# viniciusvidal2/slam-sensor-fusion

Hardware: AMD Instinct MI355X
Metric: scans_per_s_200k_scan_vs_10M_map (higher is better)
Workload: dtype f32 points / f64 accumulation

## Files before the change

include/slamfusion.h:

```cpp
#ifndef SLAMFUSION_H
#define SLAMFUSION_H
#include <stdint.h>

#ifdef __cplusplus
extern "C" {
#endif

#define SF_VERSION 210

typedef enum {
    SF_OK = 0,
    SF_ERR_INVALID = -1,
    SF_ERR_HIP = -2,
    SF_ERR_NOMEM = -3,
    SF_ERR_STATE = -4,
    SF_ERR_OVERFLOW = -5,
    SF_ERR_COMM = -6
} sf_status;

typedef struct sf_ctx sf_ctx;
typedef struct sf_cloud sf_cloud;
typedef struct sf_map sf_map;
typedef struct sf_icp sf_icp;

// ... 28 lines not shown
int sf_cloud_from_pointcloud2(sf_cloud *c, const void *data, int64_t n_points, int point_step, int off_x, int off_y, int off_z);
#define SF_PC2_FLOAT32 7
#define SF_PC2_FLOAT64 8
int sf_cloud_from_pointcloud2_msg(sf_cloud *c, const void *data, int64_t data_bytes, int64_t width, int64_t height, int point_step, int64_t row_step,
                                  int off_x, int off_y, int off_z, int datatype, int is_bigendian);
int sf_cloud_load_pcd(sf_cloud *c, const char *path);
int sf_cloud_save_pcd(sf_cloud *c, const char *path);
int sf_pcd_read(const char *path, float **xyz, int64_t *n);
int sf_pcd_write_binary(const char *path, const float *xyz, int64_t n);
void sf_free(void *p);

#define SF_VOXEL_PCL 0
#define SF_VOXEL_O3D 1
#define SF_VOXEL_PCL64 2
#define SF_FLAG_VOXEL_OVERFLOW 1
int sf_cloud_voxel_downsample(sf_cloud *c, double leaf, int flavour, int *status_flags);
int sf_cloud_voxel_merge(sf_cloud *map, sf_cloud *pending, double leaf, int *status_flags, int *merged);
int sf_cloud_voxel_merge_min_points(int64_t n);
int sf_cloud_voxel_point_ids(sf_cloud *c, int32_t *ids, int64_t cap_values, int64_t *n_values);
int sf_cloud_voxel_out_ids(sf_cloud *c, int32_t *ids, int64_t cap_values, int64_t *n_values);
int sf_cloud_voxel_out_means_f64(sf_cloud *c, double *xyz, int64_t cap_points, int64_t *n_points);
int sf_cloud_voxel_point_ids64(sf_cloud *c, int64_t *ids, int64_t cap_values, int64_t *n_values);
int sf_cloud_voxel_out_ids64(sf_cloud *c, int64_t *ids, int64_t cap_values, int64_t *n_values);

int sf_map_create(sf_ctx *ctx, sf_map **out);
void sf_map_destroy(sf_map *m);
int sf_map_build(sf_map *m, sf_cloud *cloud, float cell);
int sf_map_size(sf_map *m, int64_t *n);
int sf_map_cell_size(sf_map *m, float *cell, int32_t dims[3]);
#define SF_PATCH_NO_MERGE        0
#define SF_PATCH_BOUND_REPLACED (-1)
#define SF_PATCH_ORIGIN_MOVED   (-2)
#define SF_PATCH_LIMITS         (-3)
#define SF_PATCH_CLAMPED_POINT  (-4)
int sf_map_patch(sf_map *m, sf_cloud *cloud, int *patched);
int sf_map_set_origin_lattice(sf_map *m, int cells);
int sf_map_index_info(sf_map *m, int64_t *n_indexed, int64_t *n_cells, float org[3], float *inv_h, float *gap_eps);
int sf_map_download_index(sf_map *m, float *pts4, int64_t cap_points, uint32_t *cell_start, int64_t cap_cells);
int sf_map_window_none(sf_map *m);
int sf_map_window_sphere(sf_map *m, const float center[3], double radius);
int sf_map_window_obb(sf_map *m, const double center[3], const double R[9], const double extent[3]);
int sf_map_window_count(sf_map *m, int64_t *n);
int sf_map_estimate_normals(sf_map *m, float radius);
int sf_map_estimate_normals_cov(sf_map *m, float radius, int with_covariance);
int sf_map_download_covariances(sf_map *m, double *cov6, int64_t cap_points, int64_t *n);
int sf_map_set_normals(sf_map *m, const float *normals, int64_t n);
int sf_map_set_normals_carry(sf_map *m, int on);
int sf_map_normals_carry_info(sf_map *m, int64_t out[4]);
int sf_map_download_normals(sf_map *m, float *normals, int32_t *n_neighbors, int64_t cap, int64_t *n);
int sf_map_nn(sf_map *m, const float *queries, int64_t n, float max_d2, int32_t *idx, float *d2);
#define SF_KNN_MAX 64
int sf_map_knn(sf_map *m, const float *queries, int64_t n, int k, float max_d2, int32_t *idx, float *d2, int32_t *count);
int sf_map_estimate_normals_knn(sf_map *m, int k, float max_radius, int with_covariance);
int sf_map_profile_launches(sf_map *m, int on);
int sf_map_last_launch_ms(sf_map *m, float *ms);

typedef struct {
    float T[16];
    float error;
    int32_t iterations;
    int32_t converged;
    int32_t n_corr;
    int32_t n_research;
    int32_t flags;
    double fitness;
    double rmse;
    double T64[16];
} sf_icp_result;
#define SF_ICP_FLAG_FEW_CORR 1
#define SF_ICP_FLAG_SINGULAR 2
#define SF_ICP_FLAG_BARRIER_TIMEOUT 8
#define SF_ICP_FLAG_SHARD_STALE 4

#define SF_ICP_REF_CPP 0
#define SF_ICP_O3D_P2P 1
#define SF_ICP_P2PLANE 2

int sf_icp_create(sf_ctx *ctx, float max_correspondence_dist, int num_iterations,
                  float acceptable_mean_error, float transformation_epsilon, sf_icp **out);
void sf_icp_destroy(sf_icp *icp);
int sf_icp_set_max_correspondence_dist(sf_icp *icp, float v);
int sf_icp_set_num_iterations(sf_icp *icp, int v);
int sf_icp_set_transformation_epsilon(sf_icp *icp, float v);
int sf_icp_set_acceptable_mean_error(sf_icp *icp, float v);
int sf_icp_set_initial_transformation(sf_icp *icp, const float T[16]);
int sf_icp_set_initial_transformation_f64(sf_icp *icp, const double T[16]);
int sf_icp_set_debug_mode(sf_icp *icp, int on);
int sf_icp_set_source(sf_icp *icp, const float *xyz, int64_t n);
int sf_icp_set_source_cloud(sf_icp *icp, sf_cloud *cloud);
int sf_icp_set_source_scan(sf_icp *icp, sf_cloud *raw, int stride, const float center[3], double radius);
int sf_icp_source_count(sf_icp *icp, int64_t *n);
int sf_icp_set_target(sf_icp *icp, const float *xyz, int64_t n);
int sf_icp_set_target_map(sf_icp *icp, sf_map *map);
int sf_icp_align(sf_icp *icp, int mode, sf_icp_result *out);

int sf_icp_set_source_batch(sf_icp *icp, const float *xyz, int64_t n_per_scan, int batch);
int sf_icp_set_source_batch_device(sf_icp *icp, const void *d_xyz, int64_t n_per_scan, int batch);
int sf_icp_set_initial_batch_f64(sf_icp *icp, const double *inits);
int sf_icp_align_batch(sf_icp *icp, int mode, sf_icp_result *out );
int sf_icp_align_batch_async(sf_icp *icp, int mode);
int sf_icp_fetch_results(sf_icp *icp, sf_icp_result *out);
int sf_icp_fetch_previous(sf_icp *icp, sf_icp_result *out);
int sf_icp_use_graph(sf_icp *icp, int on);
int sf_icp_graph_counts(sf_icp *icp, int64_t *captures, int64_t *launches);
int sf_icp_set_fused(sf_icp *icp, int on);
int sf_icp_fused_count(sf_icp *icp, int64_t *launches);
int sf_icp_fused_redone(sf_icp *icp, int64_t *redone);
int sf_icp_test_inject_barrier_timeout(sf_icp *icp);
#define SF_ORDER_AUTO 0
#define SF_ORDER_AS_GIVEN 1
#define SF_ORDER_CELL 2
int sf_icp_set_query_order(sf_icp *icp, int order);
int sf_icp_set_nn_reuse(sf_icp *icp, int on);
int sf_icp_set_wide_scan_points(sf_icp *icp, int64_t points);
int sf_icp_set_pipeline(sf_icp *icp, int on);
int sf_icp_set_tile_search(sf_icp *icp, int mode);
int sf_icp_tile_info(sf_icp *icp, int64_t out[12]);
int sf_icp_set_freeze(sf_icp *icp, int on);
int sf_icp_set_freeze_params(sf_icp *icp, float guard_scale, float guard_min, float guard_max, int max_tries, int from_launch);
int sf_icp_freeze_stats(sf_icp *icp, int64_t out[5]);
int sf_icp_set_defer_search(sf_icp *icp, int on);
int sf_icp_defer_stats(sf_icp *icp, int64_t out[2]);
#define SF_ROBUST_NONE 0
#define SF_ROBUST_HUBER 1
#define SF_ROBUST_CAUCHY 2
#define SF_ROBUST_TUKEY 3
#define SF_ROBUST_GM 4
int sf_icp_set_robust_kernel(sf_icp *icp, int kind, double k);

#define SF_COV_EIG_EPS 1e-12
#define SF_COV_FEW_CORR 1
#define SF_COV_SINGULAR 2
#define SF_COV_DEGENERATE_TRANS 4
#define SF_COV_DEGENERATE_ROT 8
typedef struct {
    double info[36];
    double cov[36];
    double sigma2, sigma2_hat, weight_sum;
    double trans_info[3], trans_dir[9];
    double rot_info[3], rot_dir[9];
    int64_t n_corr;
    int32_t flags;
} sf_icp_covariance;
int sf_icp_set_covariance(sf_icp *icp, int on, double sensor_sigma);
int sf_icp_set_degeneracy_thresholds(sf_icp *icp, double trans, double rot, double inflate_trans_var, double inflate_rot_var);
int sf_icp_fetch_covariance(sf_icp *icp, sf_icp_covariance *out);
int sf_icp_fetch_covariance_previous(sf_icp *icp, sf_icp_covariance *out);

int sf_icp_set_shard(sf_icp *icp, float x_lo, float x_hi);
int sf_icp_set_shard_margin(sf_icp *icp, float margin_m);
int sf_icp_set_exchange_buffer(sf_icp *icp, void *d_buf, int64_t nbytes);
void *sf_icp_exchange_ptr(sf_icp *icp, int64_t *nbytes);
int sf_icp_step_begin(sf_icp *icp, int mode, int first);
int sf_icp_step_end(sf_icp *icp, int mode, int last);

typedef struct sf_comm sf_comm;
int sf_comm_load_rccl(const char *library_path);
int sf_comm_unique_id(void *id128);
int sf_comm_create(sf_ctx *ctx, int nranks, int rank, const void *id128, sf_comm **out);
void sf_comm_destroy(sf_comm *c);
int sf_comm_size(const sf_comm *c, int *nranks, int *rank);
int sf_comm_allreduce_f64(sf_comm *c, void *d_buf, int64_t count);
#define SF_COMM_RCCL 0
#define SF_COMM_P2P 1
#define SF_COMM_P2P_HANDLE_BYTES 128
int sf_comm_p2p_create(sf_ctx *ctx, int nranks, int rank, int64_t max_count, sf_comm **out);
int sf_comm_p2p_handle(sf_comm *c, void *handle);
int sf_comm_p2p_connect(sf_comm *c, const void *handles);
int sf_comm_p2p_rendezvous(sf_comm *c, const char *name, double timeout_s);
int sf_comm_set_timeout(sf_comm *c, double seconds);
int sf_comm_abort(sf_comm *c);
int sf_comm_status(sf_comm *c);
int sf_comm_kind(const sf_comm *c);
int sf_icp_align_sharded_async(sf_icp *icp, int mode, sf_comm *comm, int first);
int sf_icp_align_sharded(sf_icp *icp, int mode, sf_comm *comm, sf_icp_result *out, int *resumes );
// ... 150 lines not shown
```

slam_sensor_fusion_amd/api.py:

```python
import atexit
import ctypes as C
import os
import weakref

import numpy as np

_HERE = os.path.dirname(os.path.abspath(__file__))
LIB_PATH = os.path.join(_HERE, "lib", "libslamfusion.so")

SF_ICP_REF_CPP, SF_ICP_O3D_P2P, SF_ICP_P2PLANE = 0, 1, 2
SF_VOXEL_PCL, SF_VOXEL_O3D, SF_VOXEL_PCL64 = 0, 1, 2
SF_FLAG_VOXEL_OVERFLOW = 1
SF_ICP_FLAG_FEW_CORR, SF_ICP_FLAG_SINGULAR, SF_ICP_FLAG_SHARD_STALE, SF_ICP_FLAG_BARRIER_TIMEOUT = 1, 2, 4, 8
PROF_NN, PROF_REDUCE, PROF_COLLECTIVE, PROF_SOLVE, PROF_SHARD_BUILD = 0, 1, 2, 3, 4
SF_ERR_COMM = -6
MODES = {"ref_cpp": SF_ICP_REF_CPP, "o3d_p2p": SF_ICP_O3D_P2P, "p2plane": SF_ICP_P2PLANE}
ROBUST_KINDS = {"none": 0, "huber": 1, "cauchy": 2, "tukey": 3, "gm": 4}


class SlamFusionError(RuntimeError):
    pass


class IcpResult(C.Structure):
# ... 328 lines not shown

    def set_origin_lattice(self, cells):
        _check(self.lib.sf_map_set_origin_lattice(self.h, C.c_int(int(cells))))
        return self

    def patch(self, cloud):
        done = C.c_int(0)
        _check(self.lib.sf_map_patch(self.h, cloud.h, C.byref(done)))
        self.last_patch = done.value
        return done.value > 0

    def index(self):
        n, nc, org, inv_h, eps = C.c_int64(), C.c_int64(), (C.c_float * 3)(), C.c_float(), C.c_float()
        _check(self.lib.sf_map_index_info(self.h, C.byref(n), C.byref(nc), org, C.byref(inv_h), C.byref(eps)))
        pts4 = np.empty((max(n.value, 1), 4), np.float32)
        cs = np.empty(nc.value + 1, np.uint32)
        _check(self.lib.sf_map_download_index(self.h, pts4.ctypes.data_as(C.c_void_p), C.c_int64(len(pts4)), cs.ctypes.data_as(C.c_void_p), C.c_int64(len(cs))))
        return dict(pts4=pts4[:n.value], cell_start=cs, org=np.array(list(org), np.float32), inv_h=inv_h.value, gap_eps=eps.value)

    def __len__(self):
        n = C.c_int64()
        _check(self.lib.sf_map_size(self.h, C.byref(n)))
        return n.value

    def cell_size(self):
        cell = C.c_float()
        dims = (C.c_int32 * 3)()
        _check(self.lib.sf_map_cell_size(self.h, C.byref(cell), dims))
        return cell.value, tuple(dims)

    def window_none(self):
        _check(self.lib.sf_map_window_none(self.h))

    def window_sphere(self, center, radius):
        c = _f32(center)
        _check(self.lib.sf_map_window_sphere(self.h, _p(c), C.c_double(radius)))

    def window_obb(self, center, R, extent):
        c, R, e = _f64(center), _f64(R).reshape(3, 3), _f64(extent)
        _check(self.lib.sf_map_window_obb(self.h, _p(c), _p(R), _p(e)))

    def window_count(self):
        n = C.c_int64()
        _check(self.lib.sf_map_window_count(self.h, C.byref(n)))
        return n.value

    def estimate_normals(self, radius, covariance=False):
        _check(self.lib.sf_map_estimate_normals_cov(self.h, C.c_float(radius), C.c_int(int(covariance))))

    def estimate_normals_knn(self, k, max_radius=np.inf, covariance=False):
        r = float(max_radius)
        _check(self.lib.sf_map_estimate_normals_knn(self.h, C.c_int(int(k)), C.c_float(r if np.isfinite(r) else 0.0), C.c_int(int(covariance))))

    def set_normals_carry(self, on=True):
        _check(self.lib.sf_map_set_normals_carry(self.h, C.c_int(int(bool(on)))))
        return self

    def normals_carry_info(self):
        out = (C.c_int64 * 4)()
        _check(self.lib.sf_map_normals_carry_info(self.h, out))
        return tuple(int(v) for v in out)

    def download_covariances(self):
        n = len(self)
        cov = np.empty((n, 6), np.float64)
        _check(self.lib.sf_map_download_covariances(self.h, _p(cov), C.c_int64(n), None))
        return cov

    def set_normals(self, normals):
        nrm = _f32(normals).reshape(-1, 3)
        _check(self.lib.sf_map_set_normals(self.h, _p(nrm), C.c_int64(len(nrm))))

    def download_normals(self):
        n = len(self)
        nrm = np.empty((n, 3), np.float32)
        cnt = np.empty(n, np.int32)
        _check(self.lib.sf_map_download_normals(self.h, _p(nrm), _p(cnt), C.c_int64(n), None))
        return nrm, cnt

    def nn(self, queries, max_d2=np.inf):
        q = _f32(queries).reshape(-1, 3)
        idx = np.empty(len(q), np.int32)
        d2 = np.empty(len(q), np.float32)
        _check(self.lib.sf_map_nn(self.h, _p(q), C.c_int64(len(q)), C.c_float(min(max_d2, 3.0e38)), _p(idx), _p(d2)))
        return idx, d2

    def knn(self, queries, k, max_d2=np.inf):
        q = _f32(queries).reshape(-1, 3)
        k = int(k)
        rows = max(k, 0)
        idx = np.empty((len(q), rows), np.int32)
        d2 = np.empty((len(q), rows), np.float32)
        cnt = np.empty(len(q), np.int32)
        _check(self.lib.sf_map_knn(self.h, _p(q), C.c_int64(len(q)), C.c_int(k), C.c_float(max_d2), _p(idx), _p(d2), _p(cnt)))
        return idx, d2, cnt

    def profile_launches(self, on=True):
        _check(self.lib.sf_map_profile_launches(self.h, C.c_int(int(bool(on)))))
        return self

    def last_launch_ms(self):
        ms = C.c_float()
        _check(self.lib.sf_map_last_launch_ms(self.h, C.byref(ms)))
        return ms.value

    def close(self):
# ... 123 lines not shown
        code = {False: 0, "off": 0, "auto": 1, True: 2, "always": 2}[on]
        _check(self.lib.sf_icp_set_freeze(self.h, C.c_int(code)))

    def set_robust_kernel(self, kind="none", k=None):
        code = ROBUST_KINDS[kind]
        _check(self.lib.sf_icp_set_robust_kernel(self.h, code, float("nan") if k is None and code != 0 else float(k or 0.0)))

    def set_covariance(self, on=True, sensor_sigma=0.0):
        _check(self.lib.sf_icp_set_covariance(self.h, int(bool(on)), float(sensor_sigma)))

    def set_degeneracy_thresholds(self, trans=0.0, rot=0.0, inflate_trans_var=0.0, inflate_rot_var=0.0):
        _check(self.lib.sf_icp_set_degeneracy_thresholds(self.h, float(trans), float(rot), float(inflate_trans_var), float(inflate_rot_var)))

    def fetch_covariance(self, previous=False, batch=None):
        if previous:
            arr = (IcpCovariance * int(batch or getattr(self, "_prev_batch", None) or self.batch))()
            _check(self.lib.sf_icp_fetch_covariance_previous(self.h, arr))
        else:
            arr = (IcpCovariance * int(batch or getattr(self, "_last_batch", None) or self.batch))()
            _check(self.lib.sf_icp_fetch_covariance(self.h, arr))
        return [c.as_dict() for c in arr]

    def set_wide_scan_points(self, points):
        _check(self.lib.sf_icp_set_wide_scan_points(self.h, C.c_int64(int(points))))

    def set_pipeline(self, on=True):
        _check(self.lib.sf_icp_set_pipeline(self.h, C.c_int(int(bool(on)))))

    def set_tile_search(self, on="auto"):
        code = {False: 0, "off": 0, "auto": 1, True: 2, "always": 2}[on]
        _check(self.lib.sf_icp_set_tile_search(self.h, C.c_int(code)))

    def tile_info(self):
        a = (C.c_int64 * 12)()
        _check(self.lib.sf_icp_tile_info(self.h, a))
        return {"on": bool(a[0]), "cells_per_tile": [a[1], a[2], a[3]], "tiles": [a[4], a[5], a[6]], "searched": a[7], "from_lds": a[8], "left_region": a[9],
                "beyond_ring_1": a[10], "tiles_too_dense": a[11]}

    def set_freeze_params(self, guard_scale=8.0, guard_min=2.0e-5, guard_max=3.0e-4, max_tries=3, from_launch=5):
        _check(self.lib.sf_icp_set_freeze_params(self.h, C.c_float(guard_scale), C.c_float(guard_min), C.c_float(guard_max), C.c_int(max_tries), C.c_int(from_launch)))

    def freeze_stats(self):
        a = (C.c_int64 * 5)()
        _check(self.lib.sf_icp_freeze_stats(self.h, a))
        return {"froze": a[0], "thawed": a[1], "failed": a[2], "active_queries": a[3], "frozen_at_end": a[4]}

    def set_defer_search(self, on=True):
        _check(self.lib.sf_icp_set_defer_search(self.h, C.c_int(int(bool(on)))))

    def defer_stats(self):
        a = (C.c_int64 * 2)()
        _check(self.lib.sf_icp_defer_stats(self.h, a))
        return {"deferred_queries": a[0], "capped_waves": a[1]}

    def set_query_order(self, order="auto"):
        _check(self.lib.sf_icp_set_query_order(self.h, C.c_int({"auto": 0, "as_given": 1, "cell": 2}[order])))

    def align(self, mode="ref_cpp"):
        r = IcpResult()
        _check(self.lib.sf_icp_align(self.h, C.c_int(MODES[mode]), C.byref(r)))
        return r.as_dict()

    def align_batch(self, mode="p2plane"):
        arr = (IcpResult * self.batch)()
        _check(self.lib.sf_icp_align_batch(self.h, C.c_int(MODES[mode]), arr))
        self._prev_batch, self._last_batch = getattr(self, "_last_batch", None), self.batch
        return [r.as_dict() for r in arr]

    def align_batch_async(self, mode="p2plane"):
        _check(self.lib.sf_icp_align_batch_async(self.h, C.c_int(MODES[mode])))
        self._prev_batch, self._last_batch = getattr(self, "_last_batch", None), self.batch

    def fetch_results(self, raw=False):
        arr = (IcpResult * int(getattr(self, "_last_batch", None) or self.batch))()
        _check(self.lib.sf_icp_fetch_results(self.h, arr))
        return arr if raw else [r.as_dict() for r in arr]

    def fetch_previous(self, batch=None, raw=False):
        arr = (IcpResult * int(batch or getattr(self, "_prev_batch", None) or self.batch))()
        _check(self.lib.sf_icp_fetch_previous(self.h, arr))
        return arr if raw else [r.as_dict() for r in arr]

    def set_shard(self, x_lo, x_hi):
        _check(self.lib.sf_icp_set_shard(self.h, C.c_float(x_lo), C.c_float(x_hi)))

    def set_exchange_buffer(self, ptr, nbytes):
        _check(self.lib.sf_icp_set_exchange_buffer(self.h, C.c_void_p(ptr), C.c_int64(nbytes)))

    def exchange_ptr(self):
        n = C.c_int64()
        p = self.lib.sf_icp_exchange_ptr(self.h, C.byref(n))
        return p, n.value

    def set_shard_margin(self, margin_m):
        _check(self.lib.sf_icp_set_shard_margin(self.h, C.c_float(margin_m)))

    def step_begin(self, mode, first):
        _check(self.lib.sf_icp_step_begin(self.h, C.c_int(MODES[mode]), C.c_int(int(first))))
        if int(first) == 1:
            self._last_batch = self.batch

    def step_end(self, mode, last):
        _check(self.lib.sf_icp_step_end(self.h, C.c_int(MODES[mode]), C.c_int(int(last))))

    def align_sharded(self, mode, comm):
        arr = (IcpResult * self.batch)()
# ... 610 lines not shown
```

slam_sensor_fusion_amd/csrc/sf_common.hpp:

```cpp
#pragma once
#include <hip/hip_runtime.h>
#include <cstdarg>
#include <cstdint>
#include <cstdio>
#include <cstring>
#include <new>
#include <vector>

#include "slamfusion.h"

namespace sf {

void set_error(const char *fmt, ...);

#define SF_HIP(call)                                                                          \
    do {                                                                                      \
        hipError_t e_ = (call);                                                               \
        if (e_ != hipSuccess) {                                                               \
            sf::set_error("%s failed: %s (%s:%d)", #call, hipGetErrorString(e_), __FILE__,    \
                          __LINE__);                                                          \
            return SF_ERR_HIP;                                                                \
        }                                                                                     \
    } while (0)

// ... 80 lines not shown
    bool zombie = false;
};

struct sf_cloud {
    sf_ctx *ctx = nullptr;
    sf::DevBuf xyz;
    int64_t n = 0;
    sf::DevBuf spare;
    sf::DevBuf flags;
    sf::DevBuf raw;
    sf::DevBuf last_idx;
    int64_t n_last_idx = -1;
    bool vox_wide = false;
    sf::DevBuf vox_point_ids; int64_t n_vox_point_vals = 0;
    sf::DevBuf vox_out_ids;   int64_t n_vox_out_vals = 0;
    sf::DevBuf vox_out_means; int64_t n_vox_out_pts = 0;
    uint64_t stamp = 0;
    uint64_t bounds_stamp = 0;
    float bounds_mn[3] = {0, 0, 0}, bounds_mx[3] = {0, 0, 0};
    struct MergeRecord {
        bool valid = false;
        uint64_t epoch = 0, stamp_before = 0, stamp_after = 0;
        int64_t n_old = 0, n_groups = 0, n_fresh = 0;
        float old_mn[3] = {0, 0, 0}, old_mx[3] = {0, 0, 0};
        float cen_mn[3] = {0, 0, 0}, cen_mx[3] = {0, 0, 0};
        bool touched_extreme = false;
        const uint32_t *coarse = nullptr;
        const uint32_t *g_rank = nullptr, *g_fresh = nullptr, *fresh_pos = nullptr, *fresh_rank = nullptr;
        const float *g_centroid = nullptr, *g_old = nullptr;
    } merge;
};

struct SfWindow {
    int kind;
    float c[3];
    float r2;
    double oc[3];
    double oR[9];
    double ohalf[3];
};

struct SfGrid {
    float org[3];
    float inv_h;
    float h;
    float gap_eps;
    int dim[3];
    const uint32_t *cell_start;
    const float4 *pts;
    const float4 *nrm;
    int64_t n;
};

struct sf_map {
    sf_ctx *ctx = nullptr;
    sf::DevBuf pts4, nrm4, cell_start, keys, vals, keys2, vals2;
    sf::DevBuf pts4_alt, patch_tmp;
    double h_exact = 0;
    float src_mn[3] = {0, 0, 0}, src_mx[3] = {0, 0, 0};
    int origin_lattice = 0;
    uint64_t src_stamp = 0;
    sf::DevBuf d_window;
    sf::DevBuf cov6;
    sf::DevBuf nrm4_alt, cov6_alt, carry_tmp, carry_list;
    bool normals_carry = false;
    bool nrm_estimated = false;
    float nrm_radius = 0;
    int nrm_knn_k = 0;
    bool nrm_with_cov = false;
    int64_t carry_info[4] = {-1, 0, 0, 0};
    bool profile = false;
    hipEvent_t prof_ev[2] = {nullptr, nullptr};
    float last_launch_ms = -1.0f;
    int64_t n = 0;
    bool built = false, has_normals = false, has_cov = false;
    uint64_t generation = 0;
    SfGrid grid{};
    SfWindow window{};
};

struct sf_comm;

namespace sf {
int comm_allreduce_f64(sf_comm *c, void *d_buf, int64_t count);
sf_ctx *comm_ctx(const sf_comm *c);
int compact_cloud(sf_cloud *c, const uint8_t *d_flags);
int ensure_scratch(sf_ctx *ctx, size_t bytes);
int upload_staged(sf_ctx *ctx, void *dst, const void *src, size_t bytes);
uint64_t next_generation();
inline void cloud_touch(sf_cloud *c) { c->stamp = next_generation(); c->merge.valid = false; }
void ctx_retain(sf_ctx *ctx);
void ctx_release(sf_ctx *ctx);
struct MinMaxHost { float mn[3], mx[3]; int64_t n_finite; };
struct MinMaxDev { float mn[3], mx[3]; unsigned long long cnt; };
int cloud_minmax_enqueue(sf_ctx *ctx, const float *d_xyz, int64_t n, MinMaxDev *d_out);
int cloud_minmax(sf_ctx *ctx, const float *d_xyz, int64_t n, MinMaxHost *out);
}
```

slam_sensor_fusion_amd/csrc/sf_icp.hip:

```cpp
#include "sf_common.hpp"
#include "sf_nn.hpp"
#include "sf_tile.hpp"
#include "sf_order.hpp"
#include "sf_p2p.hpp"

#include <cfloat>
#include <cstdlib>
#include <cmath>
#include <vector>
#include <mutex>
#include <string>

namespace {

constexpr int BLK = 256;
constexpr int NREC_P2P = 17;
constexpr int NREC_PLANE = 30;
constexpr int REC_STRIDE = 32;

struct IcpState {
    double T[16];
    double rec[REC_STRIDE];
    double fitness, rmse, prev_fitness, prev_rmse;
    float last_error, err_pending;
// ... 460 lines not shown
    }
    return need;
}

struct QueryIn {
    double sx, sy, sz;
    float qx, qy, qz;
    float4 c1, c2;
    float e;
    size_t o;
    bool valid;
};

template <int MODE, bool SHARD>
__device__ __forceinline__ QueryIn query_in(const float *__restrict__ X0x, const float *__restrict__ X0y, const float *__restrict__ X0z, int n, int b, const IcpState *S, float xlo,
                                            float xhi, const uint32_t *__restrict__ own_off, const float4 *__restrict__ qcache, int64_t cache_n, bool cache_live, int slot,
                                            int n_live)
{
    QueryIn q;
    q.sx = q.sy = q.sz = 0.0;
    q.qx = q.qy = q.qz = 0.0f;
    q.c1 = q.c2 = make_float4(0.f, 0.f, 0.f, 0.f);
    q.e = 0.0f;
    q.o = 0;
    q.valid = false;
    if (slot < n_live) {
        const size_t o = SHARD ? (size_t)own_off[b] + (size_t)slot : (size_t)b * n + (size_t)slot;
        q.o = o;
        if (cache_live) {
            q.c1 = qcache[o];
            if (MODE == 2) { q.c2 = qcache[(size_t)cache_n + o]; q.e = q.c2.w; }
            else q.e = reinterpret_cast<const float *>(qcache + (size_t)cache_n)[o];
        }
        const double x0 = X0x[o], y0 = X0y[o], z0 = X0z[o];
        q.sx = S->T[0] * x0 + S->T[1] * y0 + S->T[2] * z0 + S->T[3];
        q.sy = S->T[4] * x0 + S->T[5] * y0 + S->T[6] * z0 + S->T[7];
        q.sz = S->T[8] * x0 + S->T[9] * y0 + S->T[10] * z0 + S->T[11];
        q.qx = (float)q.sx; q.qy = (float)q.sy; q.qz = (float)q.sz;
        q.valid = !SHARD || (q.qx >= xlo && q.qx < xhi);
    }
    return q;
}

__device__ __forceinline__ LanePair make_pair(const QueryIn &q, const sf::NNHit &hit, const float4 &tn)
{
    LanePair P;
    P.sx = q.sx; P.sy = q.sy; P.sz = q.sz;
    P.px = hit.px; P.py = hit.py; P.pz = hit.pz;
    P.tn = tn;
    P.ok = hit.j >= 0;
    return P;
}

template <int MODE, bool WINDOW, bool SHARD>
__device__ __forceinline__ LanePair nn_pair(const SfGrid &g, const SfWindow &w, const float *__restrict__ X0x, const float *__restrict__ X0y, const float *__restrict__ X0z,
                                            int n, int b, const IcpState *S, float thr, float xlo, float xhi, const uint32_t *__restrict__ own_off,
                                            float4 *__restrict__ qcache, int64_t cache_n, int slot, int n_live, sf::WaveNN *ws, uint32_t *__restrict__ stats,
                                            sf::PhaseClock *pc = nullptr)
{
    const bool cache_live = qcache != nullptr && S->cache_live != 0;
    const QueryIn q = query_in<MODE, SHARD>(X0x, X0y, X0z, n, b, S, xlo, xhi, own_off, qcache, cache_n, cache_live, slot, n_live);
    const float qx = q.qx, qy = q.qy, qz = q.qz;
    const size_t o = q.o;
    float *ecache = reinterpret_cast<float *>(qcache + (size_t)cache_n);
    const float m_now = (float)S->motion;
    sf::NNHit hit;
    float4 tn;
    sf::NNHit seed;
    const bool need = reuse_certificate(q.valid, qx, qy, qz, thr, m_now, q.e, q.c1, q.c2, hit, tn, seed);
    const unsigned long long need_mask = __ballot(need);
    if (stats && (threadIdx.x & 63) == 0 && need_mask) {
        uint32_t *sh = stats + 2 * ((blockIdx.x + blockIdx.y * gridDim.x) & (NN_STATS_SHARDS - 1));
        atomicAdd(&sh[0], (uint32_t)__popcll(need_mask));
        atomicAdd(&sh[1], 1u);
    }
    SF_PH(pc, 0);
    if (need_mask != 0ull) {
        const sf::NNHit h = sf::nn_search_wave<WINDOW>(g, w, need, qx, qy, qz, thr, ws, seed, pc);
        if (need) {
            hit = h;
            if (MODE == 2 && h.j >= 0) tn = g.nrm[h.j];
            if (qcache) {
                const float en = fmaxf(sqrtf(h.lb2) * 0.9999f + m_now * 0.999998f - 1.0e-6f, 1.0e-30f);
                qcache[o] = make_float4(h.px, h.py, h.pz, __int_as_float(h.j));
                if (MODE == 2) qcache[(size_t)cache_n + o] = make_float4(tn.x, tn.y, tn.z, en);
                else ecache[o] = en;
            }
        }
    }
    if (qcache && !cache_live && !need && slot < n_live) {
        if (MODE == 2) qcache[(size_t)cache_n + o] = make_float4(0.f, 0.f, 0.f, 0.f);
        else ecache[o] = 0.0f;
    }
    SF_PH(pc, 6);
    return make_pair(q, hit, tn);
}

struct PairTerms { double wgt, ux, uy, uz, tx, ty, tz, ex, ey, ez, d2, r; double J[6]; };
template <int MODE>
__device__ __forceinline__ PairTerms pair_terms(const LanePair &P)
{
    PairTerms t;
    const bool ok = P.ok;
    t.wgt = ok ? 1.0 : 0.0;
    t.ux = ok ? P.sx : 0.0; t.uy = ok ? P.sy : 0.0; t.uz = ok ? P.sz : 0.0;
    t.tx = (double)(ok ? P.px : 0.0f); t.ty = (double)(ok ? P.py : 0.0f); t.tz = (double)(ok ? P.pz : 0.0f);
    t.ex = t.ux - t.tx; t.ey = t.uy - t.ty; t.ez = t.uz - t.tz;
    t.d2 = t.ex * t.ex + t.ey * t.ey + t.ez * t.ez;
    if (MODE == 2) {
        const double nx = (double)(ok ? P.tn.x : 0.0f), ny = (double)(ok ? P.tn.y : 0.0f), nz = (double)(ok ? P.tn.z : 0.0f);
        t.r = t.ex * nx + t.ey * ny + t.ez * nz;
        t.J[0] = t.uy * nz - t.uz * ny; t.J[1] = t.uz * nx - t.ux * nz; t.J[2] = t.ux * ny - t.uy * nx;
        t.J[3] = nx; t.J[4] = ny; t.J[5] = nz;
    } else {
        t.r = 0.0;
#pragma unroll
        for (int a = 0; a < 6; ++a) t.J[a] = 0.0;
    }
    return t;
}

struct RobustArg { int kind; double k; };
__device__ __forceinline__ double robust_weight(const RobustArg &rk, double r)
// ... 21 lines not shown
            v[13] = fma(t.uz, t.tx, v[13]); v[14] = fma(t.uz, t.ty, v[14]); v[15] = fma(t.uz, t.tz, v[15]);
        } else {
            v[0] += t.d2;
        }
    } else {
        if (h == 0) { v[0] += t.wgt; v[1] = fma(t.r, t.r, v[1]); }
        int k = 2;
#pragma unroll
        for (int a = 0; a < 6; ++a) {
#pragma unroll
            for (int c = a; c < 6; ++c) {
                if (h == 0 && k < 16) v[k] = fma(t.J[a], t.J[c], v[k]);
                if (h == 1 && k >= 16) v[k - 16] = fma(t.J[a], t.J[c], v[k - 16]);
                ++k;
            }
        }
        if (h == 1) {
#pragma unroll
            for (int a = 0; a < 6; ++a) v[7 + a] = fma(t.J[a], t.r, v[7 + a]);
            v[13] += t.d2;
        }
    }
}

__device__ __forceinline__ void add_half_robust(const PairTerms &t, int h, double (&v)[16], double w)
{
    double Jw[6];
#pragma unroll
    for (int a = 0; a < 6; ++a) Jw[a] = w * t.J[a];
    if (h == 0) { v[0] += t.wgt; v[1] = fma(t.r, t.r, v[1]); }
    int k = 2;
#pragma unroll
    for (int a = 0; a < 6; ++a) {
#pragma unroll
        for (int c = a; c < 6; ++c) {
            if (h == 0 && k < 16) v[k] = fma(Jw[a], t.J[c], v[k]);
            if (h == 1 && k >= 16) v[k - 16] = fma(Jw[a], t.J[c], v[k - 16]);
            ++k;
        }
    }
    if (h == 1) {
#pragma unroll
        for (int a = 0; a < 6; ++a) v[7 + a] = fma(Jw[a], t.r, v[7 + a]);
        v[13] += t.d2;
    }
}

#ifdef SF_PHASE_TRACE
__device__ unsigned long long g_phase_trace[sf::PH_SHARDS * sf::PH_SLOTS];
#endif
template <int MODE, bool WINDOW, bool SHARD, int Q>
__global__ __launch_bounds__(BLK, NN_RED_WAVES) void k_nn_red(SfGrid g, SfWindow w, const float *__restrict__ X0x, const float *__restrict__ X0y, const float *__restrict__ X0z,
                                                int n, const IcpState *__restrict__ st, float thr, float xlo, float xhi, double *__restrict__ partials, int nblocks,
                                                const uint32_t *__restrict__ own_off, float4 *__restrict__ qcache, int64_t cache_n, uint32_t *__restrict__ stats)
{
    constexpr bool ROBUST = false;
    [[maybe_unused]] constexpr RobustArg rk{0, 0.0};
#include "sf_nn_red_body.inc"
}

template <bool WINDOW, bool SHARD, int Q>
__global__ __launch_bounds__(BLK, NN_RED_WAVES) void k_nn_red_rob(SfGrid g, SfWindow w, const float *__restrict__ X0x, const float *__restrict__ X0y, const float *__restrict__ X0z,
                                                    int n, const IcpState *__restrict__ st, float thr, float xlo, float xhi, double *__restrict__ partials, int nblocks,
                                                    const uint32_t *__restrict__ own_off, float4 *__restrict__ qcache, int64_t cache_n, uint32_t *__restrict__ stats, RobustArg rk)
{
    constexpr int MODE = 2;
    constexpr bool ROBUST = true;
#include "sf_nn_red_body.inc"
}

constexpr int ORDER_YBLK = 16;
__device__ __forceinline__ uint64_t order_cell(const SfGrid &g, int cx, int cy, int cz)
{
    const uint64_t yb = (uint64_t)(cy / ORDER_YBLK), yi = (uint64_t)(cy % ORDER_YBLK);
    return ((yb * (uint64_t)g.dim[2] + (uint64_t)cz) * ORDER_YBLK + yi) * (uint64_t)g.dim[0] + (uint64_t)cx;
}

struct CellKeyFn {
    SfGrid g;
    const float *x, *y, *z;
    const IcpState *st;
    int n, shift;
    const uint16_t *lut;
    int lut_shift;
    struct Point { float x, y, z; };
    struct Pose { float T[12]; };
    __device__ __forceinline__ Pose prepare(int b) const
    {
        Pose P;
#pragma unroll
        for (int k = 0; k < 12; ++k) P.T[k] = (float)st[b].T[k];
        return P;
    }
    __device__ __forceinline__ Point load(uint32_t o) const { return Point{x[o], y[o], z[o]}; }
    __device__ __forceinline__ uint32_t key(const Pose &P, const Point &p) const
    {
        const float qx = fmaf(P.T[0], p.x, fmaf(P.T[1], p.y, fmaf(P.T[2], p.z, P.T[3])));
        const float qy = fmaf(P.T[4], p.x, fmaf(P.T[5], p.y, fmaf(P.T[6], p.z, P.T[7])));
        const float qz = fmaf(P.T[8], p.x, fmaf(P.T[9], p.y, fmaf(P.T[10], p.z, P.T[11])));
        if (!(isfinite(qx) && isfinite(qy) && isfinite(qz))) return sf::ORD_KEY_NONE;
        const int cx = (int)fminf(fmaxf(floorf((qx - g.org[0]) * g.inv_h), 0.0f), (float)(g.dim[0] - 1));
        const int cy = (int)fminf(fmaxf(floorf((qy - g.org[1]) * g.inv_h), 0.0f), (float)(g.dim[1] - 1));
        const int cz = (int)fminf(fmaxf(floorf((qz - g.org[2]) * g.inv_h), 0.0f), (float)(g.dim[2] - 1));
        if (lut) return (uint32_t)lut[order_cell(g, cx, cy, cz) >> lut_shift];
        const uint64_t key = order_cell(g, cx, cy, cz) >> shift;
        return (uint32_t)(key < (uint64_t)(sf::ORD_KEY_NONE - 1u) ? key : (uint64_t)(sf::ORD_KEY_NONE - 1u));
    }
};

__global__ __launch_bounds__(sf::ORD_BLK) void k_order_hist(sf::OrderSrc s, CellKeyFn kf, uint16_t *__restrict__ keys, uint32_t *__restrict__ counts)
{
    sf::order_hist_body(s, kf, keys, counts);
}

constexpr int ORDER_LUT_LOG2 = 16;
__global__ __launch_bounds__(256) void k_order_lut_hist(SfGrid g, int lut_shift, uint32_t *__restrict__ hist)
{
// ... 688 lines not shown
    return stays_in || stays_out;
}

struct FzArgs {
    const float *X0x, *X0y, *X0z;
    int n;
    const IcpState *st;
    float thr, xlo, xhi;
    double *partials;
    int nblocks;
    const uint32_t *own_off;
    float4 *qcache;
    int64_t cache_n;
    uint32_t *stats;
    const FreezeState *fz;
    double *mom_part;
    uint32_t *act_cnt;
    uint16_t *act_ids;
    const uint32_t *act_all;
};

template <int Q, bool SHARD>
__device__ __forceinline__ void nn_red_fz_row(const SfGrid &g, const SfWindow &w, const FzArgs &A, int b, int bx, int fmode)
{
    constexpr int MODE = 2;
    constexpr int NREC = NREC_PLANE;
    static_assert(FZ_CAP == 64 * Q, "wave 0 takes FZ_CAP active queries in Q rounds of 64");
    const float *__restrict__ X0x = A.X0x, *__restrict__ X0y = A.X0y, *__restrict__ X0z = A.X0z;
    const int n = A.n, nblocks = A.nblocks;
    const float thr = A.thr, xlo = A.xlo, xhi = A.xhi;
    double *__restrict__ partials = A.partials, *__restrict__ mom_part = A.mom_part;
    const uint32_t *__restrict__ own_off = A.own_off, *__restrict__ act_all = A.act_all;
    float4 *__restrict__ qcache = A.qcache;
    const int64_t cache_n = A.cache_n;
    uint32_t *__restrict__ stats = A.stats, *__restrict__ act_cnt = A.act_cnt;
    uint16_t *__restrict__ act_ids = A.act_ids;
    const FreezeState *__restrict__ fz = A.fz;
    const IcpState *S = A.st + b;
    const int n_live = SHARD ? (int)(own_off[b + 1] - own_off[b]) : n;
    const int wv = threadIdx.x >> 6, lane = threadIdx.x & 63;
    const size_t row = (size_t)b * nblocks + bx;
    double *dst = partials + row * REC_STRIDE;
    __shared__ sf::WaveNN nn_ws[BLK / 64];
    LanePair P[Q];
    if (fmode == 2) {
        const int64_t total = fz[b].n_active, first = (int64_t)bx * FZ_CAP;
        if (first >= total) return;
        __shared__ double fstage[Q][32];
        if (wv < Q) {
            const uint32_t cnt = (uint32_t)min<int64_t>(total - first, FZ_CAP);
            const uint32_t *list = act_all + (size_t)b * nblocks * FZ_CAP + (size_t)first;
            const uint32_t i = (uint32_t)(wv * 64 + lane);
            const int slot = i < cnt ? (int)list[i] : n_live;
            const LanePair A1 = nn_pair<MODE, false, SHARD>(g, w, X0x, X0y, X0z, n, b, S, thr, xlo, xhi, own_off, qcache, cache_n, slot, n_live, &nn_ws[wv], stats);
#pragma unroll
            for (int h = 0; h < 2; ++h) {
                double v[16];
#pragma unroll
                for (int k = 0; k < 16; ++k) v[k] = 0.0;
                const PairTerms t = pair_terms<MODE>(A1);
                add_half<MODE>(t, h, v);
                const double t0 = wave_reduce_16(v);
                if ((lane & 3) == 0) fstage[wv][16 * h + (lane >> 2)] = t0;
            }
        }
        __syncthreads();
        if (threadIdx.x < NREC) {
            double v = fstage[0][threadIdx.x];
#pragma unroll
            for (int u = 1; u < Q; ++u) v += fstage[u][threadIdx.x];
            dst[threadIdx.x] = v;
        }
        return;
    }
    if (SHARD && bx * (BLK * Q) >= n_live) return;
    __shared__ double stage[BLK / 64][32];
    __shared__ uint32_t act_w[BLK / 64][Q];
    bool active[Q];
#pragma unroll
    for (int u = 0; u < Q; ++u) active[u] = false;
    bool fast = false;
    const float m_now = (float)S->motion;
    const float guard = fz[b].guard;
    const bool attempted = qcache != nullptr && S->cache_live != 0;
    if (attempted) {
        bool any_need = false;
#pragma unroll
        for (int u = 0; u < Q; ++u) {
            const int slot = bx * (BLK * Q) + u * BLK + (int)threadIdx.x;
            const QueryIn q = query_in<MODE, SHARD>(X0x, X0y, X0z, n, b, S, xlo, xhi, own_off, qcache, cache_n, true, slot, n_live);
            sf::NNHit hit, seed;
            float4 tn;
            any_need = reuse_certificate(q.valid, q.qx, q.qy, q.qz, thr, m_now, q.e, q.c1, q.c2, hit, tn, seed) || any_need;
            P[u] = make_pair(q, hit, tn);
            if (fmode == 1) active[u] = !stays_frozen<SHARD>(q, slot < n_live, thr, m_now, guard, xlo, xhi);
        }
        fast = __ballot(any_need) == 0ull;
    }
    if (!fast) {
        asm volatile("" ::: "memory");
#pragma unroll
        for (int u = 0; u < Q; ++u) {
            const int slot = bx * (BLK * Q) + u * BLK + (int)threadIdx.x;
            P[u] = nn_pair<MODE, false, SHARD>(g, w, X0x, X0y, X0z, n, b, S, thr, xlo, xhi, own_off, qcache, cache_n, slot, n_live, &nn_ws[wv], stats);
            if (fmode == 1 && !attempted) active[u] = slot < n_live;
        }
    }
    if (fmode == 1) {
#pragma unroll
        for (int u = 0; u < Q; ++u) {
            const unsigned long long bal = __ballot(active[u]);
            if (lane == 0) act_w[wv][u] = (uint32_t)__popcll(bal);
        }
        __syncthreads();
        uint32_t total = 0;
#pragma unroll
        for (int u = 0; u < Q; ++u) {
            uint32_t base = 0;
#pragma unroll
            for (int ww = 0; ww < BLK / 64; ++ww) {
                if (ww < wv) base += act_w[ww][u];
                total += act_w[ww][u];
            }
            uint32_t before = 0;
#pragma unroll
            for (int uu = 0; uu < Q; ++uu)
                if (uu < u)
#pragma unroll
                    for (int ww = 0; ww < BLK / 64; ++ww) before += act_w[ww][uu];
            const unsigned long long bal = __ballot(active[u]);
            const uint32_t rank = (uint32_t)__builtin_amdgcn_mbcnt_hi((uint32_t)(bal >> 32), __builtin_amdgcn_mbcnt_lo((uint32_t)bal, 0u));
            const uint32_t pos = before + base + rank;
            if (active[u] && pos < (uint32_t)FZ_CAP) act_ids[row * FZ_CAP + pos] = (uint16_t)(u * BLK + (int)threadIdx.x);
        }
        if (threadIdx.x == 0) act_cnt[row] = total;
    }
    bool wave_has_pairs = true;
    if (fmode == 1) {
        bool any = false;
#pragma unroll
        for (int u = 0; u < Q; ++u) any = any || (P[u].ok && active[u]);
        wave_has_pairs = __ballot(any) != 0ull;
        if (!wave_has_pairs && lane < 32) stage[wv][lane] = 0.0;
    }
    if (wave_has_pairs)
#pragma unroll
    for (int h = 0; h < 2; ++h) {
        double v[16];
#pragma unroll
        for (int k = 0; k < 16; ++k) v[k] = 0.0;
#pragma unroll
        for (int u = 0; u < Q; ++u) {
            LanePair A = P[u];
            if (fmode == 1) A.ok = A.ok && active[u];
            const PairTerms t = pair_terms<MODE>(A);
            add_half<MODE>(t, h, v);
        }
// ... 28 lines not shown
    }
}

template <int Q, bool SHARD>
__global__ __launch_bounds__(BLK, NN_RED_WAVES) void k_nn_red_fz(SfGrid g, SfWindow w, FzArgs A)
{
    const int L = blockIdx.y * gridDim.x + blockIdx.x;
    const int kk = L >> 3;
    const int b = kk % (int)gridDim.y;
    const int bx = (L & 7) * ((int)gridDim.x >> 3) + kk / (int)gridDim.y;
    if (bx >= A.nblocks) return;
    if (A.st[b].done) return;
    nn_red_fz_row<Q, SHARD>(g, w, A, b, bx, A.fz[b].mode);
}

constexpr int FZ_FEW = 16;
template <int Q, bool SHARD>
__global__ __launch_bounds__(BLK, NN_RED_WAVES) void k_nn_red_fz_few(SfGrid g, SfWindow w, FzArgs A)
{
    const int r = (int)blockIdx.x, b = (int)blockIdx.y;
    if (A.st[b].done) return;
    const int fmode = A.fz[b].mode;
    if (fmode == 2) {
        const int64_t total = A.fz[b].n_active;
        for (int bx = r; (int64_t)bx * FZ_CAP < total; bx += FZ_FEW) {
            nn_red_fz_row<Q, SHARD>(g, w, A, b, bx, 2);
            __syncthreads();
        }
        return;
    }
    for (int bx = r; bx < A.nblocks; bx += FZ_FEW) {
        nn_red_fz_row<Q, SHARD>(g, w, A, b, bx, fmode);
        __syncthreads();
    }
}


#ifndef SF_DF_WCAP
#define SF_DF_WCAP 8
#endif
constexpr int DF_WCAP = SF_DF_WCAP;
constexpr int DF_CAPPED = 255;
static_assert((BLK / 64) * DF_WCAP <= FZ_CAP && DF_WCAP < DF_CAPPED, "a row defers fewer queries than it could list as active");
struct DeferBufs {
    uint8_t *cnt;
    uint16_t *ids;
    double *part;
    uint32_t *stat;
};

template <int Q>
__global__ __launch_bounds__(BLK, NN_RED_WAVES) void k_nn_red_df(SfGrid g, SfWindow w, const float *__restrict__ X0x, const float *__restrict__ X0y, const float *__restrict__ X0z,
                                                                 int n, const IcpState *__restrict__ st, float thr, double *__restrict__ partials, int nblocks,
                                                                 float4 *__restrict__ qcache, int64_t cache_n, uint32_t *__restrict__ stats, DeferBufs df)
{
    constexpr int MODE = 2;
    constexpr int NREC = NREC_PLANE;
    const int L = blockIdx.y * gridDim.x + blockIdx.x;
    const int kk = L >> 3;
    const int b = kk % (int)gridDim.y;
    const int bx = (L & 7) * ((int)gridDim.x >> 3) + kk / (int)gridDim.y;
    if (bx >= nblocks) return;
    const IcpState *S = st + b;
    if (S->done) return;
    __shared__ sf::WaveNN nn_ws[BLK / 64];
    __shared__ double stage[BLK / 64][32];
    const int wv = threadIdx.x >> 6, lane = threadIdx.x & 63;
    const size_t seg = ((size_t)b * nblocks + bx) * (BLK / 64) + wv;
    LanePair P[Q];
    bool need[Q];
#pragma unroll
    for (int u = 0; u < Q; ++u) need[u] = false;
    const bool attempted = qcache != nullptr && S->cache_live != 0 && S->n_research >= VERIFY_FROM_SEARCH;
    bool fast = false;
    uint32_t listed = 0;
    if (attempted) {
        const float m_now = (float)S->motion;
#pragma unroll
        for (int u = 0; u < Q; ++u) {
            const int slot = bx * (BLK * Q) + u * BLK + (int)threadIdx.x;
            const QueryIn q = query_in<MODE, false>(X0x, X0y, X0z, n, b, S, 0.0f, 0.0f, nullptr, qcache, cache_n, true, slot, n);
            sf::NNHit hit, seed;
            float4 tn;
            need[u] = reuse_certificate(q.valid, q.qx, q.qy, q.qz, thr, m_now, q.e, q.c1, q.c2, hit, tn, seed);
            P[u] = make_pair(q, hit, tn);
        }
        uint32_t failing = 0;
#pragma unroll
        for (int u = 0; u < Q; ++u) failing += (uint32_t)__popcll(__ballot(need[u]));
        fast = failing <= (uint32_t)DF_WCAP;
        listed = fast ? failing : (uint32_t)DF_CAPPED;
    }
    if (lane == 0) df.cnt[seg] = (uint8_t)listed;
    if (fast && listed != 0u) {
        uint32_t before = 0;
#pragma unroll
        for (int u = 0; u < Q; ++u) {
            const unsigned long long bal = __ballot(need[u]);
            const uint32_t rank = (uint32_t)__builtin_amdgcn_mbcnt_hi((uint32_t)(bal >> 32), __builtin_amdgcn_mbcnt_lo((uint32_t)bal, 0u));
            if (need[u]) df.ids[seg * DF_WCAP + before + rank] = (uint16_t)(u * BLK + (int)threadIdx.x);
            before += (uint32_t)__popcll(bal);
        }
    }
    if (!fast) {
        asm volatile("" ::: "memory");
#pragma unroll
        for (int u = 0; u < Q; ++u) {
            const int slot = bx * (BLK * Q) + u * BLK + (int)threadIdx.x;
            P[u] = nn_pair<MODE, false, false>(g, w, X0x, X0y, X0z, n, b, S, thr, 0.0f, 0.0f, nullptr, qcache, cache_n, slot, n, &nn_ws[wv], stats);
        }
    }
#pragma unroll
    for (int h = 0; h < 2; ++h) {
        double v[16];
#pragma unroll
        for (int k = 0; k < 16; ++k) v[k] = 0.0;
#pragma unroll
        for (int u = 0; u < Q; ++u) {
            const PairTerms t = pair_terms<MODE>(P[u]);
            add_half<MODE>(t, h, v);
        }
        const double t0 = wave_reduce_16(v);
        if ((lane & 3) == 0) stage[wv][16 * h + (lane >> 2)] = t0;
    }
    __syncthreads();
    if (threadIdx.x < NREC) {
        const int c = threadIdx.x;
        double *dst = partials + ((size_t)b * nblocks + bx) * REC_STRIDE;
        dst[c] = ((stage[0][c] + stage[1][c]) + stage[2][c]) + stage[3][c];
    }
}

template <int Q>
__global__ __launch_bounds__(BLK, 2) void k_nn_deferred(SfGrid g, SfWindow w, const float *__restrict__ X0x, const float *__restrict__ X0y, const float *__restrict__ X0z,
                                                                   int n, const IcpState *__restrict__ st, float thr, int nblocks, float4 *__restrict__ qcache, int64_t cache_n,
                                                                   uint32_t *__restrict__ stats, DeferBufs df)
{
    constexpr int MODE = 2;
    constexpr int NW = BLK / 64;
    const int r = (int)blockIdx.x, b = (int)blockIdx.y;
    const IcpState *S = st + b;
    if (S->done) return;
    __shared__ sf::WaveNN nn_ws[NW];
    __shared__ double fstage[NW][32];
    __shared__ uint32_t list[BLK * DF_WCAP];
    __shared__ uint32_t wsum[NW];
    __shared__ uint32_t capped;
    const int wv = threadIdx.x >> 6, lane = threadIdx.x & 63;
    if (threadIdx.x == 0) capped = 0u;
    __syncthreads();
    const int my_rows = r < nblocks ? (nblocks - r + FZ_FEW - 1) / FZ_FEW : 0;
    const int nseg = my_rows * NW;
    double acc = 0.0;
    uint32_t n_listed = 0;
    for (int s0 = 0; s0 < nseg; s0 += BLK) {
        const int sg = s0 + (int)threadIdx.x;
        const int bx = r + (sg / NW) * FZ_FEW;
        const size_t seg = ((size_t)b * nblocks + bx) * NW + (sg % NW);
        uint32_t c = sg < nseg ? (uint32_t)df.cnt[seg] : 0u;
        if (c > (uint32_t)DF_WCAP) {
            atomicAdd(&capped, 1u);
            c = 0u;
        }
        uint32_t incl = c;
#pragma unroll
        for (int off = 1; off < 64; off <<= 1) {
            const uint32_t t = __shfl_up(incl, off, 64);
            if (lane >= off) incl += t;
        }
        if (lane == 63) wsum[wv] = incl;
        __syncthreads();
        uint32_t base = 0, total = 0;
#pragma unroll
        for (int ww = 0; ww < NW; ++ww) {
            if (ww < wv) base += wsum[ww];
            total += wsum[ww];
        }
        const uint32_t start = base + incl - c;
        for (uint32_t i = 0; i < c; ++i) list[start + i] = (uint32_t)bx * (uint32_t)(BLK * Q) + (uint32_t)df.ids[seg * DF_WCAP + i];
        __syncthreads();
        n_listed += total;
        for (uint32_t q0 = 0; q0 < total; q0 += BLK) {
            const uint32_t i = q0 + (uint32_t)threadIdx.x;
            if (q0 + (uint32_t)(wv * 64) < total) {
                const int slot = i < total ? (int)list[i] : n;
                const LanePair A1 = nn_pair<MODE, false, false>(g, w, X0x, X0y, X0z, n, b, S, thr, 0.0f, 0.0f, nullptr, qcache, cache_n, slot, n, &nn_ws[wv], stats);
#pragma unroll
                for (int h = 0; h < 2; ++h) {
                    double v[16];
#pragma unroll
                    for (int k = 0; k < 16; ++k) v[k] = 0.0;
                    const PairTerms t = pair_terms<MODE>(A1);
                    add_half<MODE>(t, h, v);
                    const double t0 = wave_reduce_16(v);
                    if ((lane & 3) == 0) fstage[wv][16 * h + (lane >> 2)] = t0;
                }
            } else if (lane < 32) {
                fstage[wv][lane] = 0.0;
            }
            __syncthreads();
            if (threadIdx.x < 32) acc += ((fstage[0][threadIdx.x] + fstage[1][threadIdx.x]) + fstage[2][threadIdx.x]) + fstage[3][threadIdx.x];
            __syncthreads();
        }
    }
    if (threadIdx.x < REC_STRIDE) df.part[((size_t)b * FZ_FEW + r) * REC_STRIDE + threadIdx.x] = threadIdx.x < NREC_PLANE ? acc : 0.0;
    __syncthreads();
    if (threadIdx.x == 0) {
        if (n_listed) atomicAdd(&df.stat[0], n_listed);
        if (capped) atomicAdd(&df.stat[1], capped);
    }
}

__device__ __forceinline__ void add_deferred_rows(const double *__restrict__ df_part, int b, double *rec)
{
    if (threadIdx.x < NREC_PLANE) {
        double v = 0.0;
#pragma unroll
        for (int r = 0; r < FZ_FEW; ++r) v += df_part[((size_t)b * FZ_FEW + r) * REC_STRIDE + threadIdx.x];
        rec[threadIdx.x] += v;
    }
    __syncthreads();
}

template <int STRIDE, int NCOL, int NT>
__device__ __forceinline__ void reduce_columns(const double *__restrict__ part, int nrows, double *out)
{
    constexpr int NS = 8;
    static_assert(NT % 128 == 0 && NT / 128 >= 1 && NT / 128 <= NS && NCOL <= 128, "slices of 128 columns");
    __shared__ double sl[NS][128];
    const int c = threadIdx.x & 127;
    for (int sidx = threadIdx.x >> 7; sidx < NS; sidx += NT / 128) {
        double v0 = 0, v1 = 0, v2 = 0, v3 = 0;
        if (c < NCOL) {
            int r = sidx;
            for (; r + 3 * NS < nrows; r += 4 * NS) {
                const double a0 = part[(size_t)r * STRIDE + c], a1 = part[(size_t)(r + NS) * STRIDE + c];
                const double a2 = part[(size_t)(r + 2 * NS) * STRIDE + c], a3 = part[(size_t)(r + 3 * NS) * STRIDE + c];
                v0 += a0; v1 += a1; v2 += a2; v3 += a3;
            }
// ... 171 lines not shown
                F->froze += 1;
                if (S->froze_launch < 0) S->froze_launch = S->n_research;
                F->motion0 = S->motion;
                for (int i = 0; i < 12; ++i) { F->Tf[i] = S->T[i]; F->D[i] = (i % 5 == 0) ? 1.0 : 0.0; }
                for (int i = 0; i < FZ_NMOM; ++i) F->mom[i] = mom[i];
            }
        }
    }
    __syncthreads();
}

__device__ __forceinline__ void freeze_after_update(const IcpState *S, FreezeState *F, double m0, double m1, const FreezeParams &fp, int request, const double *upd)
{
    if (F->mode == 2) {
        double Dn[12];
        for (int r = 0; r < 3; ++r) {
            for (int c = 0; c < 4; ++c) Dn[4 * r + c] = upd[4 * r] * F->D[c] + upd[4 * r + 1] * F->D[4 + c] + upd[4 * r + 2] * F->D[8 + c] + (c == 3 ? upd[4 * r + 3] : 0.0);
        }
        for (int i = 0; i < 12; ++i) F->D[i] = Dn[i];
    }
    if (F->mode == 2 && !(m1 - F->motion0 <= (double)F->guard * 0.98)) {
        F->mode = 0;
        F->tries += 1;
        F->thawed += 1;
    }
    if (F->mode == 0 && F->launch_mode == 0 && request && !S->done && F->tries < fp.max_tries) {
        const float gd = fmaxf((float)(m1 - m0) * fp.guard_scale, fp.guard_min);
        if (gd <= fp.guard_max) { F->guard = gd; F->mode = 1; }
    }
}

__global__ __launch_bounds__(RBLK) void k_reduce_solve_fz(IcpState *__restrict__ st, const double *__restrict__ partials, int nblocks, int n_src, int K,
                                                          const ScanBox *__restrict__ boxp, FreezeBufs fb, FreezeParams fp, int request)
{
    const int b = blockIdx.x;
    IcpState *S = st + b;
    if (S->done) return;
    FreezeState *F = fb.fz + b;
    __shared__ double rec[REC_STRIDE];
    freeze_fold<RBLK>(S, F, b, partials, nblocks, nblocks, fb, rec);
    if (fb.df_part) add_deferred_rows(fb.df_part, b, rec);
    if (threadIdx.x == 0) {
        for (int c = 0; c < NREC_PLANE; ++c) S->rec[c] = rec[c];
        double To[12];
#pragma unroll
        for (int i = 0; i < 12; ++i) To[i] = S->T[i];
        const double m0 = S->motion;
        double upd[12];
        solve_plane(S, rec, n_src, K, upd);
        track_motion(S, To, boxp[b]);
        freeze_after_update(S, F, m0, S->motion, fp, request, upd);
    }
}

__global__ void k_fz_init(FreezeState *__restrict__ fz, int batch, uint32_t *__restrict__ df_stat)
{
    const int b = blockIdx.x * blockDim.x + threadIdx.x;
    if (b == 0) df_stat[0] = df_stat[1] = 0u;
    if (b >= batch) return;
    FreezeState *F = fz + b;
    F->mode = 0; F->tries = 0; F->froze = 0; F->thawed = 0; F->n_active = 0; F->guard = 0.0f; F->launch_mode = 0; F->motion0 = 0.0;
}

constexpr int SBLK = 256;
template <int MODE>
__global__ __launch_bounds__(SBLK) void k_reduce_only(IcpState *__restrict__ st, const double *__restrict__ partials, int nblocks, double *__restrict__ xchg,
                                                      const uint32_t *__restrict__ own_off, int qpl, FreezeBufs fb)
{
    constexpr int NREC = MODE == 2 ? NREC_PLANE : NREC_P2P;
    const int b = blockIdx.x;
    __shared__ double rec[REC_STRIDE];
    if (st[b].done) {
        if (threadIdx.x < REC_STRIDE) xchg[(size_t)b * REC_STRIDE + threadIdx.x] = 0.0;
        return;
    }
    const int rows = own_off ? (int)((own_off[b + 1] - own_off[b] + BLK * qpl - 1) / (BLK * qpl)) : nblocks;
    if (MODE == 2 && fb.fz) freeze_fold<SBLK>(st + b, fb.fz + b, b, partials, nblocks, rows, fb, rec);
    else reduce_partials<NREC, SBLK>(partials + (size_t)b * nblocks * REC_STRIDE, rows, rec);
    if (MODE == 2 && fb.df_part) add_deferred_rows(fb.df_part, b, rec);
    if (threadIdx.x < REC_STRIDE) xchg[(size_t)b * REC_STRIDE + threadIdx.x] = rec[threadIdx.x];
}

template <int MODE>
__global__ void k_solve_only(IcpState *__restrict__ st, const double *__restrict__ xchg, int n_src, int K, int batch, const ScanBox *__restrict__ boxp, float margin,
                             FreezeState *__restrict__ fz, FreezeParams fp, int request)
{
    constexpr int NREC = MODE == 2 ? NREC_PLANE : NREC_P2P;
    const int b = blockIdx.x * blockDim.x + threadIdx.x;
    if (b >= batch) return;
    IcpState *S = st + b;
    if (S->done) return;
    double rec[REC_STRIDE];
#pragma unroll
    for (int c = 0; c < REC_STRIDE; ++c) rec[c] = c < NREC ? xchg[(size_t)b * REC_STRIDE + c] : 0.0;
#pragma unroll
    for (int c = 0; c < NREC; ++c) S->rec[c] = rec[c];
    double To[12];
#pragma unroll
    for (int i = 0; i < 12; ++i) To[i] = S->T[i];
    const double m0 = S->motion;
    double upd[12];
    if (MODE == 1) solve_o3d(S, rec, n_src, 0, K);
    else solve_plane(S, rec, n_src, K, upd);
    track_motion(S, To, boxp[b]);
    if (margin > 0.0f && !S->done) own_check_motion(S, boxp[b], margin);
    if (MODE == 2 && fz) freeze_after_update(S, fz + b, m0, S->motion, fp, request, upd);
// ... 473 lines not shown
#include "sf_icp_fused_body.inc"
}

#include "sf_cov.hpp"

}

struct sf_icp {
    sf_ctx *ctx = nullptr;
    IcpParams prm{};
    int debug = 0;
    int64_t cache_n = 0;
    bool reuse = true;
    int order = SF_ORDER_AUTO;
    bool ordered = false;
    std::vector<double> inits;
    double *h_inits = nullptr;
    size_t h_inits_cap = 0;
    hipEvent_t inits_ev = nullptr;
    bool inits_ev_pending = false;
    sf_map *map = nullptr;
    sf_map *own_map = nullptr;
    sf_cloud *own_cloud = nullptr;
    sf::DevBuf xchg_own;
    void *xchg = nullptr;
    int64_t xchg_bytes = 0;
    int64_t wide_from = WIDE_SCAN_POINTS;
    bool wide_auto = true;
    std::vector<IcpState> h_state;
    bool shard = false;
    float xlo = 0, xhi = 0;
    sf::DevBuf own_idx, own_blk, own_count, own_off, own_keep;
    std::vector<uint32_t> h_own;
    int64_t own_total = 0;
    float own_margin = 1.0f;
    int own_nblocks = 1;
    sf::DevBuf d_box;
    int last_mode = 0;
    bool fused = true;
    bool last_fused = false;
    sf::DevBuf bar;
    int fused_limit[4] = {-1, -1, -1, -1};
    double fused_share = 0.0;
    int64_t fused_redone = 0;
    bool inject_timeout = false;
    int64_t fused_launches = 0;
    IcpState *h_pin = nullptr;
    size_t h_pin_cap = 0;
    bool use_graph = false;
    int64_t graph_captures = 0, graph_replays = 0;
    struct GraphKey {
        int mode = -1, iters = -1, batch = -1, window = -1, ordered = -1, reuse = -1, robust_kind = -1, cov_on = -1;
        int64_t n = -1;
        const void *map = nullptr;
        uint64_t map_generation = 0, epochs = 0;
        float max_corr = 0, accept = 0, eps = 0;
        double robust_k = 0;
        double cov_prm[5] = {0, 0, 0, 0, 0};
        bool operator==(const GraphKey &o) const
        {
            return mode == o.mode && iters == o.iters && batch == o.batch && window == o.window && ordered == o.ordered && reuse == o.reuse && n == o.n && map == o.map &&
                   map_generation == o.map_generation && epochs == o.epochs && max_corr == o.max_corr && accept == o.accept && eps == o.eps &&
                   robust_kind == o.robust_kind && robust_k == o.robust_k && cov_on == o.cov_on && std::memcmp(cov_prm, o.cov_prm, sizeof(cov_prm)) == 0;
        }
    };
    struct LaneMeta {
        bool valid = false;
        bool cov = false;
        int batch = 0, mode = 0;
        std::vector<double> inits;
        int src_set = 0;
        uint64_t src_version = 0;
    };
    struct Lane {
        sf::DevBuf X;
        sf::DevBuf qcache;
        sf::DevBuf Xq, qkeys, qkeys2, qidx, qidx2;
        sf::DevBuf corr;
        sf::DevBuf state, d_inits, partials;
        sf::DevBuf fz_state, fz_part, fz_cnt, fz_ids, fz_all;
        sf::DevBuf df_cnt, df_ids, df_part, df_stat;
        sf::DevBuf qtkey, tseg, tile_stats;
        sf::DevBuf cov_part, cov_out;
        hipGraphExec_t graph_exec = nullptr;
        GraphKey graph_key;
        std::vector<double> inits_uploaded;
        uint32_t d_inits_epoch = 0xffffffffu;
        hipStream_t stream = nullptr;
        hipEvent_t done = nullptr;
        bool used = false;
        hipEvent_t started = nullptr;
        bool started_rec = false;
        LaneMeta meta;
    } lanes[2];
    int lane = 0;
    Lane &cur() { return lanes[lane]; }
    const Lane &cur() const { return lanes[lane]; }
    Lane &prev() { return lanes[lane ^ 1]; }
    struct SrcSet {
        sf::DevBuf X0;
        sf::DevBuf X0r;
        sf::DevBuf stage;
        sf::DevBuf d_boxes, d_box_parts;
        sf::DevBuf n_dev;
        int64_t n = 0;
        int64_t n_cap = 0;
        int64_t plane = 0;
        int batch = 0;
        int nblocks = 0;
        int nblocks_nn = 0;
        int qpl = 1;
        bool have_source = false;
        bool n_on_device = false;
        hipEvent_t used = nullptr;
        bool used_rec = false;
    } srcs[2];
    int src_set = 0;
    SrcSet &src() { return srcs[src_set]; }
    const SrcSet &src() const { return srcs[src_set]; }
    hipEvent_t src_ready = nullptr;
    bool src_ahead = false;
    hipEvent_t unmarked_ev = nullptr;
    bool src_unmarked_use = false;
    bool prev_ok = false;
    std::vector<IcpState> h_prev;
    sf::DevBuf order_lut;
    uint64_t order_lut_gen = 0;
    int order_lut_shift = 0, order_lut_on = 1;
    int pipeline = 1;
    hipEvent_t main_mark = nullptr;
    bool unfetched = false;
    bool mark_valid = false;
    uint64_t src_version = 0, mark_src_version = 0, mark_map_generation = 0;
    const void *mark_map = nullptr;
    SfWindow mark_window{};
    bool profiling = false;
    std::vector<hipEvent_t> ev;
    size_t ev_used = 0;
    int64_t prof_launches = 0;
    double prof_ms = 0;
    std::vector<float> prof_each;
    std::vector<int> ev_kind;
    std::vector<float> prof_phase[SF_PROF_KINDS];
    sf::DevBuf nn_stats;
    int freeze = 1;
    FreezeParams fz_prm{8.0f, 2.0e-5f, 3.0e-4f, 3};
    int fz_from = 5;
    bool fz_from_auto = true;
    int fz_fetches = 0;
    int fz_step = 0;
    int defer = 1;
    bool df_planned = false;
    int64_t nn_stats_used = 0;
    static constexpr int64_t NN_STATS_CAP = 1024;
    int robust_kind = SF_ROBUST_NONE;
    double robust_k = 0.0;
    int cov_on = 0;
    CovArg cov_arg{0.0, 0.0, 0.0, 0.0, 0.0};
    bool prev_cov_ok = false;
    int tile_mode = 0;
    bool tile_on = false;
    sf::SfTiles tiles{};
};

namespace {

using Lane = sf_icp::Lane;
using SrcSet = sf_icp::SrcSet;
float *soa(sf::DevBuf &b, int64_t total, int axis) { return b.as<float>() + (size_t)axis * (size_t)total; }
const float *queries(sf_icp *icp, int axis)
{
    Lane &ln = icp->cur(); SrcSet &ss = icp->src();
    if (icp->shard) return soa(ln.Xq, icp->own_total, axis);
    return soa(icp->ordered ? ln.Xq : ss.X0, ss.plane, axis);
}

int fused_capacity(sf_icp *icp, int mode, bool robust = false);

bool robust_on(const sf_icp *icp, int mode) { return mode == SF_ICP_P2PLANE && icp->robust_kind != SF_ROBUST_NONE; }
RobustArg robust_arg(const sf_icp *icp) { return RobustArg{icp->robust_kind, icp->robust_k}; }

constexpr int64_t ORDER_AUTO_MIN_QUERIES = 300000;

struct OrderSpan { uint64_t cells; int bits; };
OrderSpan order_span(const SfGrid &g)
{
    const uint64_t ny_pad = ((uint64_t)g.dim[1] + ORDER_YBLK - 1) / ORDER_YBLK * ORDER_YBLK;
    OrderSpan sp{(uint64_t)g.dim[0] * ny_pad * (uint64_t)g.dim[2], 0};
    while (sp.bits < 63 && (1ull << sp.bits) < sp.cells) ++sp.bits;
    return sp;
}

int order_key_shift(const SfGrid &g) { return std::max(0, order_span(g).bits - sf::ORD_KEY_BITS); }

int reuse_reset(sf_icp *icp, int64_t count)
{
    if (!icp->reuse && !icp->tile_on) return SF_OK;
    const size_t c = (size_t)std::max<int64_t>(count, 1);
    SF_TRY(icp->cur().qcache.reserve(sizeof(float4) * 2 * c));
    icp->cache_n = (int64_t)c;
    return SF_OK;
}

// ... 12 lines not shown
        if (tc[a] <= 2) return false;
        tc[a] /= 2;
    }
    for (;;) {
        int a = tc[2] <= tc[1] && tc[2] <= tc[0] ? 2 : (tc[1] <= tc[0] ? 1 : 0);
        int t2[3] = {tc[0], tc[1], tc[2]};
        t2[a] *= 2;
        if (!fits_tables(t2) || region_cells(t2) * density > budget) break;
        tc[0] = t2[0]; tc[1] = t2[1]; tc[2] = t2[2];
    }
    if (!fits_tables(tc)) return false;
    sf::SfTiles tl;
    int64_t nt = 1;
    for (int a = 0; a < 3; ++a) {
        tl.tc[a] = tc[a];
        tl.nt[a] = (g.dim[a] + tc[a] - 1) / tc[a];
        nt *= tl.nt[a];
    }
    if (nt >= (int64_t)TILE_KEY_NONE) return false;
    tl.ntiles = (int)nt;
    *out = tl;
    return true;
}

bool tile_wanted(const sf_icp *icp, int mode)
{
    const SrcSet &ss = icp->src();
    if (icp->tile_mode == 0 || robust_on(icp, mode) || icp->shard || icp->map->window.kind != 0 || (mode != SF_ICP_P2PLANE && mode != SF_ICP_O3D_P2P)) return false;
    if (ss.qpl == 1) return false;
    return icp->tile_mode == 2 || ss.n * ss.batch >= TILE_AUTO_MIN_QUERIES;
}

bool tile_launch(const sf_icp *icp, int k) { return icp->tile_on && (!icp->reuse || k < VERIFY_FROM_SEARCH); }

constexpr int ORDER_LUT_BINS = (1 << ORDER_LUT_LOG2) + 1;
int order_lut_prepare(sf_icp *icp)
{
    if (!icp->order_lut_on || !icp->map || !icp->map->built) return SF_OK;
    const SfGrid &g = icp->map->grid;
    if (g.n <= 0 || (icp->order_lut.p && icp->order_lut_gen == icp->map->generation)) return SF_OK;
    const OrderSpan sp = order_span(g);
    icp->order_lut_shift = std::max(0, sp.bits - ORDER_LUT_LOG2);
    const int nbins = (int)(sp.cells >> icp->order_lut_shift) + 1;
    SF_TRY(icp->order_lut.reserve(sizeof(uint32_t) * (size_t)ORDER_LUT_BINS + sizeof(uint16_t) * (size_t)ORDER_LUT_BINS));
    uint32_t *hist = icp->order_lut.as<uint32_t>();
    uint16_t *lut = reinterpret_cast<uint16_t *>(hist + ORDER_LUT_BINS);
    hipStream_t st = icp->ctx->stream;
    SF_HIP(hipMemsetAsync(hist, 0, sizeof(uint32_t) * (size_t)ORDER_LUT_BINS, st));
    hipLaunchKernelGGL(k_order_lut_hist, dim3(nblk(g.n)), dim3(256), 0, st, g, icp->order_lut_shift, hist);
    hipLaunchKernelGGL(k_order_lut_make, dim3(1), dim3(1024), 0, st, hist, nbins, (uint32_t)g.n, lut);
    SF_HIP(hipGetLastError());
    icp->order_lut_gen = icp->map->generation;
    return SF_OK;
}

int run_order_sort(sf_icp *icp, int nseg, int64_t longest, int64_t total, const uint32_t *seg_off, const uint32_t *src_idx)
{
    Lane &ln = icp->cur(); SrcSet &ss = icp->src();
    const SfGrid &g = icp->map->grid;
    if (seg_off) icp->tile_on = false;
    sf::OrderSrc src;
    src.src_idx = src_idx;
    src.seg_off = seg_off;
    src.n = (int)ss.n;
    src.tiles = (int)std::max<int64_t>(1, sf::div_up(longest, sf::ORD_TILE));
    CellKeyFn kf;
    kf.g = g;
    kf.x = soa(ss.X0, ss.plane, 0); kf.y = soa(ss.X0, ss.plane, 1); kf.z = soa(ss.X0, ss.plane, 2);
    kf.st = ln.state.as<IcpState>();
    kf.shift = order_key_shift(g);
    kf.lut = nullptr;
    kf.lut_shift = 0;
    if (icp->order_lut_on && icp->order_lut.p && icp->order_lut_gen == icp->map->generation) {
        kf.lut = reinterpret_cast<const uint16_t *>(icp->order_lut.as<uint32_t>() + ORDER_LUT_BINS);
        kf.lut_shift = icp->order_lut_shift;
    }
    const size_t cap = (size_t)std::max<int64_t>(total, 1);
    SF_TRY(ln.Xq.reserve(sizeof(float) * 3 * std::max(cap, (size_t)(seg_off ? 0 : ss.plane))));
    SF_TRY(ln.qkeys.reserve(sizeof(uint16_t) * cap));
    SF_TRY(ln.qkeys2.reserve(sizeof(uint32_t) * (size_t)nseg * (size_t)(src.tiles + 1) * sf::ORD_BINS));
    SF_TRY(ln.qidx.reserve(sizeof(uint32_t) * cap));
    uint16_t *keys = ln.qkeys.as<uint16_t>();
    uint32_t *counts = ln.qkeys2.as<uint32_t>(), *ordered = ln.qidx.as<uint32_t>();
    hipStream_t s = icp->ctx->stream;
    src.nseg = nseg;
    const dim3 grid(sf::order_grid(src.tiles, nseg)), blk(sf::ORD_BLK);
    if (icp->tile_on) {
        TileKeyFn tk;
        tk.g = g; tk.tl = icp->tiles;
        tk.x = kf.x; tk.y = kf.y; tk.z = kf.z;
        tk.st = kf.st; tk.n = (int)ss.n;
        const bool two = icp->tiles.ntiles > sf::ORD_BINS;
        uint32_t *first = ordered;
        if (two) {
            SF_TRY(ln.qidx2.reserve(sizeof(uint32_t) * cap));
            first = ln.qidx2.as<uint32_t>();
        }
        tk.digit = 0;
        hipLaunchKernelGGL(k_order_hist_tile, grid, blk, 0, s, src, tk, keys, counts);
        hipLaunchKernelGGL(sf::k_order_scan, dim3((unsigned)nseg), dim3(sf::ORD_BINS), 0, s, counts, src.tiles);
        hipLaunchKernelGGL(k_order_scatter, grid, blk, 0, s, src, keys, counts, first);
        if (two) {
            sf::OrderSrc src2 = src;
            src2.src_idx = first;
            tk.digit = 1;
            hipLaunchKernelGGL(k_order_hist_tile, grid, blk, 0, s, src2, tk, keys, counts);
// ... 64 lines not shown
{
    if (!icp->src_ahead) return SF_OK;
    SF_HIP(hipStreamWaitEvent(s, icp->src_ready, 0));
    icp->src_ahead = false;
    return SF_OK;
}

struct SrcScope {
    sf_icp *icp;
    hipStream_t main = nullptr;
    bool ahead = false;
    uint64_t version0 = 0;
    int rc = SF_OK;
    SrcScope(sf_icp *i, bool allowed) : icp(i), main(i->ctx->stream), version0(i->src_version)
    {
        static const bool ahead_on = []() { const char *e = std::getenv("SF_SRC_AHEAD"); return !e || std::atoi(e) != 0; }();
        const bool go = ahead_on && allowed && icp->pipeline != 0 && icp->unfetched && !icp->shard && !icp->profiling;
        if (!go) {
            rc = wait_src_ahead(icp, main);
            return;
        }
        rc = ensure_lanes(icp);
        if (rc != SF_OK) return;
        if (!icp->src_ahead) icp->src_set ^= 1;
        const SrcSet &ss = icp->src();
        hipStream_t ls = icp->prev().stream;
        if (icp->src_unmarked_use) {
            if (hipEventRecord(icp->unmarked_ev, main) != hipSuccess || hipStreamWaitEvent(ls, icp->unmarked_ev, 0) != hipSuccess) { rc = SF_ERR_HIP; return; }
            icp->src_unmarked_use = false;
        }
        if (ss.used_rec && hipStreamWaitEvent(ls, ss.used, 0) != hipSuccess) { rc = SF_ERR_HIP; return; }
        static const bool stagger_on = []() { const char *e = std::getenv("SF_UPLOAD_STAGGER"); return !e || std::atoi(e) != 0; }();
        if (stagger_on && icp->cur().started_rec && hipStreamWaitEvent(ls, icp->cur().started, 0) != hipSuccess) { rc = SF_ERR_HIP; return; }
        icp->ctx->stream = ls;
        ahead = true;
    }
    ~SrcScope()
    {
        hipStream_t ran = icp->ctx->stream;
        icp->ctx->stream = main;
        if (!ahead) return;
        if (hipEventRecord(icp->src_ready, ran) == hipSuccess) icp->src_ahead = true;
        if (icp->mark_valid && icp->mark_src_version == version0) icp->mark_src_version = icp->src_version;
    }
};

int lane_reserve(sf_icp *icp)
{
    Lane &ln = icp->cur(); const SrcSet &ss = icp->src();
    const int batch = std::max(ss.batch, 1);
    SF_TRY(ln.state.reserve(sizeof(IcpState) * (size_t)batch));
    SF_TRY(ln.d_inits.reserve(sizeof(double) * 16 * (size_t)batch));
    SF_TRY(ln.partials.reserve(sizeof(double) * (size_t)REC_STRIDE * (size_t)std::max(ss.nblocks, 1) * (size_t)batch));
    return SF_OK;
}

int icp_alloc(sf_icp *icp, int64_t n, int batch, bool outputs = true)
{
    Lane &ln = icp->cur(); SrcSet &ss = icp->src();
    const int64_t total = n * batch;
    ss.plane = std::max<int64_t>(ss.plane, sf::div_up(std::max<int64_t>(total, 1), 4096) * 4096);
    SF_TRY(ss.X0.reserve(sizeof(float) * 3 * (size_t)ss.plane));
    SF_TRY(ss.X0r.reserve(sizeof(float4) * (size_t)ss.plane));
    ss.n_cap = batch == 1 ? sf::div_up(std::max<int64_t>(n, 1), 4096) * 4096 : n;
    ss.nblocks = (int)std::max<int64_t>(1, sf::div_up(ss.n_cap, BLK));
    bool wide = n > icp->wide_from;
    if (!wide && icp->wide_auto && n > WIDE_AUTO_POINTS) {
        const int64_t cap = std::max(fused_capacity(icp, SF_ICP_O3D_P2P), fused_capacity(icp, SF_ICP_P2PLANE));
        wide = sf::div_up(n, BLK) * (int64_t)batch > cap;
    }
    ss.qpl = wide ? SF_WIDE_QPL : 1;
    ss.nblocks_nn = (int)std::max<int64_t>(1, sf::div_up(n, BLK * ss.qpl));
    ss.n = n;
    ss.batch = batch;
    if (outputs) {
        const auto e0 = ln.state.epoch;
        SF_TRY(lane_reserve(icp));
        if (ln.state.epoch != e0) ln.meta.valid = false;
        SF_TRY(icp->xchg_own.reserve(sizeof(double) * REC_STRIDE * (size_t)batch));
    }
    if (icp->inits.size() != (size_t)batch * 16) {
        icp->inits.assign((size_t)batch * 16, 0.0);
        for (int b = 0; b < batch; ++b)
            for (int d = 0; d < 4; ++d) icp->inits[(size_t)b * 16 + 5 * d] = 1.0;
    }
    icp->h_state.resize((size_t)batch);
    return SF_OK;
}

int icp_set_source_device_aos(sf_icp *icp, const float *d_aos, int64_t n, int batch, bool ahead = false)
{
    SrcSet &ss = icp->src();
    SF_TRY(icp_alloc(icp, n, batch, !ahead));
    ss.n_on_device = false;
    const int64_t total = n * batch;
    if (total > 0)
        hipLaunchKernelGGL(k_soa_from_aos, dim3(nblk(total)), dim3(256), 0, icp->ctx->stream, d_aos, total, soa(ss.X0, ss.plane, 0), soa(ss.X0, ss.plane, 1),
                           soa(ss.X0, ss.plane, 2), ss.X0r.as<float4>());
    SF_TRY(ss.n_dev.reserve(sizeof(int)));
    hipLaunchKernelGGL(k_set_int, dim3(1), dim3(1), 0, icp->ctx->stream, ss.n_dev.as<int>(), (int)n);
    SF_HIP(hipGetLastError());
    SF_TRY(ss.d_boxes.reserve(sizeof(ScanBox) * (size_t)std::max(batch, 1)));
    SF_TRY(ss.d_box_parts.reserve(sizeof(ScanBox) * BOX_PARTS * (size_t)std::max(batch, 1)));
    hipLaunchKernelGGL(k_scan_boxes_partial, dim3(BOX_PARTS, (unsigned)std::max(batch, 1)), dim3(256), 0, icp->ctx->stream, soa(ss.X0, ss.plane, 0), soa(ss.X0, ss.plane, 1),
                       soa(ss.X0, ss.plane, 2), (int)n, ss.d_box_parts.as<ScanBox>());
    hipLaunchKernelGGL(k_scan_boxes_final, dim3(nblk(std::max(batch, 1), 64)), dim3(64), 0, icp->ctx->stream, ss.d_box_parts.as<ScanBox>(), std::max(batch, 1), ss.d_boxes.as<ScanBox>());
    ss.have_source = true;
    icp->src_version += 1;
    return SF_OK;
}

struct ProfScope {
    sf_icp *icp;
    explicit ProfScope(sf_icp *i, int kind = SF_PROF_NN) : icp(i)
    {
        if (!icp->profiling) return;
        while (icp->ev.size() < icp->ev_used + 2) {
            hipEvent_t e;
            if (hipEventCreate(&e) != hipSuccess) { icp->profiling = false; return; }
            icp->ev.push_back(e);
        }
        if (icp->ev_kind.size() < icp->ev_used / 2 + 1) icp->ev_kind.resize(icp->ev_used / 2 + 1);
        icp->ev_kind[icp->ev_used / 2] = kind;
        hipError_t e = hipEventRecord(icp->ev[icp->ev_used], icp->ctx->stream);
        (void)e;
    }
    ~ProfScope()
    {
        if (!icp->profiling) return;
        hipError_t e = hipEventRecord(icp->ev[icp->ev_used + 1], icp->ctx->stream);
        (void)e;
        icp->ev_used += 2;
    }
};

void prof_collect(sf_icp *icp)
{
    for (size_t k = 0; k + 1 < icp->ev_used; k += 2) {
        float ms = 0;
        if (hipEventElapsedTime(&ms, icp->ev[k], icp->ev[k + 1]) != hipSuccess) continue;
        const int kind = k / 2 < icp->ev_kind.size() ? icp->ev_kind[k / 2] : SF_PROF_NN;
        if (kind == SF_PROF_NN) { icp->prof_ms += ms; icp->prof_launches += 1; icp->prof_each.push_back(ms); }
        else if (kind > 0 && kind < SF_PROF_KINDS) icp->prof_phase[kind].push_back(ms);
    }
    icp->ev_used = 0;
}

sf_icp::GraphKey graph_key_now(const sf_icp *icp, int mode)
{
    const Lane &ln = icp->cur(); const SrcSet &ss = icp->src();
    sf_icp::GraphKey k;
    k.mode = mode; k.iters = icp->prm.num_iters; k.batch = ss.batch; k.window = icp->map->window.kind; k.ordered = (int)icp->ordered | ((int)icp->tile_on << 1); k.reuse = (int)icp->reuse | (icp->freeze << 1) | (icp->fz_from << 3) | (icp->defer << 16);
    k.n = (mode == SF_ICP_REF_CPP && ss.batch == 1) ? -ss.n_cap : ss.n;
    k.map = (const void *)icp->map;
    k.map_generation = icp->map->generation;
    k.robust_kind = robust_on(icp, mode) ? icp->robust_kind : SF_ROBUST_NONE; k.robust_k = robust_on(icp, mode) ? icp->robust_k : 0.0;
    k.cov_on = icp->cov_on;
    if (icp->cov_on) { const double cp[5] = {icp->cov_arg.sensor_sigma, icp->cov_arg.thr_t, icp->cov_arg.thr_r, icp->cov_arg.infl_t, icp->cov_arg.infl_r}; std::memcpy(k.cov_prm, cp, sizeof(cp)); }
    k.max_corr = icp->prm.max_corr; k.accept = icp->prm.accept; k.eps = icp->prm.eps + icp->fz_prm.guard_scale * 1.0e-3f + icp->fz_prm.guard_min + icp->fz_prm.guard_max + (float)icp->fz_prm.max_tries;
    const sf::DevBuf *bufs[] = {&ss.X0, &ss.X0r, &ln.X, &ln.Xq, &ln.qcache, &ln.corr, &ln.state, &ln.partials, &icp->d_box, &ss.d_boxes, &ss.n_dev,
                                &icp->map->pts4, &icp->map->nrm4, &icp->map->cell_start, &icp->map->d_window, &ln.fz_state, &ln.fz_part, &ln.fz_cnt, &ln.fz_ids, &ln.fz_all, &ln.df_cnt, &ln.df_ids, &ln.df_part, &ln.df_stat, &ln.tseg, &ln.tile_stats, &ln.cov_part, &ln.cov_out};
    k.epochs = (uint64_t)ss.plane;
    for (const sf::DevBuf *b : bufs) k.epochs = (k.epochs * 1000003ull + b->epoch) * 1000003ull + (uint64_t)(uintptr_t)b->p;
    return k;
}

float o3d_thr(const sf_icp *icp) { return (float)((double)icp->prm.max_corr * (double)icp->prm.max_corr); }

template <int MODE>
void launch_nn_red(sf_icp *icp, bool sharded = false, bool one_per_lane = false)
{
    Lane &ln = icp->cur(); SrcSet &ss = icp->src();
    sf_map *m = icp->map;
    const int nb = sharded ? (one_per_lane ? icp->own_nblocks * ss.qpl : icp->own_nblocks) : (one_per_lane ? ss.nblocks : ss.nblocks_nn);
    const dim3 grid((unsigned)((nb + 7) & ~7), (unsigned)ss.batch), blk(BLK);
    const float *x = queries(icp, 0), *y = queries(icp, 1), *z = queries(icp, 2);
    const IcpState *st = ln.state.as<IcpState>();
    double *part = ln.partials.as<double>();
    const float thr = o3d_thr(icp);
    hipStream_t s = icp->ctx->stream;
    ProfScope ps(icp);
    uint32_t *stats = nullptr;
    if (icp->profiling && icp->nn_stats.p && icp->nn_stats_used < sf_icp::NN_STATS_CAP) stats = icp->nn_stats.as<uint32_t>() + 2 * NN_STATS_SHARDS * icp->nn_stats_used++;
    const bool win = m->window.kind != 0;
    if (MODE == 2 && robust_on(icp, MODE)) {
        const RobustArg rk = robust_arg(icp);
#define SF_LAUNCH_NNRED_ROB(W, S, QQ)                                                                                                                         \
    hipLaunchKernelGGL((k_nn_red_rob<W, S, QQ>), grid, blk, 0, s, m->grid, m->window, x, y, z, (int)ss.n, st, thr, icp->xlo, icp->xhi, part, nb, \
                       icp->own_off.as<uint32_t>(), icp->reuse ? ln.qcache.as<float4>() : nullptr, icp->cache_n, stats, rk)
        const bool q1 = ss.qpl == 1 || one_per_lane;
        if (win && sharded) { if (q1) SF_LAUNCH_NNRED_ROB(true, true, 1); else SF_LAUNCH_NNRED_ROB(true, true, SF_WIDE_QPL); }
        else if (win) { if (q1) SF_LAUNCH_NNRED_ROB(true, false, 1); else SF_LAUNCH_NNRED_ROB(true, false, SF_WIDE_QPL); }
        else if (sharded) { if (q1) SF_LAUNCH_NNRED_ROB(false, true, 1); else SF_LAUNCH_NNRED_ROB(false, true, SF_WIDE_QPL); }
        else { if (q1) SF_LAUNCH_NNRED_ROB(false, false, 1); else SF_LAUNCH_NNRED_ROB(false, false, SF_WIDE_QPL); }
#undef SF_LAUNCH_NNRED_ROB
        return;
    }
#define SF_LAUNCH_NNRED_Q(W, S, QQ)                                                                                                                              \
    hipLaunchKernelGGL((k_nn_red<MODE, W, S, QQ>), grid, blk, 0, s, m->grid, m->window, x, y, z, (int)ss.n, st, thr, icp->xlo, icp->xhi, part, nb, \
                       icp->own_off.as<uint32_t>(), icp->reuse ? ln.qcache.as<float4>() : nullptr, icp->cache_n, stats)
#define SF_LAUNCH_NNRED(W, S)                                  \
    do {                                                       \
        if (ss.qpl == 1 || one_per_lane) SF_LAUNCH_NNRED_Q(W, S, 1); \
        else SF_LAUNCH_NNRED_Q(W, S, SF_WIDE_QPL);             \
    } while (0)
    if (win && sharded) SF_LAUNCH_NNRED(true, true);
    else if (win) SF_LAUNCH_NNRED(true, false);
    else if (sharded) SF_LAUNCH_NNRED(false, true);
    else SF_LAUNCH_NNRED(false, false);
#undef SF_LAUNCH_NNRED_Q
#undef SF_LAUNCH_NNRED
}

template <int MODE>
void launch_tile_search(sf_icp *icp, bool one_per_lane)
{
    Lane &ln = icp->cur(); SrcSet &ss = icp->src();
    sf_map *m = icp->map;
    const int nb = one_per_lane ? ss.nblocks : ss.nblocks_nn;
    const float *x = queries(icp, 0), *y = queries(icp, 1), *z = queries(icp, 2);
    const IcpState *st = ln.state.as<IcpState>();
    const float thr = o3d_thr(icp);
    hipStream_t s = icp->ctx->stream;
    ProfScope ps(icp);
    unsigned long long *stats = icp->profiling ? ln.tile_stats.as<unsigned long long>() : nullptr;
    if (icp->profiling && icp->nn_stats.p && icp->nn_stats_used < sf_icp::NN_STATS_CAP) icp->nn_stats_used++;
    const unsigned tgrid = (unsigned)((icp->tiles.ntiles + 7) & ~7);
    hipLaunchKernelGGL((k_tile_search<MODE>), dim3(tgrid), dim3(sf::TILE_BLK), 0, s, m->grid, icp->tiles, x, y, z, (int)ss.n, ss.batch, st, thr, ln.tseg.as<uint32_t>(),
                       ln.qcache.as<float4>(), icp->cache_n, (int)icp->reuse, stats);
    const dim3 grid((unsigned)((nb + 7) & ~7), (unsigned)ss.batch), blk(BLK);
    if (ss.qpl == 1 || one_per_lane)
        hipLaunchKernelGGL((k_red_cached<MODE, 1>), grid, blk, 0, s, x, y, z, (int)ss.n, st, thr, ln.partials.as<double>(), nb, ln.qcache.as<float4>(), icp->cache_n);
    else
        hipLaunchKernelGGL((k_red_cached<MODE, SF_WIDE_QPL>), grid, blk, 0, s, x, y, z, (int)ss.n, st, thr, ln.partials.as<double>(), nb, ln.qcache.as<float4>(), icp->cache_n);
}

bool freeze_on(const sf_icp *icp, int mode)
{
    const SrcSet &ss = icp->src();
    const int64_t nq = icp->shard ? icp->own_total : ss.n * ss.batch;
    const bool wanted = icp->freeze == 2 || (icp->freeze == 1 && nq >= FREEZE_AUTO_MIN_QUERIES);
    return mode == SF_ICP_P2PLANE && wanted && !robust_on(icp, mode) && icp->reuse && ss.qpl == SF_WIDE_QPL && icp->map->window.kind == 0 && icp->prm.num_iters > icp->fz_from + 1 &&
           icp->fz_from >= VERIFY_FROM_SEARCH;
}

int freeze_alloc(sf_icp *icp)
{
    Lane &ln = icp->cur(); SrcSet &ss = icp->src();
    const size_t rows = (size_t)ss.batch * (size_t)std::max(ss.nblocks_nn, icp->shard ? icp->own_nblocks : 0);
    SF_TRY(ln.fz_state.reserve(sizeof(FreezeState) * (size_t)ss.batch));
    SF_TRY(ln.fz_part.reserve(sizeof(double) * FZ_NMOM * rows));
    SF_TRY(ln.fz_cnt.reserve(sizeof(uint32_t) * rows));
    SF_TRY(ln.fz_ids.reserve(sizeof(uint16_t) * FZ_CAP * rows));
    SF_TRY(ln.fz_all.reserve(sizeof(uint32_t) * FZ_CAP * rows));
    SF_TRY(ln.df_cnt.reserve(sizeof(uint8_t) * (BLK / 64) * rows));
    SF_TRY(ln.df_ids.reserve(sizeof(uint16_t) * (BLK / 64) * DF_WCAP * rows));
    SF_TRY(ln.df_part.reserve(sizeof(double) * REC_STRIDE * FZ_FEW * (size_t)ss.batch));
    SF_TRY(ln.df_stat.reserve(sizeof(uint32_t) * 2));
    return SF_OK;
}

FreezeBufs freeze_bufs(sf_icp *icp, bool on, bool deferred = false)
{
    Lane &ln = icp->cur();
    FreezeBufs fb;
    fb.fz = on ? ln.fz_state.as<FreezeState>() : nullptr;
    fb.mom_part = ln.fz_part.as<double>();
    fb.act_cnt = ln.fz_cnt.as<uint32_t>();
    fb.act_ids = ln.fz_ids.as<uint16_t>();
    fb.act_all = ln.fz_all.as<uint32_t>();
    fb.df_part = deferred ? ln.df_part.as<double>() : nullptr;
    return fb;
}

DeferBufs defer_bufs(sf_icp *icp)
{
    Lane &ln = icp->cur();
    DeferBufs d;
    d.cnt = ln.df_cnt.as<uint8_t>();
    d.ids = ln.df_ids.as<uint16_t>();
    d.part = ln.df_part.as<double>();
    d.stat = ln.df_stat.as<uint32_t>();
    return d;
}

bool defer_now(const sf_icp *icp, int mode, int k)
{
    return freeze_on(icp, mode) && icp->defer != 0 && !icp->shard && k >= VERIFY_FROM_SEARCH && k + 1 == icp->fz_from;
}

bool defer_planned(const sf_icp *icp, int mode) { return defer_now(icp, mode, icp->fz_from - 1); }

void launch_nn_deferred(sf_icp *icp, uint32_t *stats)
{
    Lane &ln = icp->cur(); SrcSet &ss = icp->src();
    sf_map *m = icp->map;
    hipLaunchKernelGGL((k_nn_deferred<SF_WIDE_QPL>), dim3((unsigned)FZ_FEW, (unsigned)ss.batch), dim3(BLK), 0, icp->ctx->stream, m->grid, m->window, queries(icp, 0), queries(icp, 1), queries(icp, 2),
                       (int)ss.n, ln.state.as<IcpState>(), o3d_thr(icp), ss.nblocks_nn, ln.qcache.as<float4>(), icp->cache_n, stats, defer_bufs(icp));
}

void launch_nn_red_df(sf_icp *icp)
{
    Lane &ln = icp->cur(); SrcSet &ss = icp->src();
    sf_map *m = icp->map;
    const int nb = ss.nblocks_nn;
    const dim3 grid((unsigned)((nb + 7) & ~7), (unsigned)ss.batch), blk(BLK);
    ProfScope ps(icp);
    uint32_t *stats = nullptr;
    if (icp->profiling && icp->nn_stats.p && icp->nn_stats_used < sf_icp::NN_STATS_CAP) stats = icp->nn_stats.as<uint32_t>() + 2 * NN_STATS_SHARDS * icp->nn_stats_used++;
    hipLaunchKernelGGL((k_nn_red_df<SF_WIDE_QPL>), grid, blk, 0, icp->ctx->stream, m->grid, m->window, queries(icp, 0), queries(icp, 1), queries(icp, 2), (int)ss.n, ln.state.as<IcpState>(),
                       o3d_thr(icp), ln.partials.as<double>(), nb, ln.qcache.as<float4>(), icp->cache_n, stats, defer_bufs(icp));
    launch_nn_deferred(icp, stats);
}

void launch_nn_red_fz(sf_icp *icp, bool sharded, bool few)
{
    Lane &ln = icp->cur(); SrcSet &ss = icp->src();
    sf_map *m = icp->map;
    const int nb = sharded ? icp->own_nblocks : ss.nblocks_nn;
    const dim3 grid_full((unsigned)((nb + 7) & ~7), (unsigned)ss.batch), grid_few((unsigned)FZ_FEW, (unsigned)ss.batch), blk(BLK);
    ProfScope ps(icp);
    FzArgs A;
    A.X0x = queries(icp, 0); A.X0y = queries(icp, 1); A.X0z = queries(icp, 2);
    A.n = (int)ss.n;
    A.st = ln.state.as<IcpState>();
    A.thr = o3d_thr(icp); A.xlo = icp->xlo; A.xhi = icp->xhi;
    A.partials = ln.partials.as<double>();
    A.nblocks = nb;
    A.own_off = icp->own_off.as<uint32_t>();
    A.qcache = ln.qcache.as<float4>();
    A.cache_n = icp->cache_n;
    A.stats = nullptr;
    if (icp->profiling && icp->nn_stats.p && icp->nn_stats_used < sf_icp::NN_STATS_CAP) A.stats = icp->nn_stats.as<uint32_t>() + 2 * NN_STATS_SHARDS * icp->nn_stats_used++;
    A.fz = ln.fz_state.as<FreezeState>();
    A.mom_part = ln.fz_part.as<double>();
    A.act_cnt = ln.fz_cnt.as<uint32_t>();
    A.act_ids = ln.fz_ids.as<uint16_t>();
    A.act_all = ln.fz_all.as<uint32_t>();
    hipStream_t s = icp->ctx->stream;
    if (few) {
        if (sharded) hipLaunchKernelGGL((k_nn_red_fz_few<SF_WIDE_QPL, true>), grid_few, blk, 0, s, m->grid, m->window, A);
        else hipLaunchKernelGGL((k_nn_red_fz_few<SF_WIDE_QPL, false>), grid_few, blk, 0, s, m->grid, m->window, A);
    } else {
        if (sharded) hipLaunchKernelGGL((k_nn_red_fz<SF_WIDE_QPL, true>), grid_full, blk, 0, s, m->grid, m->window, A);
        else hipLaunchKernelGGL((k_nn_red_fz<SF_WIDE_QPL, false>), grid_full, blk, 0, s, m->grid, m->window, A);
    }
}

bool freeze_nn_now(const sf_icp *icp, int mode) { return freeze_on(icp, mode) && icp->fz_step >= icp->fz_from; }
bool freeze_solve_now(const sf_icp *icp, int mode) { return freeze_on(icp, mode) && icp->fz_step + 1 >= icp->fz_from; }
int freeze_start_pass(sf_icp *icp, int mode)
{
    Lane &ln = icp->cur(); SrcSet &ss = icp->src();
    icp->fz_step = 0;
    if (!freeze_on(icp, mode)) return SF_OK;
    SF_TRY(freeze_alloc(icp));
    hipLaunchKernelGGL(k_fz_init, dim3(nblk(ss.batch, 64)), dim3(64), 0, icp->ctx->stream, ln.fz_state.as<FreezeState>(), ss.batch, ln.df_stat.as<uint32_t>());
    return SF_OK;
}

int launch_state_init(sf_icp *icp)
{
    Lane &ln = icp->cur();
    hipStream_t s = icp->ctx->stream;
// ... 23 lines not shown
    }
    hipLaunchKernelGGL(k_state_init, dim3(nblk(B, 64)), dim3(64), 0, s, ln.state.as<IcpState>(), ln.d_inits.as<double>(), args, B);
    return SF_OK;
}

#define COV_DECLINE_MSG "the pose covariance (sf_icp_set_covariance) serves unsharded alignments enqueued whole: switch it off for sharded / stepping alignments"
int cov_alloc(sf_icp *icp)
{
    Lane &ln = icp->cur(); SrcSet &ss = icp->src();
    const size_t B = (size_t)std::max(ss.batch, 1);
    SF_TRY(ln.cov_part.reserve(sizeof(double) * (size_t)REC_STRIDE * (size_t)std::max(ss.nblocks, 1) * B));
    SF_TRY(ln.cov_out.reserve(sizeof(sf_icp_covariance) * B));
    return SF_OK;
}

template <int MODE>
void launch_cov(sf_icp *icp, bool in_list)
{
    Lane &ln = icp->cur(); SrcSet &ss = icp->src();
    sf_map *m = icp->map;
    hipStream_t s = icp->ctx->stream;
    const int nb = ss.nblocks, B = ss.batch;
    const dim3 grid((unsigned)((nb + 7) & ~7), (unsigned)B), blk(BLK);
    const bool win = m->window.kind != 0;
    const float thr = MODE == 0 ? icp->prm.max_corr : o3d_thr(icp);
    const SfWindow *wdev = (MODE == 0 && win && in_list) ? m->d_window.as<SfWindow>() : nullptr;
    const int *nl = (MODE == 0 && B == 1) ? ss.n_dev.as<int>() : nullptr;
    const RobustArg rk = robust_on(icp, MODE) ? robust_arg(icp) : RobustArg{SF_ROBUST_NONE, 0.0};
    double *part = ln.cov_part.as<double>();
    if (win)
        hipLaunchKernelGGL((k_nn_cov<MODE, true>), grid, blk, 0, s, m->grid, m->window, wdev, queries(icp, 0), queries(icp, 1), queries(icp, 2), (int)ss.n, nl, ln.state.as<IcpState>(), thr, part, nb, rk);
    else
        hipLaunchKernelGGL((k_nn_cov<MODE, false>), grid, blk, 0, s, m->grid, m->window, wdev, queries(icp, 0), queries(icp, 1), queries(icp, 2), (int)ss.n, nl, ln.state.as<IcpState>(), thr, part, nb, rk);
    hipLaunchKernelGGL(k_cov_solve<MODE>, dim3((unsigned)B), dim3(COV_SBLK), 0, s, part, nb, icp->cov_arg, ln.cov_out.as<sf_icp_covariance>());
}

void enqueue_cov(sf_icp *icp, int mode, bool in_list)
{
    if (mode == SF_ICP_REF_CPP) launch_cov<0>(icp, in_list);
    else if (mode == SF_ICP_O3D_P2P) launch_cov<1>(icp, in_list);
    else launch_cov<2>(icp, in_list);
}

int enqueue_align(sf_icp *icp, int mode)
{
    Lane &ln = icp->cur(); SrcSet &ss = icp->src();
    sf_map *m = icp->map;
    hipStream_t s = icp->ctx->stream;
    IcpState *st = ln.state.as<IcpState>();
    double *part = ln.partials.as<double>();
    const int K = icp->prm.num_iters;
    const int B = ss.batch;
    const int n = (int)ss.n;
    if (mode == SF_ICP_O3D_P2P) {
        for (int k = 0; k <= K; ++k) {
            if (tile_launch(icp, k)) launch_tile_search<1>(icp, false);
            else launch_nn_red<1>(icp);
            hipLaunchKernelGGL(k_reduce_solve<1>, dim3(B), dim3(RBLK), 0, s, st, part, ss.nblocks_nn, n, k, K, ss.d_boxes.as<ScanBox>());
        }
    } else if (mode == SF_ICP_P2PLANE) {
        const bool fz = freeze_on(icp, mode);
        if (fz) {
            hipLaunchKernelGGL(k_fz_init, dim3(nblk(B, 64)), dim3(64), 0, s, ln.fz_state.as<FreezeState>(), B, ln.df_stat.as<uint32_t>());
        }
        const bool wide = ss.qpl > 1 && !icp->shard;
        for (int k = 0; k < K; ++k) {
            const bool q1 = wide && k < VERIFY_FROM_SEARCH;
            const bool df = !q1 && defer_now(icp, mode, k);
            if (fz && k >= icp->fz_from) launch_nn_red_fz(icp, false, k > icp->fz_from);
            else if (tile_launch(icp, k)) launch_tile_search<2>(icp, q1);
            else if (df) launch_nn_red_df(icp);
            else launch_nn_red<2>(icp, false, q1);
            if (fz && k + 1 >= icp->fz_from)
                hipLaunchKernelGGL(k_reduce_solve_fz, dim3(B), dim3(RBLK), 0, s, st, part, q1 ? ss.nblocks : ss.nblocks_nn, n, K, ss.d_boxes.as<ScanBox>(), freeze_bufs(icp, true, df),
                                   icp->fz_prm, (int)(k + 2 < K));
            else if (q1)
                hipLaunchKernelGGL(k_reduce_solve<2>, dim3(B), dim3(RBLK), 0, s, st, part, ss.nblocks, n, k, K, ss.d_boxes.as<ScanBox>());
            else
                hipLaunchKernelGGL(k_reduce_solve<2>, dim3(B), dim3(RBLK), 0, s, st, part, ss.nblocks_nn, n, k, K, ss.d_boxes.as<ScanBox>());
        }
    } else {
        SF_TRY(ln.X.reserve(sizeof(float) * 3 * (size_t)std::max<int64_t>(ss.plane, 1)));
        SF_TRY(ln.corr.reserve(sizeof(float4) * (size_t)std::max<int64_t>(ss.plane, 1)));
        float *Xx = soa(ln.X, ss.plane, 0), *Xy = soa(ln.X, ss.plane, 1), *Xz = soa(ln.X, ss.plane, 2);
        float4 *corr = ln.corr.as<float4>();
        const dim3 gpts((unsigned)ss.nblocks, (unsigned)B), gred((unsigned)ss.nblocks, (unsigned)B);
        const int *nl = B == 1 ? ss.n_dev.as<int>() : nullptr;
        const bool win = m->window.kind != 0;
        const float thr = icp->prm.max_corr;
        const dim3 gnn((unsigned)((ss.nblocks + 7) & ~7), (unsigned)B);
        auto nn = [&](int force) {
            ProfScope ps(icp);
            if (win) hipLaunchKernelGGL(k_ref_nn<true>, gnn, dim3(BLK), 0, s, m->grid, m->d_window.as<SfWindow>(), Xx, Xy, Xz, n, nl, st, thr, force, corr, ss.nblocks);
            else hipLaunchKernelGGL(k_ref_nn<false>, gnn, dim3(BLK), 0, s, m->grid, (const SfWindow *)nullptr, Xx, Xy, Xz, n, nl, st, thr, force, corr, ss.nblocks);
        };
        auto red = [&](int apply, int only_research) {
            hipLaunchKernelGGL(k_ref_red, gred, dim3(BLK), 0, s, Xx, Xy, Xz, n, nl, st, corr, apply, only_research, part, ss.nblocks);
        };
        auto decide = [&](int phase) { hipLaunchKernelGGL(k_ref_decide, dim3(B), dim3(RBLK), 0, s, st, part, ss.nblocks, icp->prm, phase); };
        hipLaunchKernelGGL(k_ref_init, gpts, dim3(BLK), 0, s, queries(icp, 0), queries(icp, 1), queries(icp, 2), n, nl, st, Xx, Xy, Xz, corr);
        nn(1);
        red(0, 0);
        decide(0);
        for (int i = 0; i < K; ++i) {
            decide(1);
            nn(0);
// ... 177 lines not shown
        r->T[i] = (float)r->T64[i];
    }
    r->iterations = S.iterations;
    r->n_corr = S.n_corr;
    r->n_research = S.n_research;
    r->flags = S.flags;
    r->fitness = S.fitness;
    r->rmse = S.rmse;
    if (mode == SF_ICP_REF_CPP) {
        r->error = failed ? 1e6f : S.last_error;
        r->converged = failed ? 0 : (S.last_error < icp->prm.accept);
    } else {
        r->error = (float)S.rmse;
        r->converged = S.converged;
    }
}

int states_to_host(sf_icp *icp, int count = -1)
{
    hipStream_t s = icp->ctx->stream;
    const size_t nb = (size_t)(count >= 0 ? count : icp->src().batch);
    if (icp->h_state.size() < nb) icp->h_state.resize(nb);
    if (icp->last_fused && icp->h_pin) {
        SF_HIP(hipStreamSynchronize(s));
        std::memcpy(icp->h_state.data(), icp->h_pin, sizeof(IcpState) * nb);
        return SF_OK;
    }
    SF_HIP(hipMemcpyAsync(icp->h_state.data(), icp->cur().state.p, sizeof(IcpState) * nb, hipMemcpyDeviceToHost, s));
    SF_HIP(hipStreamSynchronize(s));
    return SF_OK;
}

int fetch_states(sf_icp *icp)
{
    SF_TRY(states_to_host(icp));
    if (icp->profiling) prof_collect(icp);
    return SF_OK;
}

}

extern "C" int sf_icp_create(sf_ctx *ctx, float max_correspondence_dist, int num_iterations, float acceptable_mean_error, float transformation_epsilon, sf_icp **out)
{
    SF_CHECK(ctx && out, SF_ERR_INVALID, "bad arguments");
    sf_icp *icp = new (std::nothrow) sf_icp();
    SF_CHECK(icp, SF_ERR_NOMEM, "out of host memory");
    icp->ctx = ctx;
    sf::ctx_retain(ctx);
    icp->prm.max_corr = max_correspondence_dist;
    icp->prm.num_iters = num_iterations;
    icp->prm.accept = acceptable_mean_error;
    icp->prm.eps = transformation_epsilon;
    if (const char *e = std::getenv("SF_ORDER_LUT")) icp->order_lut_on = std::atoi(e) != 0;
    *out = icp;
    return SF_OK;
}

extern "C" void sf_icp_destroy(sf_icp *icp)
{
    if (!icp) return;
    hipError_t e = hipStreamSynchronize(icp->ctx->stream);
    (void)e;
    fused_release(icp);
    for (Lane &ln : icp->lanes)
        if (ln.graph_exec) { e = hipGraphExecDestroy(ln.graph_exec); (void)e; }
    for (Lane &ln : icp->lanes) {
        if (ln.stream) { e = hipStreamSynchronize(ln.stream); (void)e; e = hipStreamDestroy(ln.stream); (void)e; }
        if (ln.done) { e = hipEventDestroy(ln.done); (void)e; }
        if (ln.started) { e = hipEventDestroy(ln.started); (void)e; }
    }
    for (SrcSet &ss : icp->srcs)
        if (ss.used) { e = hipEventDestroy(ss.used); (void)e; }
    if (icp->src_ready) { e = hipEventDestroy(icp->src_ready); (void)e; }
    if (icp->unmarked_ev) { e = hipEventDestroy(icp->unmarked_ev); (void)e; }
    if (icp->main_mark) { e = hipEventDestroy(icp->main_mark); (void)e; }
    for (hipEvent_t ev : icp->ev) { e = hipEventDestroy(ev); (void)e; }
    if (icp->inits_ev) { e = hipEventDestroy(icp->inits_ev); (void)e; }
    if (icp->h_inits) { e = hipHostFree(icp->h_inits); (void)e; }
    if (icp->h_pin) { e = hipHostFree(icp->h_pin); (void)e; }
    if (icp->own_map) sf_map_destroy(icp->own_map);
    if (icp->own_cloud) sf_cloud_destroy(icp->own_cloud);
    sf_ctx *ctx = icp->ctx;
    delete icp;
    sf::ctx_release(ctx);
}

extern "C" int sf_icp_set_max_correspondence_dist(sf_icp *icp, float v) { SF_CHECK(icp, SF_ERR_INVALID, "icp is NULL"); icp->prm.max_corr = v; return SF_OK; }
extern "C" int sf_icp_set_num_iterations(sf_icp *icp, int v) { SF_CHECK(icp, SF_ERR_INVALID, "icp is NULL"); icp->prm.num_iters = v; return SF_OK; }
extern "C" int sf_icp_set_transformation_epsilon(sf_icp *icp, float v) { SF_CHECK(icp, SF_ERR_INVALID, "icp is NULL"); icp->prm.eps = v; return SF_OK; }
extern "C" int sf_icp_set_acceptable_mean_error(sf_icp *icp, float v) { SF_CHECK(icp, SF_ERR_INVALID, "icp is NULL"); icp->prm.accept = v; return SF_OK; }
extern "C" int sf_icp_set_debug_mode(sf_icp *icp, int on) { SF_CHECK(icp, SF_ERR_INVALID, "icp is NULL"); icp->debug = on; return SF_OK; }

extern "C" int sf_icp_set_initial_transformation(sf_icp *icp, const float T[16])
{
    SF_CHECK(icp && T, SF_ERR_INVALID, "bad arguments");
    if (icp->inits.size() < 16) icp->inits.assign(16, 0.0);
    for (int i = 0; i < 16; ++i) icp->inits[i] = T[i];
    return SF_OK;
}

extern "C" int sf_icp_set_initial_transformation_f64(sf_icp *icp, const double T[16])
{
    SF_CHECK(icp && T, SF_ERR_INVALID, "bad arguments");
    if (icp->inits.size() < 16) icp->inits.assign(16, 0.0);
    for (int i = 0; i < 16; ++i) icp->inits[i] = T[i];
    return SF_OK;
// ... 132 lines not shown
}

extern "C" int sf_icp_set_pipeline(sf_icp *icp, int on)
{
    SF_CHECK(icp, SF_ERR_INVALID, "icp is NULL");
    icp->pipeline = on != 0;
    return SF_OK;
}

extern "C" int sf_icp_set_tile_search(sf_icp *icp, int mode)
{
    SF_CHECK(icp && mode >= 0 && mode <= 2, SF_ERR_INVALID, "bad arguments");
    icp->tile_mode = mode;
    return SF_OK;
}

extern "C" int sf_icp_tile_info(sf_icp *icp, int64_t out[12])
{
    SF_CHECK(icp && out, SF_ERR_INVALID, "bad arguments");
    for (int i = 0; i < 12; ++i) out[i] = 0;
    out[0] = icp->tile_on ? 1 : 0;
    if (!icp->tile_on) return SF_OK;
    for (int a = 0; a < 3; ++a) { out[1 + a] = icp->tiles.tc[a]; out[4 + a] = icp->tiles.nt[a]; }
    if (icp->cur().tile_stats.p) {
        SF_HIP(hipSetDevice(icp->ctx->device));
        unsigned long long h[TILE_STATS];
        SF_HIP(hipMemcpyAsync(h, icp->cur().tile_stats.p, sizeof(h), hipMemcpyDeviceToHost, icp->ctx->stream));
        SF_HIP(hipStreamSynchronize(icp->ctx->stream));
        for (int i = 0; i < 5; ++i) out[7 + i] = (int64_t)h[i];
    }
    return SF_OK;
}

extern "C" int sf_icp_set_defer_search(sf_icp *icp, int on)
{
    SF_CHECK(icp, SF_ERR_INVALID, "icp is NULL");
    icp->defer = on != 0;
    return SF_OK;
}

extern "C" int sf_icp_defer_stats(sf_icp *icp, int64_t out[2])
{
    SF_CHECK(icp && out, SF_ERR_INVALID, "bad arguments");
    out[0] = out[1] = 0;
    if (!icp->df_planned || !icp->cur().df_stat.p) return SF_OK;
    uint32_t h[2] = {0u, 0u};
    SF_HIP(hipMemcpyAsync(h, icp->cur().df_stat.p, sizeof(h), hipMemcpyDeviceToHost, icp->ctx->stream));
    SF_HIP(hipStreamSynchronize(icp->ctx->stream));
    out[0] = (int64_t)h[0];
    out[1] = (int64_t)h[1];
    return SF_OK;
}

extern "C" int sf_icp_set_freeze(sf_icp *icp, int on)
{
    SF_CHECK(icp, SF_ERR_INVALID, "icp is NULL");
    SF_CHECK(on >= 0 && on <= 2, SF_ERR_INVALID, "sf_icp_set_freeze: 0 (off), 1 (auto) or 2 (always)");
    icp->freeze = on;
    return SF_OK;
}

namespace {
constexpr int FZ_FROM_DEFAULT = 5, FZ_PROBE_EVERY = 32;
void freeze_learn_schedule(sf_icp *icp)
{
    if (!icp->fz_from_auto || icp->last_fused || icp->shard || icp->last_mode != SF_ICP_P2PLANE) return;
    const int K = icp->prm.num_iters;
    if (++icp->fz_fetches >= FZ_PROBE_EVERY) { icp->fz_fetches = 0; icp->fz_from = FZ_FROM_DEFAULT; return; }
    if (!freeze_on(icp, icp->last_mode)) return;
    int latest = -1, never = 0;
    for (int b = 0; b < icp->src().batch; ++b) {
        const IcpState &S = icp->h_state[(size_t)b];
        if (S.froze_launch >= 0) latest = std::max(latest, S.froze_launch);
        else if (S.iterations >= K) never += 1;
    }
    if (latest < 0) icp->fz_from = std::max(FZ_FROM_DEFAULT, K);
    else if (never * 4 <= icp->src().batch) icp->fz_from = std::min(std::max(FZ_FROM_DEFAULT, latest), std::max(FZ_FROM_DEFAULT, K - 2));
}
}

extern "C" int sf_icp_set_robust_kernel(sf_icp *icp, int kind, double k)
{
    SF_CHECK(icp, SF_ERR_INVALID, "icp is NULL");
    SF_CHECK(kind >= SF_ROBUST_NONE && kind <= SF_ROBUST_GM, SF_ERR_INVALID, "unknown robust kernel %d", kind);
    SF_CHECK(kind == SF_ROBUST_NONE || (std::isfinite(k) && k > 0.0), SF_ERR_INVALID, "the robust kernel's scale must be finite and > 0 (got %g)", k);
    icp->robust_kind = kind;
    icp->robust_k = kind == SF_ROBUST_NONE ? 0.0 : k;
    return SF_OK;
}

extern "C" int sf_icp_set_freeze_params(sf_icp *icp, float guard_scale, float guard_min, float guard_max, int max_tries, int from_launch)
{
    SF_CHECK(icp, SF_ERR_INVALID, "icp is NULL");
    SF_CHECK(guard_scale >= 0.0f && guard_min >= 0.0f && guard_max >= guard_min && max_tries >= 0 && from_launch >= VERIFY_FROM_SEARCH && from_launch < 1024, SF_ERR_INVALID,
             "bad freeze parameters");
    icp->fz_prm = FreezeParams{guard_scale, guard_min, guard_max, max_tries};
    icp->fz_from = from_launch;
    icp->fz_from_auto = false;
    return SF_OK;
}

extern "C" int sf_icp_freeze_stats(sf_icp *icp, int64_t out[5])
{
    SF_CHECK(icp && out, SF_ERR_INVALID, "bad arguments");
    Lane &ln = icp->cur(); SrcSet &ss = icp->src();
    for (int i = 0; i < 5; ++i) out[i] = 0;
// ... 114 lines not shown
        Lane &ln = icp->cur();
        rc = lane_reserve(icp);
        if (rc != SF_OK) return;
        if (hipStreamWaitEvent(ln.stream, icp->main_mark, 0) != hipSuccess) { rc = SF_ERR_HIP; return; }
        if (ln.used && hipStreamWaitEvent(ln.stream, ln.done, 0) != hipSuccess) { rc = SF_ERR_HIP; return; }
        rc = wait_src_ahead(icp, ln.stream);
        if (rc != SF_OK) return;
        icp->ctx->stream = ln.stream;
        piped = true;
        if (hipEventRecord(ln.started, ln.stream) == hipSuccess) ln.started_rec = true;
    }
    ~LaneScope()
    {
        hipStream_t ran = icp->ctx->stream;
        icp->ctx->stream = main;
        Lane &ln = icp->cur(); SrcSet &ss = icp->src();
        if (!ln.done) return;
        if (ss.used && hipEventRecord(ss.used, ran) == hipSuccess) ss.used_rec = true;
        if (hipEventRecord(ln.done, ran) != hipSuccess) return;
        ln.used = true;
        if (piped) { hipError_t e = hipStreamWaitEvent(main, ln.done, 0); (void)e; }
    }
};

void lane_describe(sf_icp *icp, int mode, bool cov)
{
    sf_icp::LaneMeta &M = icp->cur().meta;
    M.valid = true; M.cov = cov; M.batch = icp->src().batch; M.mode = mode;
    M.inits = icp->inits; M.src_set = icp->src_set; M.src_version = icp->src_version;
}

int step_adopt_source(sf_icp *icp)
{
    SF_TRY(wait_src_ahead(icp, icp->ctx->stream));
    Lane &ln = icp->cur();
    const auto e0 = ln.state.epoch;
    SF_TRY(lane_reserve(icp));
    if (ln.state.epoch != e0) ln.meta.valid = false;
    SF_TRY(icp->xchg_own.reserve(sizeof(double) * REC_STRIDE * (size_t)std::max(icp->src().batch, 1)));
    icp->src_unmarked_use = true;
    return SF_OK;
}
}

extern "C" int sf_icp_align_batch_async(sf_icp *icp, int mode)
{
    SF_TRY(check_ready(icp, mode));
    SF_CHECK(!icp->shard, SF_ERR_STATE, "a sharded alignment needs the exchange between its halves: use sf_icp_step_begin / sf_icp_step_end");
    SF_HIP(hipSetDevice(icp->ctx->device));
    const SrcSet &ss = icp->src();
    icp->last_mode = mode;
    icp->last_fused = fused_eligible(icp, mode);
    icp->df_planned = !icp->last_fused && defer_planned(icp, mode);
    SF_TRY(order_lut_prepare(icp));
    const bool beside = icp->unfetched;
    LaneScope lanes(icp, icp->pipeline != 0 && !icp->last_fused && !icp->profiling && !ss.n_on_device);
    SF_TRY(lanes.rc);
    Lane &ln = icp->cur();
    if (!lanes.piped) SF_TRY(lane_reserve(icp));
    icp->unfetched = true;
    icp->prev_ok = lanes.piped && beside && icp->prev().meta.valid;
    icp->prev_cov_ok = icp->prev_ok && icp->prev().meta.cov;
    lane_describe(icp, mode, icp->cov_on != 0);
    hipStream_t s = icp->ctx->stream;
    if (icp->cov_on) SF_TRY(cov_alloc(icp));
    SF_TRY(launch_state_init(icp));
    if (icp->last_fused) {
        SF_TRY(order_queries(icp, mode));
        SF_TRY(launch_fused(icp, mode));
        if (icp->cov_on) {
            enqueue_cov(icp, mode, false);
            SF_HIP(hipGetLastError());
        }
        return SF_OK;
    }
    if (mode == SF_ICP_REF_CPP && icp->map->window.kind != 0) {
        SF_TRY(icp->map->d_window.reserve(sizeof(SfWindow)));
        hipLaunchKernelGGL(k_set_window, dim3(1), dim3(1), 0, s, icp->map->d_window.as<SfWindow>(), icp->map->window);
    }
    SF_TRY(order_queries(icp, mode));
    if (mode != SF_ICP_REF_CPP) SF_TRY(reuse_reset(icp, ss.n * ss.batch));
    if (freeze_on(icp, mode)) SF_TRY(freeze_alloc(icp));
    if (icp->use_graph && !icp->profiling && (icp->map->window.kind == 0 || mode == SF_ICP_REF_CPP)) {
        if (mode == SF_ICP_REF_CPP) {
            SF_TRY(ln.X.reserve(sizeof(float) * 3 * (size_t)std::max<int64_t>(ss.plane, 1)));
            SF_TRY(ln.corr.reserve(sizeof(float4) * (size_t)std::max<int64_t>(ss.plane, 1)));
        }
        const sf_icp::GraphKey key = graph_key_now(icp, mode);
        const bool hit = ln.graph_exec && key == ln.graph_key;
        if (!hit) {
            if (ln.graph_exec) { hipError_t e = hipGraphExecDestroy(ln.graph_exec); (void)e; ln.graph_exec = nullptr; }
            hipGraph_t graph = nullptr;
            SF_HIP(hipStreamBeginCapture(s, hipStreamCaptureModeThreadLocal));
            int rc = enqueue_align(icp, mode);
            hipError_t e = hipStreamEndCapture(s, &graph);
            if (rc != SF_OK) return rc;
            SF_CHECK(e == hipSuccess, SF_ERR_HIP, "hipStreamEndCapture: %s", hipGetErrorString(e));
            e = hipGraphInstantiate(&ln.graph_exec, graph, nullptr, nullptr, 0);
            hipError_t e2 = hipGraphDestroy(graph);
            (void)e2;
            SF_CHECK(e == hipSuccess, SF_ERR_HIP, "hipGraphInstantiate: %s", hipGetErrorString(e));
            ln.graph_key = key;
            icp->graph_captures += 1;
        }
        icp->graph_replays += 1;
        SF_HIP(hipGraphLaunch(ln.graph_exec, s));
        return SF_OK;
// ... 186 lines not shown
    hipStream_t s = icp->ctx->stream;
    IcpState *st = ln.state.as<IcpState>();
    SF_TRY(icp->own_blk.reserve(sizeof(uint32_t) * (size_t)nbf * (size_t)B));
    SF_TRY(icp->own_count.reserve(sizeof(uint32_t) * (size_t)B));
    SF_TRY(icp->own_off.reserve(sizeof(uint32_t) * (size_t)(B + 1)));
    const float *X = soa(ss.X0, ss.plane, 0), *Y = soa(ss.X0, ss.plane, 1), *Z = soa(ss.X0, ss.plane, 2);
    const dim3 grid((unsigned)nbf, (unsigned)B);
    if (resume) hipLaunchKernelGGL(k_own_resume, dim3(nblk(B, 64)), dim3(64), 0, s, st, B);
    SF_TRY(icp->own_keep.reserve(sizeof(unsigned long long) * (size_t)nbf * (size_t)B * (BLK / 64)));
    hipLaunchKernelGGL(k_own_count, grid, dim3(BLK), 0, s, X, Y, Z, n, st, icp->xlo, icp->xhi, icp->own_margin, icp->own_blk.as<uint32_t>(), nbf, icp->own_keep.as<unsigned long long>());
    hipLaunchKernelGGL(k_own_scan, dim3((unsigned)B), dim3(1024), 0, s, st, icp->own_blk.as<uint32_t>(), nbf, icp->own_count.as<uint32_t>());
    icp->h_own.assign((size_t)B + 1, 0u);
    SF_HIP(hipMemcpyAsync(icp->h_own.data() + 1, icp->own_count.p, sizeof(uint32_t) * (size_t)B, hipMemcpyDeviceToHost, s));
    SF_HIP(hipStreamSynchronize(s));
    uint32_t maxc = 0;
    for (int b = 0; b < B; ++b) {
        maxc = std::max(maxc, icp->h_own[(size_t)b + 1]);
        icp->h_own[(size_t)b + 1] += icp->h_own[(size_t)b];
    }
    const int64_t own = (int64_t)icp->h_own[(size_t)B];
    icp->own_total = own;
    icp->own_nblocks = (int)std::max<int64_t>(1, sf::div_up((int64_t)maxc, BLK * ss.qpl));
    SF_HIP(hipMemcpyAsync(icp->own_off.p, icp->h_own.data(), sizeof(uint32_t) * (size_t)(B + 1), hipMemcpyHostToDevice, s));
    const size_t cap = (size_t)std::max<int64_t>(own, 1);
    SF_TRY(icp->own_idx.reserve(sizeof(uint32_t) * cap));
    SF_TRY(ln.Xq.reserve(sizeof(float) * 3 * cap));
    if (own > 0) {
        hipLaunchKernelGGL(k_own_scatter, grid, dim3(BLK), 0, s, n, st, icp->own_keep.as<unsigned long long>(), icp->own_blk.as<uint32_t>(), nbf, icp->own_off.as<uint32_t>(),
                           icp->own_idx.as<uint32_t>());
        SF_TRY(run_order_sort(icp, B, (int64_t)maxc, own, icp->own_off.as<uint32_t>(), icp->own_idx.as<uint32_t>()));
    }
    hipLaunchKernelGGL(k_own_mark, dim3(nblk(B, 64)), dim3(64), 0, s, st, B);
    SF_HIP(hipGetLastError());
    return reuse_reset(icp, own);
}

}

extern "C" int sf_icp_step_begin(sf_icp *icp, int mode, int first)
{
    SF_TRY(check_ready(icp, mode));
    SF_CHECK(mode != SF_ICP_REF_CPP, SF_ERR_INVALID, "stepping supports O3D_P2P and P2PLANE");
    SF_CHECK(first >= 0 && first <= 2, SF_ERR_INVALID, "first must be 0, 1 or 2");
    SF_CHECK(!icp->cov_on, SF_ERR_STATE, COV_DECLINE_MSG);
    SF_CHECK(first != 2 || icp->shard, SF_ERR_STATE, "resume (first = 2) is a sharded-path operation");
    Lane &ln = icp->cur(); SrcSet &ss = icp->src();
    SF_HIP(hipSetDevice(icp->ctx->device));
    icp->last_mode = mode;
    icp->last_fused = false;
    if (first) SF_TRY(step_adopt_source(icp));
    if (first == 1) lane_describe(icp, mode, false);
    if (first) icp->df_planned = defer_planned(icp, mode);
    if (first) SF_TRY(order_lut_prepare(icp));
    if (first == 1) SF_TRY(launch_state_init(icp));
    if (icp->shard) {
        if (first) SF_TRY(shard_build(icp, first == 2));
    } else if (first) {
        SF_TRY(order_queries(icp, mode));
        SF_TRY(reuse_reset(icp, ss.n * ss.batch));
    }
    if (first) SF_TRY(freeze_start_pass(icp, mode));
    double *x = reinterpret_cast<double *>(sf_icp_exchange_ptr(icp, nullptr));
    hipStream_t s = icp->ctx->stream;
    const bool q1 = mode == SF_ICP_P2PLANE && ss.qpl > 1 && icp->fz_step < VERIFY_FROM_SEARCH;
    const int nb = icp->shard ? (q1 ? icp->own_nblocks * ss.qpl : icp->own_nblocks) : (q1 ? ss.nblocks : ss.nblocks_nn);
    const int qpl_now = q1 ? 1 : ss.qpl;
    const uint32_t *off = icp->shard ? icp->own_off.as<uint32_t>() : nullptr;
    if (mode == SF_ICP_O3D_P2P) {
        launch_nn_red<1>(icp, icp->shard);
        ProfScope ps(icp, SF_PROF_REDUCE);
        hipLaunchKernelGGL(k_reduce_only<1>, dim3(ss.batch), dim3(SBLK), 0, s, ln.state.as<IcpState>(), ln.partials.as<double>(), nb, x, off, ss.qpl, freeze_bufs(icp, false));
    } else {
        const bool df = !q1 && defer_now(icp, mode, icp->fz_step);
        if (freeze_nn_now(icp, mode)) launch_nn_red_fz(icp, icp->shard, icp->fz_step > icp->fz_from);
        else if (df) launch_nn_red_df(icp);
        else launch_nn_red<2>(icp, icp->shard, q1);
        ProfScope ps(icp, SF_PROF_REDUCE);
        hipLaunchKernelGGL(k_reduce_only<2>, dim3(ss.batch), dim3(SBLK), 0, s, ln.state.as<IcpState>(), ln.partials.as<double>(), nb, x, off, qpl_now,
                           freeze_bufs(icp, freeze_nn_now(icp, mode), df));
    }
    SF_HIP(hipGetLastError());
    return SF_OK;
}

extern "C" int sf_icp_step_end(sf_icp *icp, int mode, int last)
{
    SF_TRY(check_ready(icp, mode));
    Lane &ln = icp->cur(); SrcSet &ss = icp->src();
    (void)last;
    const double *x = reinterpret_cast<const double *>(sf_icp_exchange_ptr(icp, nullptr));
    hipStream_t s = icp->ctx->stream;
    const int K = icp->prm.num_iters;
    ProfScope ps(icp, SF_PROF_SOLVE);
    if (mode == SF_ICP_O3D_P2P)
        hipLaunchKernelGGL(k_solve_only<1>, dim3(nblk(ss.batch, 64)), dim3(64), 0, s, ln.state.as<IcpState>(), x, (int)ss.n, K, ss.batch, ss.d_boxes.as<ScanBox>(),
                           icp->shard ? icp->own_margin : 0.0f, (FreezeState *)nullptr, icp->fz_prm, 0);
    else
        hipLaunchKernelGGL(k_solve_only<2>, dim3(nblk(ss.batch, 64)), dim3(64), 0, s, ln.state.as<IcpState>(), x, (int)ss.n, K, ss.batch, ss.d_boxes.as<ScanBox>(),
                           icp->shard ? icp->own_margin : 0.0f, freeze_solve_now(icp, mode) ? ln.fz_state.as<FreezeState>() : (FreezeState *)nullptr, icp->fz_prm,
                           (int)(icp->fz_step + 2 < K));
    icp->fz_step += 1;
    SF_HIP(hipGetLastError());
    return SF_OK;
}

extern "C" int sf_icp_profile_read_launches(sf_icp *icp, float *ms, uint32_t *searched_queries, uint32_t *searched_waves, int64_t cap, int64_t *n)
// ... 233 lines not shown
```

slam_sensor_fusion_amd/csrc/sf_map.hip:

```cpp
#include "sf_common.hpp"
#include "sf_nn.hpp"
#include "sf_knn.hpp"

#include "sf_sort.hpp"
#include <cmath>
#include <cstring>

namespace {

inline unsigned nblk(int64_t n, int b = 256) { return (unsigned)sf::div_up(n > 0 ? n : 1, b); }

struct GridGeom { float org[3]; float inv_h; int dim[3]; uint64_t ncell; };

inline void prof_begin(sf_map *m)
{
    if (!m->profile) return;
    for (int i = 0; i < 2; ++i)
        if (!m->prof_ev[i] && hipEventCreate(&m->prof_ev[i]) != hipSuccess) { m->prof_ev[i] = nullptr; m->profile = false; return; }
    hipError_t e = hipEventRecord(m->prof_ev[0], m->ctx->stream);
    (void)e;
}
inline void prof_end(sf_map *m)
{
    if (!m->profile) return;
// ... 84 lines not shown
    const double step = (double)lattice * h;
    return (float)(std::floor((double)mn / step) * step);
}

inline bool table_by_scan(uint64_t ncell, int64_t n_points, int lattice) { return ncell > (1ull << 28) || lattice > 0 || ncell > 16ull * (uint64_t)std::max<int64_t>(n_points, 1); }

int build_cell_table(sf_map *m, const GridGeom &g, const void *sorted_keys, int64_t n_valid, bool wide, bool by_scan)
{
    sf_ctx *ctx = m->ctx;
    hipStream_t st = ctx->stream;
    uint32_t *cs = m->cell_start.as<uint32_t>() + 1;
    if (by_scan && n_valid > 0) {
        const size_t entries = (size_t)g.ncell + 8;
        SF_HIP(hipMemsetAsync(m->cell_start.p, 0, sizeof(uint32_t) * entries, st));
        if (wide) hipLaunchKernelGGL(k_cell_tails<uint64_t>, dim3(nblk(n_valid)), dim3(256), 0, st, static_cast<const uint64_t *>(sorted_keys), n_valid, cs);
        else hipLaunchKernelGGL(k_cell_tails<uint32_t>, dim3(nblk(n_valid)), dim3(256), 0, st, static_cast<const uint32_t *>(sorted_keys), n_valid, cs);
        const size_t piece = (size_t)1 << 30;
        uint32_t *t = m->cell_start.as<uint32_t>();
        for (size_t off = 0; off < entries; off += piece) {
            const size_t len = std::min(piece, entries - off);
            if (off > 0) hipLaunchKernelGGL(k_carry_max, dim3(1), dim3(1), 0, st, t + off);
            SF_TRY(sf::scan_u32<1>(ctx, t + off, t + off, (int64_t)len));
        }
    } else {
        hipLaunchKernelGGL(k_fill_u32, dim3(nblk((int64_t)g.ncell + 8)), dim3(256), 0, st, m->cell_start.as<uint32_t>(), (int64_t)g.ncell + 8, (uint32_t)n_valid);
        SF_HIP(hipMemsetAsync(m->cell_start.p, 0, sizeof(uint32_t), st));
        if (n_valid > 0)
            hipLaunchKernelGGL(k_cell_bounds, dim3(nblk(n_valid)), dim3(256), 0, st, static_cast<const uint32_t *>(sorted_keys), n_valid, (uint32_t)g.ncell, cs);
        else
            hipLaunchKernelGGL(k_fill_u32, dim3(nblk((int64_t)g.ncell + 2)), dim3(256), 0, st, cs, (int64_t)g.ncell + 2, 0u);
    }
    return SF_OK;
}
}

extern "C" int sf_map_create(sf_ctx *ctx, sf_map **out)
{
    SF_CHECK(ctx && out, SF_ERR_INVALID, "bad arguments");
    sf_map *m = new (std::nothrow) sf_map();
    SF_CHECK(m, SF_ERR_NOMEM, "out of host memory");
    m->ctx = ctx;
    sf::ctx_retain(ctx);
    *out = m;
    return SF_OK;
}

extern "C" void sf_map_destroy(sf_map *m)
{
    if (!m) return;
    hipError_t e = hipStreamSynchronize(m->ctx->stream);
    (void)e;
    m->pts4.release(); m->nrm4.release(); m->cov6.release(); m->d_window.release(); m->cell_start.release(); m->keys.release(); m->vals.release();
    m->keys2.release(); m->vals2.release(); m->pts4_alt.release(); m->patch_tmp.release();
    m->nrm4_alt.release(); m->cov6_alt.release(); m->carry_tmp.release(); m->carry_list.release();
    for (hipEvent_t ev : m->prof_ev)
        if (ev) { hipError_t e2 = hipEventDestroy(ev); (void)e2; }
    sf_ctx *ctx = m->ctx;
    delete m;
    sf::ctx_release(ctx);
}

extern "C" int sf_map_build(sf_map *m, sf_cloud *cloud, float cell)
{
    SF_CHECK(m && cloud, SF_ERR_INVALID, "bad arguments");
    SF_CHECK(cloud->n < (int64_t)(1 << 28), SF_ERR_OVERFLOW, "map too large for one GPU index (2^28 points): shard it");
    sf_ctx *ctx = m->ctx;
    SF_HIP(hipSetDevice(ctx->device));
    hipStream_t st = ctx->stream;
    const int64_t n = cloud->n;
    m->built = false;
    m->has_normals = false;
    m->nrm_estimated = false;
    m->nrm_knn_k = 0;
    m->n = 0;
    m->window.kind = 0;
    const float *xyz = cloud->xyz.as<float>();

    sf::MinMaxHost mm;
    if (n > 0 && cloud->stamp != 0 && cloud->bounds_stamp == cloud->stamp) {
        for (int d = 0; d < 3; ++d) { mm.mn[d] = cloud->bounds_mn[d]; mm.mx[d] = cloud->bounds_mx[d]; }
        mm.n_finite = n;
    } else {
        SF_TRY(sf::cloud_minmax(ctx, xyz, n, &mm));
    }
    const int64_t n_valid = mm.n_finite;

    double ext[3];
    for (int d = 0; d < 3; ++d) ext[d] = n_valid > 0 ? (double)mm.mx[d] - (double)mm.mn[d] : 0.0;
    double h = cell;
    if (!(h > 0)) {
        double vol = std::max(ext[0], 1e-3) * std::max(ext[1], 1e-3) * std::max(ext[2], 1e-3);
        h = std::cbrt(1.5 * vol / (double)std::max<int64_t>(n_valid, 1));
        h = std::min(std::max(h, 0.05), 1.0e6);
    }
    size_t free_b = 0, total_b = 0;
    SF_HIP(hipMemGetInfo(&free_b, &total_b));
    const double max_cells = std::min(34359738368.0, std::max(1.0e9, (double)free_b / 4.0 / sizeof(uint32_t)));
    int dim[3];
    float org[3] = {0, 0, 0};
    for (;;) {
        h = (double)(float)h;
        double cells = 1;
        bool ok = true;
        for (int d = 0; d < 3; ++d) {
            org[d] = n_valid > 0 ? grid_origin(mm.mn[d], h, m->origin_lattice) : 0.0f;
            double c = std::floor((n_valid > 0 ? (double)mm.mx[d] - (double)org[d] : 0.0) / h) + 1;
            if (c > 2.0e9) ok = false;
            dim[d] = ok ? (int)c : 1;
            cells *= c;
        }
        if (ok && cells <= max_cells) break;
        SF_CHECK(cell <= 0, SF_ERR_OVERFLOW, "cell %.4g gives too many cells for this extent (%.3g; this device holds a table of %.3g)", (double)cell, cells, max_cells);
        h *= 1.5;
    }
    GridGeom g;
    for (int d = 0; d < 3; ++d) { g.org[d] = org[d]; g.dim[d] = dim[d]; }
    g.inv_h = (float)(1.0 / h);
    g.ncell = (uint64_t)dim[0] * (uint64_t)dim[1] * (uint64_t)dim[2];
    const bool wide = g.ncell >= 0xffffffffull;
    const bool by_scan = table_by_scan(g.ncell, n_valid, m->origin_lattice);

    const size_t np = (size_t)std::max<int64_t>(n, 1), ksz = wide ? sizeof(uint64_t) : sizeof(uint32_t);
    SF_TRY(m->keys.reserve(ksz * np));
    SF_TRY(m->vals.reserve(sizeof(uint32_t) * np));
// ... 153 lines not shown
    const uint32_t del = wpre[w] + (uint32_t)__popc(words[w] & ((1u << bit) - 1u));
    const size_t o = (size_t)p - (size_t)del + (size_t)lo;
    const uint32_t id = j + f;
    if (CARRY >= 1 && o >= (size_t)n_out) return;
    pts_out[o] = make_float4(a.x, a.y, a.z, __uint_as_float(id));
    keys_out[o] = key;
    if (CARRY >= 1) {
        nrm_out[o] = nrm[p];
        if (CARRY == 2) {
#pragma unroll
            for (int d = 0; d < 3; ++d) cov_out[3 * o + d] = cov[3 * (size_t)p + d];
        }
    }
}

__global__ __launch_bounds__(256) void k_patch_new(PatchGeom geo, const float4 *__restrict__ pts, int64_t n_old, const uint32_t *__restrict__ bitmap, const uint32_t *__restrict__ blk_pre,
                                                    const uint32_t *__restrict__ skey, const uint32_t *__restrict__ sval, int64_t n_groups, const uint32_t *__restrict__ g_rank,
                                                    const uint32_t *__restrict__ fresh_pos, const float *__restrict__ g_centroid, float4 *__restrict__ pts_out,
                                                    uint32_t *__restrict__ keys_out)
{
    const int64_t e = (int64_t)blockIdx.x * blockDim.x + threadIdx.x;
    if (e >= n_groups) return;
    const uint32_t key = skey[e], g = sval[e], r = g_rank[g];
    int64_t lo = 0, hi = n_old;
    while (lo < hi) {
        const int64_t mid = (lo + hi) >> 1;
        const float4 a = pts[mid];
        const uint32_t k = patch_key(geo, a.x, a.y, a.z, nullptr);
        if (k < key || (k == key && __float_as_uint(a.w) < r)) lo = mid + 1;
        else hi = mid;
    }
    const size_t o = (size_t)e + (size_t)lo - (size_t)patch_del_before(bitmap, blk_pre, (uint32_t)lo);
    const uint32_t id = r + fresh_pos[g];
    pts_out[o] = make_float4(g_centroid[3 * (size_t)g], g_centroid[3 * (size_t)g + 1], g_centroid[3 * (size_t)g + 2], __uint_as_float(id));
    keys_out[o] = key;
}

int carry_reestimate(sf_map *m, const sf_cloud::MergeRecord &rec, const int old_dim[3], float radius, bool with_cov, int64_t *n_dirty);

}

extern "C" int sf_map_patch(sf_map *m, sf_cloud *cloud, int *patched)
{
    SF_CHECK(m && cloud, SF_ERR_INVALID, "bad arguments");
    SF_CHECK(m->built, SF_ERR_STATE, "sf_map_patch: the map has no index yet (sf_map_build)");
    SF_CHECK(m->ctx == cloud->ctx, SF_ERR_INVALID, "map and cloud must live on the same context");
    if (patched) *patched = 0;
    sf_ctx *ctx = m->ctx;
    SF_HIP(hipSetDevice(ctx->device));
    hipStream_t st = ctx->stream;
    const float cell = (float)m->h_exact;
    const sf_cloud::MergeRecord &rec = cloud->merge;
    const SfGrid old = m->grid;
    const uint64_t old_cells = (uint64_t)old.dim[0] * (uint64_t)old.dim[1] * (uint64_t)old.dim[2];
    const int64_t n_old = rec.n_old, ng = rec.n_groups, n_out = cloud->n;
    const int knn_k = (m->normals_carry && m->has_normals && m->nrm_estimated) ? m->nrm_knn_k : 0;
    const bool knn_cov = knn_k > 0 && m->has_cov && m->nrm_with_cov;
    const bool carry = m->normals_carry && m->has_normals && m->nrm_estimated && knn_k == 0;
    const float carry_radius = m->nrm_radius;
    const bool carry_cov = carry && m->has_cov && m->nrm_with_cov;
    auto knn_again = [&]() -> int {
        SF_TRY(sf_map_estimate_normals_knn(m, knn_k, carry_radius, knn_cov ? 1 : 0));
        m->carry_info[0] = 0;
        m->carry_info[1] = 0;
        m->carry_info[2] = m->grid.n;
        return SF_OK;
    };
    m->carry_info[0] = -1; m->carry_info[1] = m->carry_info[2] = 0; m->carry_info[3] = m->n;
    auto rebuild = [&](int why) -> int {
        if (patched) *patched = why;
        SF_TRY(sf_map_build(m, cloud, cell));
        m->carry_info[3] = m->n;
        if (knn_k > 0) return knn_again();
        if (!carry) return SF_OK;
        SF_TRY(sf_map_estimate_normals_cov(m, carry_radius, carry_cov ? 1 : 0));
        m->carry_info[0] = 0;
        m->carry_info[2] = m->grid.n;
        return SF_OK;
    };
    if (!rec.valid || rec.epoch != ctx->merge_epoch || rec.stamp_after != cloud->stamp || rec.stamp_before != m->src_stamp || n_old != m->n || old.n != m->n || ng <= 0 ||
        n_out != n_old + rec.n_fresh)
        return rebuild(SF_PATCH_NO_MERGE);
    if (n_out >= (int64_t)(1 << 28) || old_cells >= 0xffffffffull) return rebuild(SF_PATCH_LIMITS);

    float new_mn[3], new_mx[3];
    for (int d = 0; d < 3; ++d)
        if (rec.old_mn[d] != m->src_mn[d] || rec.old_mx[d] != m->src_mx[d]) return rebuild(SF_PATCH_NO_MERGE);
    if (rec.touched_extreme) {
        sf::MinMaxHost mm;
        SF_TRY(sf::cloud_minmax(ctx, cloud->xyz.as<float>(), n_out, &mm));
        if (mm.n_finite != n_out) return rebuild(SF_PATCH_BOUND_REPLACED);
        for (int d = 0; d < 3; ++d) { cloud->bounds_mn[d] = new_mn[d] = mm.mn[d]; cloud->bounds_mx[d] = new_mx[d] = mm.mx[d]; }
        cloud->bounds_stamp = cloud->stamp;
    } else {
        for (int d = 0; d < 3; ++d) { new_mn[d] = std::min(m->src_mn[d], rec.cen_mn[d]); new_mx[d] = std::max(m->src_mx[d], rec.cen_mx[d]); }
    }
    for (int d = 0; d < 3; ++d)
        if (grid_origin(new_mn[d], m->h_exact, m->origin_lattice) != old.org[d]) return rebuild(SF_PATCH_ORIGIN_MOVED);

    const double h = m->h_exact;
    size_t free_b = 0, total_b = 0;
    SF_HIP(hipMemGetInfo(&free_b, &total_b));
    free_b += m->cell_start.cap;
    const double max_cells = std::min(34359738368.0, std::max(1.0e9, (double)free_b / 4.0 / sizeof(uint32_t)));
    GridGeom g;
    PatchGeom pg;
// ... 574 lines not shown
    SF_TRY(m->nrm4.reserve(sizeof(float4) * (size_t)std::max<int64_t>(m->n, 1)));
    m->has_cov = false;
    if (with_covariance) SF_TRY(m->cov6.reserve(sizeof(double) * 6 * (size_t)std::max<int64_t>(m->n, 1)));
    const int R = normals_reach(radius, m->grid.h);
    prof_begin(m);
    if (m->grid.n > 0)
        hipLaunchKernelGGL(k_normals, dim3(nblk(m->grid.n)), dim3(256), 0, ctx->stream, m->grid, (double)radius * (double)radius, R, m->nrm4.as<float4>(),
                           with_covariance ? m->cov6.as<double>() : nullptr);
    prof_end(m);
    SF_HIP(hipGetLastError());
    SF_HIP(hipStreamSynchronize(ctx->stream));
    prof_read(m);
    m->grid.nrm = m->nrm4.as<float4>();
    m->has_normals = true;
    m->has_cov = with_covariance != 0;
    m->nrm_estimated = true;
    m->nrm_knn_k = 0;
    m->nrm_radius = radius;
    m->nrm_with_cov = with_covariance != 0;
    m->generation = sf::next_generation();
    return SF_OK;
}

extern "C" int sf_map_estimate_normals_knn(sf_map *m, int k, float max_radius, int with_covariance)
{
    SF_CHECK(m && m->built, SF_ERR_STATE, "map not built");
    SF_CHECK(k >= 1 && k <= SF_KNN_MAX, SF_ERR_INVALID, "k must be 1 .. %d (got %d)", SF_KNN_MAX, k);
    SF_CHECK(!std::isnan(max_radius), SF_ERR_INVALID, "max_radius must be a number (<= 0 or inf: no limit)");
    sf_ctx *ctx = m->ctx;
    SF_HIP(hipSetDevice(ctx->device));
    SF_TRY(m->nrm4.reserve(sizeof(float4) * (size_t)std::max<int64_t>(m->n, 1)));
    m->has_cov = false;
    if (with_covariance) SF_TRY(m->cov6.reserve(sizeof(double) * 6 * (size_t)std::max<int64_t>(m->n, 1)));
    const float thr = (max_radius > 0 && std::isfinite(max_radius)) ? (float)(max_radius * max_radius) : INFINITY;
    SfWindow none{};
    prof_begin(m);
    if (m->grid.n > 0)
        hipLaunchKernelGGL(k_normals_knn, dim3(nblk(m->grid.n)), dim3(256), 0, ctx->stream, m->grid, none, k, thr, m->nrm4.as<float4>(), with_covariance ? m->cov6.as<double>() : nullptr);
    prof_end(m);
    SF_HIP(hipGetLastError());
    SF_HIP(hipStreamSynchronize(ctx->stream));
    prof_read(m);
    m->grid.nrm = m->nrm4.as<float4>();
    m->has_normals = true;
    m->has_cov = with_covariance != 0;
    m->nrm_estimated = true;
    m->nrm_knn_k = k;
    m->nrm_radius = max_radius;
    m->nrm_with_cov = with_covariance != 0;
    m->generation = sf::next_generation();
    return SF_OK;
}

extern "C" int sf_map_profile_launches(sf_map *m, int on)
{
    SF_CHECK(m, SF_ERR_INVALID, "bad arguments");
    m->profile = on != 0;
    m->last_launch_ms = -1.0f;
    return SF_OK;
}

extern "C" int sf_map_last_launch_ms(sf_map *m, float *ms)
{
    SF_CHECK(m && ms, SF_ERR_INVALID, "bad arguments");
    SF_CHECK(m->profile && m->last_launch_ms >= 0.0f, SF_ERR_STATE, "nothing timed (sf_map_profile_launches, then a query or an estimate)");
    *ms = m->last_launch_ms;
    return SF_OK;
}

extern "C" int sf_map_set_normals_carry(sf_map *m, int on)
{
    SF_CHECK(m, SF_ERR_INVALID, "bad arguments");
    m->normals_carry = on != 0;
    return SF_OK;
}

extern "C" int sf_map_normals_carry_info(sf_map *m, int64_t out[4])
{
    SF_CHECK(m && out, SF_ERR_INVALID, "bad arguments");
    for (int k = 0; k < 4; ++k) out[k] = m->carry_info[k];
    return SF_OK;
}

extern "C" int sf_map_estimate_normals(sf_map *m, float radius) { return sf_map_estimate_normals_cov(m, radius, 0); }

extern "C" int sf_map_download_covariances(sf_map *m, double *cov6, int64_t cap, int64_t *n)
{
    SF_CHECK(m && m->built && m->has_cov, SF_ERR_STATE, "no covariances (sf_map_estimate_normals_cov with with_covariance = 1)");
    if (n) *n = m->n;
    SF_CHECK(cap >= m->n && cov6, SF_ERR_INVALID, "buffer too small");
    sf_ctx *ctx = m->ctx;
    SF_HIP(hipSetDevice(ctx->device));
    sf::DevBuf dc;
    const size_t bytes = sizeof(double) * 6 * (size_t)std::max<int64_t>(m->n, 1);
    SF_TRY(dc.reserve(bytes));
    SF_HIP(hipMemsetAsync(dc.p, 0, bytes, ctx->stream));
    if (m->grid.n > 0)
        hipLaunchKernelGGL(k_cov_to_host_order, dim3(nblk(m->grid.n)), dim3(256), 0, ctx->stream, m->grid, m->cov6.as<double>(), dc.as<double>());
    SF_HIP(hipMemcpyAsync(cov6, dc.p, sizeof(double) * 6 * (size_t)m->n, hipMemcpyDeviceToHost, ctx->stream));
    SF_HIP(hipStreamSynchronize(ctx->stream));
    return SF_OK;
}

extern "C" int sf_map_set_normals(sf_map *m, const float *normals, int64_t n)
{
    SF_CHECK(m && m->built, SF_ERR_STATE, "map not built");
// ... 39 lines not shown
```

slam_sensor_fusion_amd/csrc/sf_nn_red_body.inc:

```
    constexpr int NREC = MODE == 2 ? NREC_PLANE : NREC_P2P;
    const int L = blockIdx.y * gridDim.x + blockIdx.x;
    const int kk = L >> 3;
    const int b = kk % (int)gridDim.y;
    const int bx = (L & 7) * ((int)gridDim.x >> 3) + kk / (int)gridDim.y;
    if (bx >= nblocks) return;
    const IcpState *S = st + b;
    if (S->done) return;
    const int n_live = SHARD ? (int)(own_off[b + 1] - own_off[b]) : n;
    if (SHARD && bx * (BLK * Q) >= n_live) return;
    __shared__ sf::WaveNN nn_ws[BLK / 64];
    __shared__ double stage[BLK / 64][32];
    const int wv = threadIdx.x >> 6, lane = threadIdx.x & 63;
#ifdef SF_PHASE_TRACE
    sf::PhaseClock pclk, *pc = &pclk;
    pclk.start();
#else
    sf::PhaseClock *pc = nullptr;
#endif
    LanePair P[Q];
    bool fast = false;
    if (Q > 1 && qcache != nullptr && S->cache_live != 0 && S->n_research >= VERIFY_FROM_SEARCH) {
        const float m_now = (float)S->motion;
        bool any_need = false;
#pragma unroll
        for (int u = 0; u < Q; ++u) {
            const int slot = bx * (BLK * Q) + u * BLK + (int)threadIdx.x;
            const QueryIn q = query_in<MODE, SHARD>(X0x, X0y, X0z, n, b, S, xlo, xhi, own_off, qcache, cache_n, true, slot, n_live);
            sf::NNHit hit, seed;
            float4 tn;
            any_need = reuse_certificate(q.valid, q.qx, q.qy, q.qz, thr, m_now, q.e, q.c1, q.c2, hit, tn, seed) || any_need;
            P[u] = make_pair(q, hit, tn);
        }
        fast = __ballot(any_need) == 0ull;
    }
    if (!fast) {
        asm volatile("" ::: "memory");
#pragma unroll
        for (int u = 0; u < Q; ++u) {
            const int slot = bx * (BLK * Q) + u * BLK + (int)threadIdx.x;
            P[u] = nn_pair<MODE, WINDOW, SHARD>(g, w, X0x, X0y, X0z, n, b, S, thr, xlo, xhi, own_off, qcache, cache_n, slot, n_live, &nn_ws[wv], stats, pc);
        }
    }
#pragma unroll
    for (int h = 0; h < 2; ++h) {
        double v[16];
#pragma unroll
        for (int k = 0; k < 16; ++k) v[k] = 0.0;
#pragma unroll
        for (int u = 0; u < Q; ++u) {
            const PairTerms t = pair_terms<MODE>(P[u]);
            if constexpr (ROBUST) add_half_robust(t, h, v, robust_weight(rk, t.r));
            else add_half<MODE>(t, h, v);
        }
        if (MODE == 1 && h == 1) {
            const double t1 = wave_reduce_1(v[0]);
            if (lane == 0) stage[wv][16] = t1;
        } else {
            const double t0 = wave_reduce_16(v);
            if ((lane & 3) == 0) stage[wv][16 * h + (lane >> 2)] = t0;
        }
    }
    SF_PH(pc, 7);
    __syncthreads();
    if (threadIdx.x < NREC) {
        const int c = threadIdx.x;
        double *dst = partials + ((size_t)b * nblocks + bx) * REC_STRIDE;
        dst[c] = ((stage[0][c] + stage[1][c]) + stage[2][c]) + stage[3][c];
    }
#ifdef SF_PHASE_TRACE
    SF_PH(pc, 8);
    pclk.count(14, 1u);
    if (lane == 0) {
        unsigned long long *dstp = g_phase_trace + (size_t)(L & (sf::PH_SHARDS - 1)) * sf::PH_SLOTS;
        for (int i = 0; i < sf::PH_SLOTS; ++i) atomicAdd(&dstp[i], (unsigned long long)pclk.acc[i]);
    }
#endif
```

Baseline: 19370.

## Add precomputed map k-NN adjacency to certify nearest neighbours without grid search

Builds a per-map-point adjacency table holding its 6 nearest neighbours plus first-neighbour and K-th-neighbour radii. During ICP, queries whose reuse certificate fails try the previous match's adjacency line. Either a triangle-inequality test on r1 proves the old match is still nearest, or the 6 neighbours are scanned and checked against rK, so the full grid search can be skipped. The cost is a one-off k-NN build over the whole map, extra per-query loads and divergence, stat atomics, and a new graph-key dependency.

After: 19170. 0.99x the previous value.

```diff
diff --git a/include/slamfusion.h b/include/slamfusion.h
--- a/include/slamfusion.h
+++ b/include/slamfusion.h
@@ -104,6 +104,10 @@
 #define SF_KNN_MAX 64
 int sf_map_knn(sf_map *m, const float *queries, int64_t n, int k, float max_d2, int32_t *idx, float *d2, int32_t *count);
 int sf_map_estimate_normals_knn(sf_map *m, int k, float max_radius, int with_covariance);
+#define SF_ADJ_K 6
+int sf_map_build_adjacency(sf_map *m);
+int sf_map_adjacency_info(sf_map *m, int64_t out[6], float *radius, float *build_ms);
+int sf_map_download_adjacency(sf_map *m, int32_t *idx, float *r1, float *rK, int64_t cap, int64_t *n);
 int sf_map_profile_launches(sf_map *m, int on);
 int sf_map_last_launch_ms(sf_map *m, float *ms);
 
@@ -173,6 +177,8 @@
 int sf_icp_freeze_stats(sf_icp *icp, int64_t out[5]);
 int sf_icp_set_defer_search(sf_icp *icp, int on);
 int sf_icp_defer_stats(sf_icp *icp, int64_t out[2]);
+int sf_icp_set_adjacency(sf_icp *icp, int mode);
+int sf_icp_adjacency_stats(sf_icp *icp, int64_t out[3]);
 #define SF_ROBUST_NONE 0
 #define SF_ROBUST_HUBER 1
 #define SF_ROBUST_CAUCHY 2
diff --git a/slam_sensor_fusion_amd/api.py b/slam_sensor_fusion_amd/api.py
--- a/slam_sensor_fusion_amd/api.py
+++ b/slam_sensor_fusion_amd/api.py
@@ -404,6 +404,21 @@
         r = float(max_radius)
         _check(self.lib.sf_map_estimate_normals_knn(self.h, C.c_int(int(k)), C.c_float(r if np.isfinite(r) else 0.0), C.c_int(int(covariance))))
 
+    def build_adjacency(self):
+        _check(self.lib.sf_map_build_adjacency(self.h))
+
+    def adjacency_info(self):
+        a, r, ms = (C.c_int64 * 6)(), C.c_float(), C.c_float()
+        _check(self.lib.sf_map_adjacency_info(self.h, a, C.byref(r), C.byref(ms)))
+        return {"valid": bool(a[0]), "k": a[1], "line_bytes": a[2], "lines": a[3], "builds": a[4], "drops": a[5], "radius": r.value, "build_ms": ms.value}
+
+    def download_adjacency(self):
+        info = self.adjacency_info()
+        n, k = max(int(info["lines"]), 1), int(info["k"])
+        idx, r1, rk, got = np.empty((n, k), np.int32), np.empty(n, np.float32), np.empty(n, np.float32), C.c_int64()
+        _check(self.lib.sf_map_download_adjacency(self.h, _p(idx), _p(r1), _p(rk), C.c_int64(n), C.byref(got)))
+        return idx[:got.value], r1[:got.value], rk[:got.value]
+
     def set_normals_carry(self, on=True):
         _check(self.lib.sf_map_set_normals_carry(self.h, C.c_int(int(bool(on)))))
         return self
@@ -633,6 +648,14 @@
         a = (C.c_int64 * 2)()
         _check(self.lib.sf_icp_defer_stats(self.h, a))
         return {"deferred_queries": a[0], "capped_waves": a[1]}
+
+    def set_adjacency(self, mode="auto"):
+        _check(self.lib.sf_icp_set_adjacency(self.h, C.c_int({"off": 0, "auto": 1, "always": 2}.get(mode, mode))))
+
+    def adjacency_stats(self):
+        a = (C.c_int64 * 3)()
+        _check(self.lib.sf_icp_adjacency_stats(self.h, a))
+        return {"anchor": a[0], "adjacency": a[1], "searched": a[2]}
 
     def set_query_order(self, order="auto"):
         _check(self.lib.sf_icp_set_query_order(self.h, C.c_int({"auto": 0, "as_given": 1, "cell": 2}[order])))
diff --git a/slam_sensor_fusion_amd/csrc/sf_common.hpp b/slam_sensor_fusion_amd/csrc/sf_common.hpp
--- a/slam_sensor_fusion_amd/csrc/sf_common.hpp
+++ b/slam_sensor_fusion_amd/csrc/sf_common.hpp
@@ -156,6 +156,16 @@
     int64_t n;
 };
 
+#ifndef SF_ADJ_K
+#define SF_ADJ_K 6
+#endif
+namespace sf {
+struct alignas(32) AdjLine {
+    float r1, rK;
+    int32_t idx[SF_ADJ_K];
+};
+}
+
 struct sf_map {
     sf_ctx *ctx = nullptr;
     sf::DevBuf pts4, nrm4, cell_start, keys, vals, keys2, vals2;
@@ -179,6 +189,12 @@
     int64_t n = 0;
     bool built = false, has_normals = false, has_cov = false;
     uint64_t generation = 0;
+    sf::DevBuf adj;
+    bool adj_valid = false;
+    uint64_t adj_stamp = 0;
+    float adj_radius = 0;
+    int64_t adj_builds = 0, adj_drops = 0;
+    float adj_build_ms = -1.0f;
     SfGrid grid{};
     SfWindow window{};
 };
@@ -192,6 +208,8 @@
 int ensure_scratch(sf_ctx *ctx, size_t bytes);
 int upload_staged(sf_ctx *ctx, void *dst, const void *src, size_t bytes);
 uint64_t next_generation();
+int map_adjacency_enqueue(sf_map *m);
+inline void map_adjacency_drop(sf_map *m) { if (m->adj_valid) m->adj_drops += 1; m->adj_valid = false; m->adj_stamp = 0; }
 inline void cloud_touch(sf_cloud *c) { c->stamp = next_generation(); c->merge.valid = false; }
 void ctx_retain(sf_ctx *ctx);
 void ctx_release(sf_ctx *ctx);
diff --git a/slam_sensor_fusion_amd/csrc/sf_icp.hip b/slam_sensor_fusion_amd/csrc/sf_icp.hip
--- a/slam_sensor_fusion_amd/csrc/sf_icp.hip
+++ b/slam_sensor_fusion_amd/csrc/sf_icp.hip
@@ -536,11 +536,14 @@
     return P;
 }
 
+struct AdjArg { const sf::AdjLine *lines; unsigned long long *stat; int t1_from, t2_from; };
+constexpr int ADJ_STAT_SHARDS = 256;
+
 template <int MODE, bool WINDOW, bool SHARD>
 __device__ __forceinline__ LanePair nn_pair(const SfGrid &g, const SfWindow &w, const float *__restrict__ X0x, const float *__restrict__ X0y, const float *__restrict__ X0z,
                                             int n, int b, const IcpState *S, float thr, float xlo, float xhi, const uint32_t *__restrict__ own_off,
                                             float4 *__restrict__ qcache, int64_t cache_n, int slot, int n_live, sf::WaveNN *ws, uint32_t *__restrict__ stats,
-                                            sf::PhaseClock *pc = nullptr)
+                                            const AdjArg &adj, sf::PhaseClock *pc = nullptr)
 {
     const bool cache_live = qcache != nullptr && S->cache_live != 0;
     const QueryIn q = query_in<MODE, SHARD>(X0x, X0y, X0z, n, b, S, xlo, xhi, own_off, qcache, cache_n, cache_live, slot, n_live);
@@ -551,8 +554,66 @@
     sf::NNHit hit;
     float4 tn;
     sf::NNHit seed;
-    const bool need = reuse_certificate(q.valid, qx, qy, qz, thr, m_now, q.e, q.c1, q.c2, hit, tn, seed);
+    bool need = reuse_certificate(q.valid, qx, qy, qz, thr, m_now, q.e, q.c1, q.c2, hit, tn, seed);
+    if (!WINDOW && !SHARD && adj.lines != nullptr) {
+        const bool cand = need && seed.j >= 0 && S->n_research >= adj.t1_from;
+        if (__ballot(cand) != 0ull) {
+            int tier = 0;
+            if (cand) {
+                const int32_t ja = seed.j;
+                const float4 *line = reinterpret_cast<const float4 *>(adj.lines + ja);
+                const float4 l0 = line[0];
+                const float da = sqrtf(seed.d2) * 1.0001f + 1.0e-6f;
+                sf::NNHit h = seed;
+                h.lb2 = 3.0e38f;
+                float room = 0.0f;
+                if (da + da < l0.x) {
+                    tier = 1;
+                    room = l0.x - da;
+                } else if (da < l0.y && S->n_research >= adj.t2_from) {
+                    const float4 l1 = line[1];
+                    static_assert(SF_ADJ_K == 6, "the two 16-byte halves of a line are read as such");
+                    const int32_t id[SF_ADJ_K] = {__float_as_int(l0.z), __float_as_int(l0.w), __float_as_int(l1.x), __float_as_int(l1.y), __float_as_int(l1.z), __float_as_int(l1.w)};
+                    float4 p[SF_ADJ_K];
+#pragma unroll
+                    for (int r = 0; r < SF_ADJ_K; ++r) p[r] = sf::load_point(g, (uint32_t)id[r], id[r] >= 0);
+#pragma unroll
+                    for (int r = 0; r < SF_ADJ_K; ++r) sf::consider<false, true>(w, p[r].x, p[r].y, p[r].z, id[r], id[r] >= 0, qx, qy, qz, h);
+                    room = l0.y - da;
+                    if (sqrtf(h.d2) * 1.0001f + 1.0e-6f < room) tier = 2;
+                    else seed = sf::NNHit{h.d2, h.j, h.px, h.py, h.pz, 0.0f};
+                }
+                if (tier != 0) {
+                    need = false;
+                    const bool none = !(h.d2 < thr);
+                    const float dn = fminf(fminf(sqrtf(h.lb2), room), none ? sqrtf(h.d2) : 3.0e38f);
+                    const float en = fmaxf(dn * 0.9999f + m_now * 0.999998f - 1.0e-6f, 1.0e-30f);
+                    if (!none) {
+                        hit.d2 = h.d2; hit.j = h.j; hit.px = h.px; hit.py = h.py; hit.pz = h.pz;
+                        tn = q.c2;
+                        if (MODE == 2 && h.j != ja) tn = g.nrm[h.j];
+                    }
+                    if (none || h.j != ja) {
+                        qcache[o] = none ? make_float4(0.f, 0.f, 0.f, __int_as_float(-1)) : make_float4(h.px, h.py, h.pz, __int_as_float(h.j));
+                        if (MODE == 2) qcache[(size_t)cache_n + o] = make_float4(tn.x, tn.y, tn.z, en);
+                        else ecache[o] = en;
+                    } else {
+                        if (MODE == 2) reinterpret_cast<float *>(qcache + (size_t)cache_n + o)[3] = en;
+                        else ecache[o] = en;
+                    }
+                }
+            }
+            const unsigned long long t1 = __ballot(tier == 1), t2 = __ballot(tier == 2);
+            if (adj.stat && (threadIdx.x & 63) == 0) {
+                unsigned long long *sh = adj.stat + 4 * ((blockIdx.x + blockIdx.y * gridDim.x) & (ADJ_STAT_SHARDS - 1));
+                if (t1) atomicAdd(&sh[0], (unsigned long long)__popcll(t1));
+                if (t2) atomicAdd(&sh[1], (unsigned long long)__popcll(t2));
+            }
+        }
+    }
     const unsigned long long need_mask = __ballot(need);
+    if (!WINDOW && !SHARD && adj.stat && (threadIdx.x & 63) == 0 && need_mask)
+        atomicAdd(&adj.stat[4 * ((blockIdx.x + blockIdx.y * gridDim.x) & (ADJ_STAT_SHARDS - 1)) + 2], (unsigned long long)__popcll(need_mask));
     if (stats && (threadIdx.x & 63) == 0 && need_mask) {
         uint32_t *sh = stats + 2 * ((blockIdx.x + blockIdx.y * gridDim.x) & (NN_STATS_SHARDS - 1));
         atomicAdd(&sh[0], (uint32_t)__popcll(need_mask));
@@ -680,7 +741,7 @@
 template <int MODE, bool WINDOW, bool SHARD, int Q>
 __global__ __launch_bounds__(BLK, NN_RED_WAVES) void k_nn_red(SfGrid g, SfWindow w, const float *__restrict__ X0x, const float *__restrict__ X0y, const float *__restrict__ X0z,
                                                 int n, const IcpState *__restrict__ st, float thr, float xlo, float xhi, double *__restrict__ partials, int nblocks,
-                                                const uint32_t *__restrict__ own_off, float4 *__restrict__ qcache, int64_t cache_n, uint32_t *__restrict__ stats)
+                                                const uint32_t *__restrict__ own_off, float4 *__restrict__ qcache, int64_t cache_n, uint32_t *__restrict__ stats, AdjArg adj)
 {
     constexpr bool ROBUST = false;
     [[maybe_unused]] constexpr RobustArg rk{0, 0.0};
@@ -690,7 +751,7 @@
 template <bool WINDOW, bool SHARD, int Q>
 __global__ __launch_bounds__(BLK, NN_RED_WAVES) void k_nn_red_rob(SfGrid g, SfWindow w, const float *__restrict__ X0x, const float *__restrict__ X0y, const float *__restrict__ X0z,
                                                     int n, const IcpState *__restrict__ st, float thr, float xlo, float xhi, double *__restrict__ partials, int nblocks,
-                                                    const uint32_t *__restrict__ own_off, float4 *__restrict__ qcache, int64_t cache_n, uint32_t *__restrict__ stats, RobustArg rk)
+                                                    const uint32_t *__restrict__ own_off, float4 *__restrict__ qcache, int64_t cache_n, uint32_t *__restrict__ stats, RobustArg rk, AdjArg adj)
 {
     constexpr int MODE = 2;
     constexpr bool ROBUST = true;
@@ -1485,7 +1546,7 @@
             const uint32_t *list = act_all + (size_t)b * nblocks * FZ_CAP + (size_t)first;
             const uint32_t i = (uint32_t)(wv * 64 + lane);
             const int slot = i < cnt ? (int)list[i] : n_live;
-            const LanePair A1 = nn_pair<MODE, false, SHARD>(g, w, X0x, X0y, X0z, n, b, S, thr, xlo, xhi, own_off, qcache, cache_n, slot, n_live, &nn_ws[wv], stats);
+            const LanePair A1 = nn_pair<MODE, false, SHARD>(g, w, X0x, X0y, X0z, n, b, S, thr, xlo, xhi, own_off, qcache, cache_n, slot, n_live, &nn_ws[wv], stats, AdjArg{nullptr, nullptr, 0, 0});
 #pragma unroll
             for (int h = 0; h < 2; ++h) {
                 double v[16];
@@ -1535,7 +1596,7 @@
 #pragma unroll
         for (int u = 0; u < Q; ++u) {
             const int slot = bx * (BLK * Q) + u * BLK + (int)threadIdx.x;
-            P[u] = nn_pair<MODE, false, SHARD>(g, w, X0x, X0y, X0z, n, b, S, thr, xlo, xhi, own_off, qcache, cache_n, slot, n_live, &nn_ws[wv], stats);
+            P[u] = nn_pair<MODE, false, SHARD>(g, w, X0x, X0y, X0z, n, b, S, thr, xlo, xhi, own_off, qcache, cache_n, slot, n_live, &nn_ws[wv], stats, AdjArg{nullptr, nullptr, 0, 0});
             if (fmode == 1 && !attempted) active[u] = slot < n_live;
         }
     }
@@ -1670,7 +1731,7 @@
 template <int Q>
 __global__ __launch_bounds__(BLK, NN_RED_WAVES) void k_nn_red_df(SfGrid g, SfWindow w, const float *__restrict__ X0x, const float *__restrict__ X0y, const float *__restrict__ X0z,
                                                                  int n, const IcpState *__restrict__ st, float thr, double *__restrict__ partials, int nblocks,
-                                                                 float4 *__restrict__ qcache, int64_t cache_n, uint32_t *__restrict__ stats, DeferBufs df)
+                                                                 float4 *__restrict__ qcache, int64_t cache_n, uint32_t *__restrict__ stats, DeferBufs df, AdjArg adj)
 {
     constexpr int MODE = 2;
     constexpr int NREC = NREC_PLANE;
@@ -1725,7 +1786,7 @@
 #pragma unroll
         for (int u = 0; u < Q; ++u) {
             const int slot = bx * (BLK * Q) + u * BLK + (int)threadIdx.x;
-            P[u] = nn_pair<MODE, false, false>(g, w, X0x, X0y, X0z, n, b, S, thr, 0.0f, 0.0f, nullptr, qcache, cache_n, slot, n, &nn_ws[wv], stats);
+            P[u] = nn_pair<MODE, false, false>(g, w, X0x, X0y, X0z, n, b, S, thr, 0.0f, 0.0f, nullptr, qcache, cache_n, slot, n, &nn_ws[wv], stats, adj);
         }
     }
 #pragma unroll
@@ -1752,7 +1813,7 @@
 template <int Q>
 __global__ __launch_bounds__(BLK, 2) void k_nn_deferred(SfGrid g, SfWindow w, const float *__restrict__ X0x, const float *__restrict__ X0y, const float *__restrict__ X0z,
                                                                    int n, const IcpState *__restrict__ st, float thr, int nblocks, float4 *__restrict__ qcache, int64_t cache_n,
-                                                                   uint32_t *__restrict__ stats, DeferBufs df)
+                                                                   uint32_t *__restrict__ stats, DeferBufs df, AdjArg adj)
 {
     constexpr int MODE = 2;
     constexpr int NW = BLK / 64;
@@ -1802,7 +1863,7 @@
             const uint32_t i = q0 + (uint32_t)threadIdx.x;
             if (q0 + (uint32_t)(wv * 64) < total) {
                 const int slot = i < total ? (int)list[i] : n;
-                const LanePair A1 = nn_pair<MODE, false, false>(g, w, X0x, X0y, X0z, n, b, S, thr, 0.0f, 0.0f, nullptr, qcache, cache_n, slot, n, &nn_ws[wv], stats);
+                const LanePair A1 = nn_pair<MODE, false, false>(g, w, X0x, X0y, X0z, n, b, S, thr, 0.0f, 0.0f, nullptr, qcache, cache_n, slot, n, &nn_ws[wv], stats, adj);
 #pragma unroll
                 for (int h = 0; h < 2; ++h) {
                     double v[16];
@@ -2080,6 +2141,8 @@
         freeze_after_update(S, F, m0, S->motion, fp, request, upd);
     }
 }
+
+__global__ void k_adj_stat_init(unsigned long long *__restrict__ stat) { stat[blockIdx.x * blockDim.x + threadIdx.x] = 0ull; }
 
 __global__ void k_fz_init(FreezeState *__restrict__ fz, int batch, uint32_t *__restrict__ df_stat)
 {
@@ -2659,15 +2722,15 @@
     struct GraphKey {
         int mode = -1, iters = -1, batch = -1, window = -1, ordered = -1, reuse = -1, robust_kind = -1, cov_on = -1;
         int64_t n = -1;
-        const void *map = nullptr;
-        uint64_t map_generation = 0, epochs = 0;
+        const void *map = nullptr, *adj = nullptr;
+        uint64_t map_generation = 0, epochs = 0, adj_stamp = 0;
         float max_corr = 0, accept = 0, eps = 0;
         double robust_k = 0;
         double cov_prm[5] = {0, 0, 0, 0, 0};
         bool operator==(const GraphKey &o) const
         {
             return mode == o.mode && iters == o.iters && batch == o.batch && window == o.window && ordered == o.ordered && reuse == o.reuse && n == o.n && map == o.map &&
-                   map_generation == o.map_generation && epochs == o.epochs && max_corr == o.max_corr && accept == o.accept && eps == o.eps &&
+                   map_generation == o.map_generation && epochs == o.epochs && adj == o.adj && adj_stamp == o.adj_stamp && max_corr == o.max_corr && accept == o.accept && eps == o.eps &&
                    robust_kind == o.robust_kind && robust_k == o.robust_k && cov_on == o.cov_on && std::memcmp(cov_prm, o.cov_prm, sizeof(cov_prm)) == 0;
         }
     };
@@ -2687,6 +2750,7 @@
         sf::DevBuf state, d_inits, partials;
         sf::DevBuf fz_state, fz_part, fz_cnt, fz_ids, fz_all;
         sf::DevBuf df_cnt, df_ids, df_part, df_stat;
+        sf::DevBuf adj_stat;
         sf::DevBuf qtkey, tseg, tile_stats;
         sf::DevBuf cov_part, cov_out;
         hipGraphExec_t graph_exec = nullptr;
@@ -2756,6 +2820,11 @@
     bool fz_from_auto = true;
     int fz_fetches = 0;
     int fz_step = 0;
+    int adjacency = 0;
+    const void *adj_seen_map = nullptr;
+    uint64_t adj_seen_gen = 0;
+    bool adj_counted = false;
+    int adj_t1_from = 1, adj_t2_from = 1;
     int defer = 1;
     bool df_planned = false;
     int64_t nn_stats_used = 0;
@@ -2874,6 +2943,41 @@
     SF_HIP(hipGetLastError());
     icp->order_lut_gen = icp->map->generation;
     return SF_OK;
+}
+
+const sf::AdjLine *adjacency_lines(const sf_icp *icp, bool sharded)
+{
+    const sf_map *m = icp->map;
+    if (icp->adjacency == 0 || sharded || icp->shard || !icp->reuse || m->window.kind != 0 || !m->adj_valid) return nullptr;
+    return m->adj.as<sf::AdjLine>();
+}
+
+AdjArg adjacency_arg(sf_icp *icp, bool sharded)
+{
+    AdjArg a{adjacency_lines(icp, sharded), nullptr, icp->adj_t1_from, icp->adj_t2_from};
+    if (!sharded && !icp->shard && icp->map->window.kind == 0) a.stat = icp->cur().adj_stat.as<unsigned long long>();
+    return a;
+}
+
+int adjacency_prepare(sf_icp *icp, int mode)
+{
+    sf_map *m = icp->map;
+    const SrcSet &ss = icp->src();
+    const bool seen = icp->adj_seen_map == (const void *)m && icp->adj_seen_gen == m->generation;
+    icp->adj_seen_map = (const void *)m;
+    icp->adj_seen_gen = m->generation;
+    if (mode == SF_ICP_REF_CPP || icp->last_fused || icp->adjacency == 0 || icp->shard || !icp->reuse || m->window.kind != 0 || m->adj_valid || m->grid.n <= 0) return SF_OK;
+    if (!(icp->adjacency == 2 || (seen && ss.n * ss.batch >= ORDER_AUTO_MIN_QUERIES))) return SF_OK;
+    SF_TRY(sf::map_adjacency_enqueue(m));
+    icp->mark_valid = false;
+    return SF_OK;
+}
+
+void adjacency_stat_begin(sf_icp *icp)
+{
+    Lane &ln = icp->cur();
+    icp->adj_counted = ln.adj_stat.p != nullptr;
+    if (ln.adj_stat.p) hipLaunchKernelGGL(k_adj_stat_init, dim3(4 * ADJ_STAT_SHARDS / 256), dim3(256), 0, icp->ctx->stream, ln.adj_stat.as<unsigned long long>());
 }
 
 int run_order_sort(sf_icp *icp, int nseg, int64_t longest, int64_t total, const uint32_t *seg_off, const uint32_t *src_idx)
@@ -3044,6 +3148,7 @@
     SF_TRY(ln.state.reserve(sizeof(IcpState) * (size_t)batch));
     SF_TRY(ln.d_inits.reserve(sizeof(double) * 16 * (size_t)batch));
     SF_TRY(ln.partials.reserve(sizeof(double) * (size_t)REC_STRIDE * (size_t)std::max(ss.nblocks, 1) * (size_t)batch));
+    SF_TRY(ln.adj_stat.reserve(sizeof(unsigned long long) * 4 * (size_t)ADJ_STAT_SHARDS));
     return SF_OK;
 }
 
@@ -3146,12 +3251,13 @@
     k.n = (mode == SF_ICP_REF_CPP && ss.batch == 1) ? -ss.n_cap : ss.n;
     k.map = (const void *)icp->map;
     k.map_generation = icp->map->generation;
+    k.adj = (const void *)adjacency_lines(icp, false); k.adj_stamp = k.adj ? icp->map->adj_stamp : 0;
     k.robust_kind = robust_on(icp, mode) ? icp->robust_kind : SF_ROBUST_NONE; k.robust_k = robust_on(icp, mode) ? icp->robust_k : 0.0;
     k.cov_on = icp->cov_on;
     if (icp->cov_on) { const double cp[5] = {icp->cov_arg.sensor_sigma, icp->cov_arg.thr_t, icp->cov_arg.thr_r, icp->cov_arg.infl_t, icp->cov_arg.infl_r}; std::memcpy(k.cov_prm, cp, sizeof(cp)); }
     k.max_corr = icp->prm.max_corr; k.accept = icp->prm.accept; k.eps = icp->prm.eps + icp->fz_prm.guard_scale * 1.0e-3f + icp->fz_prm.guard_min + icp->fz_prm.guard_max + (float)icp->fz_prm.max_tries;
     const sf::DevBuf *bufs[] = {&ss.X0, &ss.X0r, &ln.X, &ln.Xq, &ln.qcache, &ln.corr, &ln.state, &ln.partials, &icp->d_box, &ss.d_boxes, &ss.n_dev,
-                                &icp->map->pts4, &icp->map->nrm4, &icp->map->cell_start, &icp->map->d_window, &ln.fz_state, &ln.fz_part, &ln.fz_cnt, &ln.fz_ids, &ln.fz_all, &ln.df_cnt, &ln.df_ids, &ln.df_part, &ln.df_stat, &ln.tseg, &ln.tile_stats, &ln.cov_part, &ln.cov_out};
+                                &icp->map->pts4, &icp->map->nrm4, &icp->map->cell_start, &icp->map->d_window, &ln.fz_state, &ln.fz_part, &ln.fz_cnt, &ln.fz_ids, &ln.fz_all, &ln.df_cnt, &ln.df_ids, &ln.df_part, &ln.df_stat, &ln.adj_stat, &ln.tseg, &ln.tile_stats, &ln.cov_part, &ln.cov_out};
     k.epochs = (uint64_t)ss.plane;
     for (const sf::DevBuf *b : bufs) k.epochs = (k.epochs * 1000003ull + b->epoch) * 1000003ull + (uint64_t)(uintptr_t)b->p;
     return k;
@@ -3175,11 +3281,12 @@
     uint32_t *stats = nullptr;
     if (icp->profiling && icp->nn_stats.p && icp->nn_stats_used < sf_icp::NN_STATS_CAP) stats = icp->nn_stats.as<uint32_t>() + 2 * NN_STATS_SHARDS * icp->nn_stats_used++;
     const bool win = m->window.kind != 0;
+    const AdjArg adj = adjacency_arg(icp, sharded);
     if (MODE == 2 && robust_on(icp, MODE)) {
         const RobustArg rk = robust_arg(icp);
 #define SF_LAUNCH_NNRED_ROB(W, S, QQ)                                                                                                                         \
     hipLaunchKernelGGL((k_nn_red_rob<W, S, QQ>), grid, blk, 0, s, m->grid, m->window, x, y, z, (int)ss.n, st, thr, icp->xlo, icp->xhi, part, nb, \
-                       icp->own_off.as<uint32_t>(), icp->reuse ? ln.qcache.as<float4>() : nullptr, icp->cache_n, stats, rk)
+                       icp->own_off.as<uint32_t>(), icp->reuse ? ln.qcache.as<float4>() : nullptr, icp->cache_n, stats, rk, adj)
         const bool q1 = ss.qpl == 1 || one_per_lane;
         if (win && sharded) { if (q1) SF_LAUNCH_NNRED_ROB(true, true, 1); else SF_LAUNCH_NNRED_ROB(true, true, SF_WIDE_QPL); }
         else if (win) { if (q1) SF_LAUNCH_NNRED_ROB(true, false, 1); else SF_LAUNCH_NNRED_ROB(true, false, SF_WIDE_QPL); }
@@ -3190,7 +3297,7 @@
     }
 #define SF_LAUNCH_NNRED_Q(W, S, QQ)                                                                                                                              \
     hipLaunchKernelGGL((k_nn_red<MODE, W, S, QQ>), grid, blk, 0, s, m->grid, m->window, x, y, z, (int)ss.n, st, thr, icp->xlo, icp->xhi, part, nb, \
-                       icp->own_off.as<uint32_t>(), icp->reuse ? ln.qcache.as<float4>() : nullptr, icp->cache_n, stats)
+                       icp->own_off.as<uint32_t>(), icp->reuse ? ln.qcache.as<float4>() : nullptr, icp->cache_n, stats, adj)
 #define SF_LAUNCH_NNRED(W, S)                                  \
     do {                                                       \
         if (ss.qpl == 1 || one_per_lane) SF_LAUNCH_NNRED_Q(W, S, 1); \
@@ -3288,7 +3395,7 @@
     Lane &ln = icp->cur(); SrcSet &ss = icp->src();
     sf_map *m = icp->map;
     hipLaunchKernelGGL((k_nn_deferred<SF_WIDE_QPL>), dim3((unsigned)FZ_FEW, (unsigned)ss.batch), dim3(BLK), 0, icp->ctx->stream, m->grid, m->window, queries(icp, 0), queries(icp, 1), queries(icp, 2),
-                       (int)ss.n, ln.state.as<IcpState>(), o3d_thr(icp), ss.nblocks_nn, ln.qcache.as<float4>(), icp->cache_n, stats, defer_bufs(icp));
+                       (int)ss.n, ln.state.as<IcpState>(), o3d_thr(icp), ss.nblocks_nn, ln.qcache.as<float4>(), icp->cache_n, stats, defer_bufs(icp), adjacency_arg(icp, false));
 }
 
 void launch_nn_red_df(sf_icp *icp)
@@ -3301,7 +3408,7 @@
     uint32_t *stats = nullptr;
     if (icp->profiling && icp->nn_stats.p && icp->nn_stats_used < sf_icp::NN_STATS_CAP) stats = icp->nn_stats.as<uint32_t>() + 2 * NN_STATS_SHARDS * icp->nn_stats_used++;
     hipLaunchKernelGGL((k_nn_red_df<SF_WIDE_QPL>), grid, blk, 0, icp->ctx->stream, m->grid, m->window, queries(icp, 0), queries(icp, 1), queries(icp, 2), (int)ss.n, ln.state.as<IcpState>(),
-                       o3d_thr(icp), ln.partials.as<double>(), nb, ln.qcache.as<float4>(), icp->cache_n, stats, defer_bufs(icp));
+                       o3d_thr(icp), ln.partials.as<double>(), nb, ln.qcache.as<float4>(), icp->cache_n, stats, defer_bufs(icp), adjacency_arg(icp, false));
     launch_nn_deferred(icp, stats);
 }
 
@@ -3431,6 +3538,7 @@
     const int K = icp->prm.num_iters;
     const int B = ss.batch;
     const int n = (int)ss.n;
+    if (mode != SF_ICP_REF_CPP) adjacency_stat_begin(icp);
     if (mode == SF_ICP_O3D_P2P) {
         for (int k = 0; k <= K; ++k) {
             if (tile_launch(icp, k)) launch_tile_search<1>(icp, false);
@@ -3714,6 +3822,9 @@
     icp->prm.accept = acceptable_mean_error;
     icp->prm.eps = transformation_epsilon;
     if (const char *e = std::getenv("SF_ORDER_LUT")) icp->order_lut_on = std::atoi(e) != 0;
+    if (const char *e = std::getenv("SF_ADJ_T1_FROM")) icp->adj_t1_from = std::atoi(e);
+    if (const char *e = std::getenv("SF_ADJ_T2_FROM")) icp->adj_t2_from = std::atoi(e);
+    if (const char *e = std::getenv("SF_ADJACENCY")) icp->adjacency = std::min(std::max(std::atoi(e), 0), 2);
     *out = icp;
     return SF_OK;
 }
@@ -3952,6 +4063,30 @@
     return SF_OK;
 }
 
+extern "C" int sf_icp_set_adjacency(sf_icp *icp, int mode)
+{
+    SF_CHECK(icp, SF_ERR_INVALID, "icp is NULL");
+    SF_CHECK(mode >= 0 && mode <= 2, SF_ERR_INVALID, "adjacency mode must be 0 (off), 1 (auto) or 2 (always), got %d", mode);
+    icp->adjacency = mode;
+    return SF_OK;
+}
+
+extern "C" int sf_icp_adjacency_stats(sf_icp *icp, int64_t out[3])
+{
+    SF_CHECK(icp && out, SF_ERR_INVALID, "bad arguments");
+    out[0] = out[1] = out[2] = 0;
+    if (!icp->adj_counted || !icp->cur().adj_stat.p) return SF_OK;
+    std::vector<unsigned long long> h(4 * (size_t)ADJ_STAT_SHARDS, 0ull);
+    SF_HIP(hipMemcpyAsync(h.data(), icp->cur().adj_stat.p, sizeof(unsigned long long) * h.size(), hipMemcpyDeviceToHost, icp->ctx->stream));
+    SF_HIP(hipStreamSynchronize(icp->ctx->stream));
+    for (size_t k = 0; k < h.size(); k += 4) {
+        out[0] += (int64_t)h[k];
+        out[1] += (int64_t)h[k + 1];
+        out[2] += (int64_t)h[k + 2];
+    }
+    return SF_OK;
+}
+
 extern "C" int sf_icp_set_freeze(sf_icp *icp, int on)
 {
     SF_CHECK(icp, SF_ERR_INVALID, "icp is NULL");
@@ -4172,7 +4307,9 @@
     icp->last_mode = mode;
     icp->last_fused = fused_eligible(icp, mode);
     icp->df_planned = !icp->last_fused && defer_planned(icp, mode);
+    icp->adj_counted = false;
     SF_TRY(order_lut_prepare(icp));
+    SF_TRY(adjacency_prepare(icp, mode));
     const bool beside = icp->unfetched;
     LaneScope lanes(icp, icp->pipeline != 0 && !icp->last_fused && !icp->profiling && !ss.n_on_device);
     SF_TRY(lanes.rc);
@@ -4465,6 +4602,8 @@
     if (first == 1) lane_describe(icp, mode, false);
     if (first) icp->df_planned = defer_planned(icp, mode);
     if (first) SF_TRY(order_lut_prepare(icp));
+    if (first) SF_TRY(adjacency_prepare(icp, mode));
+    if (first) adjacency_stat_begin(icp);
     if (first == 1) SF_TRY(launch_state_init(icp));
     if (icp->shard) {
         if (first) SF_TRY(shard_build(icp, first == 2));
diff --git a/slam_sensor_fusion_amd/csrc/sf_map.hip b/slam_sensor_fusion_amd/csrc/sf_map.hip
--- a/slam_sensor_fusion_amd/csrc/sf_map.hip
+++ b/slam_sensor_fusion_amd/csrc/sf_map.hip
@@ -160,7 +160,7 @@
     (void)e;
     m->pts4.release(); m->nrm4.release(); m->cov6.release(); m->d_window.release(); m->cell_start.release(); m->keys.release(); m->vals.release();
     m->keys2.release(); m->vals2.release(); m->pts4_alt.release(); m->patch_tmp.release();
-    m->nrm4_alt.release(); m->cov6_alt.release(); m->carry_tmp.release(); m->carry_list.release();
+    m->nrm4_alt.release(); m->cov6_alt.release(); m->carry_tmp.release(); m->carry_list.release(); m->adj.release();
     for (hipEvent_t ev : m->prof_ev)
         if (ev) { hipError_t e2 = hipEventDestroy(ev); (void)e2; }
     sf_ctx *ctx = m->ctx;
@@ -178,6 +178,7 @@
     const int64_t n = cloud->n;
     m->built = false;
     m->has_normals = false;
+    sf::map_adjacency_drop(m);
     m->nrm_estimated = false;
     m->nrm_knn_k = 0;
     m->n = 0;
@@ -437,6 +438,7 @@
     const float cell = (float)m->h_exact;
     const sf_cloud::MergeRecord &rec = cloud->merge;
     const SfGrid old = m->grid;
+    sf::map_adjacency_drop(m);
     const uint64_t old_cells = (uint64_t)old.dim[0] * (uint64_t)old.dim[1] * (uint64_t)old.dim[2];
     const int64_t n_old = rec.n_old, ng = rec.n_groups, n_out = cloud->n;
     const int knn_k = (m->normals_carry && m->has_normals && m->nrm_estimated) ? m->nrm_knn_k : 0;
@@ -1117,6 +1119,118 @@
     return SF_OK;
 }
 
+namespace {
+__global__ __launch_bounds__(256) void k_adjacency(SfGrid g, SfWindow w, float thr, sf::AdjLine *__restrict__ out)
+{
+    constexpr int K = SF_ADJ_K;
+    __shared__ sf::WaveKNN ws[256 / 64];
+    const int lane = (int)(threadIdx.x & 63u), wv = (int)(threadIdx.x >> 6);
+    const int64_t base = ((int64_t)blockIdx.x * 4 + wv) * 64;
+    if (base >= g.n) return;
+    const int64_t i = base + lane;
+    const float4 mine = i < g.n ? g.pts[i] : make_float4(0.0f, 0.0f, 0.0f, 0.0f);
+    const int nq = (int)min((int64_t)64, g.n - base);
+    sf::AdjLine my;
+    my.r1 = my.rK = 0.0f;
+#pragma unroll
+    for (int r = 0; r < K; ++r) my.idx[r] = -1;
+    for (int t = 0; t < nq; ++t) {
+        const float qx = __shfl(mine.x, t), qy = __shfl(mine.y, t), qz = __shfl(mine.z, t);
+        unsigned long long key;
+        const int cnt = sf::knn_search<false>(g, w, qx, qy, qz, K + 2, thr, &ws[wv], key);
+        const uint32_t self = (uint32_t)(base + t);
+        const unsigned long long sb = __ballot(lane < cnt && (uint32_t)key == self);
+        const int s = sb != 0ull ? __ffsll((long long)sb) - 1 : 64;
+        float d2_first = thr, d2_last = thr;
+#pragma unroll
+        for (int r = 0; r <= K; ++r) {
+            const int src = r < s ? r : r + 1;
+            const unsigned long long kr = __shfl(key, src & 63);
+            const bool has = src < cnt;
+            const float d2 = __uint_as_float((uint32_t)(kr >> 32));
+            if (r == 0 && has) d2_first = d2;
+            if (r == K && has) d2_last = d2;
+            if (r < K && lane == t) my.idx[r] = has ? (int32_t)(uint32_t)kr : -1;
+        }
+        if (lane == t) {
+            my.r1 = sqrtf(d2_first) * 0.9999f;
+            my.rK = sqrtf(d2_last) * 0.9999f;
+        }
+    }
+    if (i < g.n) out[i] = my;
+}
+}
+
+int sf::map_adjacency_enqueue(sf_map *m)
+{
+    if (m->adj_valid) return SF_OK;
+    sf_ctx *ctx = m->ctx;
+    SF_TRY(m->adj.reserve(sizeof(sf::AdjLine) * (size_t)std::max<int64_t>(m->grid.n, 1)));
+    const float R = m->grid.h;
+    SfWindow none{};
+    if (m->grid.n > 0) hipLaunchKernelGGL(k_adjacency, dim3(nblk(m->grid.n)), dim3(256), 0, ctx->stream, m->grid, none, R * R, m->adj.as<sf::AdjLine>());
+    SF_HIP(hipGetLastError());
+    m->adj_valid = true;
+    m->adj_stamp = sf::next_generation();
+    m->adj_radius = R;
+    m->adj_builds += 1;
+    m->adj_build_ms = -1.0f;
+    return SF_OK;
+}
+
+extern "C" int sf_map_build_adjacency(sf_map *m)
+{
+    SF_CHECK(m && m->built, SF_ERR_STATE, "map not built");
+    if (m->adj_valid) return SF_OK;
+    sf_ctx *ctx = m->ctx;
+    SF_HIP(hipSetDevice(ctx->device));
+    hipEvent_t ev[2] = {nullptr, nullptr};
+    SF_HIP(hipEventCreate(&ev[0]));
+    hipError_t e = hipEventCreate(&ev[1]);
+    if (e != hipSuccess) { hipError_t e2 = hipEventDestroy(ev[0]); (void)e2; SF_HIP(e); }
+    int rc = hipEventRecord(ev[0], ctx->stream) == hipSuccess ? SF_OK : SF_ERR_HIP;
+    if (rc == SF_OK) rc = sf::map_adjacency_enqueue(m);
+    if (rc == SF_OK && hipEventRecord(ev[1], ctx->stream) != hipSuccess) rc = SF_ERR_HIP;
+    if (rc == SF_OK && hipStreamSynchronize(ctx->stream) != hipSuccess) rc = SF_ERR_HIP;
+    float ms = -1.0f;
+    if (rc == SF_OK && hipEventElapsedTime(&ms, ev[0], ev[1]) == hipSuccess) m->adj_build_ms = ms;
+    for (hipEvent_t x : ev) { hipError_t e2 = hipEventDestroy(x); (void)e2; }
+    if (rc != SF_OK) { sf::map_adjacency_drop(m); sf::set_error("sf_map_build_adjacency: the build failed on the device"); }
+    return rc;
+}
+
+extern "C" int sf_map_adjacency_info(sf_map *m, int64_t out[6], float *radius, float *build_ms)
+{
+    SF_CHECK(m && out, SF_ERR_INVALID, "bad arguments");
+    out[0] = m->adj_valid ? 1 : 0;
+    out[1] = SF_ADJ_K;
+    out[2] = (int64_t)sizeof(sf::AdjLine);
+    out[3] = m->adj_valid ? m->grid.n : 0;
+    out[4] = m->adj_builds;
+    out[5] = m->adj_drops;
+    if (radius) *radius = m->adj_valid ? m->adj_radius : 0.0f;
+    if (build_ms) *build_ms = m->adj_valid ? m->adj_build_ms : -1.0f;
+    return SF_OK;
+}
+
+extern "C" int sf_map_download_adjacency(sf_map *m, int32_t *idx, float *r1, float *rK, int64_t cap, int64_t *n)
+{
+    SF_CHECK(m && m->built && m->adj_valid, SF_ERR_STATE, "no adjacency table (sf_map_build_adjacency)");
+    if (n) *n = m->grid.n;
+    SF_CHECK(cap >= m->grid.n && idx && r1 && rK, SF_ERR_INVALID, "buffer too small");
+    sf_ctx *ctx = m->ctx;
+    SF_HIP(hipSetDevice(ctx->device));
+    std::vector<sf::AdjLine> h((size_t)m->grid.n);
+    if (m->grid.n > 0) SF_HIP(hipMemcpyAsync(h.data(), m->adj.p, sizeof(sf::AdjLine) * h.size(), hipMemcpyDeviceToHost, ctx->stream));
+    SF_HIP(hipStreamSynchronize(ctx->stream));
+    for (size_t j = 0; j < h.size(); ++j) {
+        for (int r = 0; r < SF_ADJ_K; ++r) idx[j * SF_ADJ_K + r] = h[j].idx[r];
+        r1[j] = h[j].r1;
+        rK[j] = h[j].rK;
+    }
+    return SF_OK;
+}
+
 extern "C" int sf_map_profile_launches(sf_map *m, int on)
 {
     SF_CHECK(m, SF_ERR_INVALID, "bad arguments");
diff --git a/slam_sensor_fusion_amd/csrc/sf_nn_red_body.inc b/slam_sensor_fusion_amd/csrc/sf_nn_red_body.inc
--- a/slam_sensor_fusion_amd/csrc/sf_nn_red_body.inc
+++ b/slam_sensor_fusion_amd/csrc/sf_nn_red_body.inc
@@ -38,7 +38,7 @@
 #pragma unroll
         for (int u = 0; u < Q; ++u) {
             const int slot = bx * (BLK * Q) + u * BLK + (int)threadIdx.x;
-            P[u] = nn_pair<MODE, WINDOW, SHARD>(g, w, X0x, X0y, X0z, n, b, S, thr, xlo, xhi, own_off, qcache, cache_n, slot, n_live, &nn_ws[wv], stats, pc);
+            P[u] = nn_pair<MODE, WINDOW, SHARD>(g, w, X0x, X0y, X0z, n, b, S, thr, xlo, xhi, own_off, qcache, cache_n, slot, n_live, &nn_ws[wv], stats, adj, pc);
         }
     }
 #pragma unroll
```
